# 0215Arthur/Pytorch_News_Recommender

Measured on AMD Instinct MI355X. Metric: users/sec (train step) NRMS MIND-small hist=50 cand=5, higher is better.
Workload: dtype f16 (MFMA inputs and saved activations; fp32 accumulate, softmax, loss, master weights and Adam); 1 GPU; configs[1] shapes: NRMS(nrms_v0) train step, 512 users/GPU, hist=50, cand=5, title_len=30, d=300, h=10, q=200, V=45800, dropout=0.2, Adam(lr=1e-3); users_per_gpu=512, global_batch=512, parallelism=dp1, precision=fp16, resident_batches=32

## Files before the change

include/nrms_hip.h:

```cpp
#ifndef NRMS_HIP_H
#define NRMS_HIP_H

#include <stddef.h>
#include <stdint.h>

#ifdef __cplusplus
extern "C" {
#endif

#define NRMS_OK            0
#define NRMS_EINVAL       -1
#define NRMS_ELAUNCH      -2
#define NRMS_EWORKSPACE   -3

#define NRMS_PRECISION_FP32   0
#define NRMS_PRECISION_BF16X3 1
#define NRMS_PRECISION_BF16   2
#define NRMS_FP16_KP 320
#define NRMS_FP16_DP 320
#define NRMS_FP16_QP 224
#define NRMS_PRECISION_FP16   3

#define NRMS_FLAG_PAD_ROW_ZERO 1
#define NRMS_FLAG_DEFER_WQKV 2
// ... 11 lines not shown
    int32_t  q_dim;
    int32_t  vocab;
    float    p_drop_embed;
    float    p_drop_ctx;
    int32_t  precision;
    int32_t  use_output_proj;
    int32_t  mask_mode;
    int32_t  flags;
    uint64_t seed;
    float    loss_scale;
    float    p_drop_attn;
    const int32_t* seq_index;
} nrms_encoder_desc;

typedef struct nrms_encoder_weights {
    const float* table;
    const float* w_qkv;
    const float* b_qkv;
    const float* w_o;
    const float* b_o;
    const float* w_add;
    const float* b_add;
    const float* q_vec;
} nrms_encoder_weights;

typedef struct nrms_encoder_grads {
    float* table;
    float* w_qkv;
    float* b_qkv;
    float* w_o;
    float* b_o;
    float* w_add;
    float* b_add;
    float* q_vec;
} nrms_encoder_grads;

typedef struct nrms_encoder_acts {
    float* x;
    float* qkv;
    float* attn;
    float* ctx;
    float* t;
    float* w;
    void*  scratch;
} nrms_encoder_acts;

size_t nrms_encoder_fwd_scratch_bytes(const nrms_encoder_desc* desc);
size_t nrms_encoder_fused_qkv_bytes(const nrms_encoder_desc* desc);
int nrms_encoder_fwd(const nrms_encoder_desc* desc, const nrms_encoder_weights* w,
                     const int64_t* ids, const float* x, const uint8_t* mask ,
                     const nrms_encoder_acts* acts, float* out, void* stream);

size_t nrms_encoder_bwd_workspace_bytes(const nrms_encoder_desc* desc);
int nrms_encoder_bwd(const nrms_encoder_desc* desc, const nrms_encoder_weights* w,
                     const int64_t* ids, const float* x, const uint8_t* mask,
                     const nrms_encoder_acts* acts, const float* dout,
                     const nrms_encoder_grads* grads, float* dx,
                     void* workspace, size_t workspace_bytes, void* stream);
typedef struct nrms_table_adam {
    float*   param;
    float*   exp_avg;
    float*   exp_avg_sq;
    double   lr, beta1, beta2, eps;
    int32_t  step;
    float    grad_scale;
    int32_t* n_nonfinite;
} nrms_table_adam;
int nrms_encoder_bwd_adam(const nrms_encoder_desc* desc, const nrms_encoder_weights* w,
                          const int64_t* ids, const float* x, const uint8_t* mask,
                          const nrms_encoder_acts* acts, const float* dout,
                          const nrms_encoder_grads* grads, float* dx,
                          void* workspace, size_t workspace_bytes, const nrms_table_adam* table_adam, void* stream);
int nrms_encoder_bwd_wqkv(const nrms_encoder_desc* desc, const int64_t* ids, const float* x,
                          const nrms_encoder_acts* acts, const nrms_encoder_grads* grads,
                          void* workspace, size_t workspace_bytes, void* stream);
int nrms_encoder_join(void* stream);

int nrms_sanitize_ids(const int64_t* src, int64_t* dst, int64_t n, int32_t vocab, int32_t* n_bad, void* stream);
int nrms_sanitize_ids_i32(const int32_t* src, int64_t* dst, int64_t n, int32_t vocab, int32_t* n_bad, void* stream);

int nrms_title_dedup(const int64_t* ids, int64_t n_titles, int32_t seq_len, int32_t* table, int64_t table_size,
                     int32_t* inverse, int32_t* rep_rows, int32_t* n_unique, void* stream);

int nrms_click_score_fwd(int32_t B, int32_t C, int32_t d, const float* cand, const float* user,
                         const uint8_t* mask, float* scores, void* stream);
int nrms_click_score_indexed(int32_t B, int32_t C, int32_t d, const float* news_vec, int64_t n_vec, const int32_t* index,
                             const float* user, const uint8_t* mask, float* scores, void* stream);
int nrms_click_score_bwd(int32_t B, int32_t C, int32_t d, const float* cand, const float* user,
                         const uint8_t* mask, const float* dscores, float* dcand, float* duser,
                         void* stream);

int nrms_ce_loss_fwd_bwd(int32_t B, int32_t C, const float* scores, float* loss_sum,
                         float* dscores, float grad_scale, void* stream);

int nrms_adam_step(size_t n, float* param, const float* grad, float* exp_avg, float* exp_avg_sq,
                   double lr, double beta1, double beta2, double eps, int32_t step, float grad_scale,
                   void* stream);

int nrms_adam_step_guarded(size_t n, float* param, const float* grad, float* exp_avg, float* exp_avg_sq,
                           double lr, double beta1, double beta2, double eps, int32_t step, float grad_scale,
                           int32_t* n_nonfinite, void* stream);
int nrms_adam_step_rest(size_t n, float* param, const float* grad, float* exp_avg, float* exp_avg_sq,
                        double lr, double beta1, double beta2, double eps, int32_t step, float grad_scale,
                        int32_t* n_nonfinite, void* stream);
int nrms_grad_guard(size_t n, float* grad, int32_t* n_nonfinite, void* stream);

int nrms_impression_auc(int32_t n_imp, int32_t max_c, const float* scores, const uint8_t* labels,
                        const int32_t* lens, double* auc, void* stream);

int nrms_impression_metrics(int32_t n_imp, int32_t max_c, const float* scores, const uint8_t* labels,
                            const int32_t* lens, int32_t k_a, int32_t k_b, double* auc, double* mrr, double* ndcg_a,
                            double* ndcg_b, int32_t* ranks, void* stream);

size_t nrms_topk_dot_workspace_bytes(int32_t B, int64_t N, int32_t d, int32_t k);
int nrms_topk_dot(int32_t B, int64_t N, int32_t d, int32_t k, const float* user, const float* items, const int64_t* exclude,
                  int32_t n_exclude, float* top_scores, int64_t* top_ids, void* workspace, size_t workspace_bytes, void* stream);

size_t nrms_topk_grouped_dot_workspace_bytes(int32_t B, int64_t N, int32_t d, int32_t k, int32_t G);
int nrms_topk_grouped_dot(int32_t B, int64_t N, int32_t d, int32_t k, int32_t G, const float* query, const float* items,
                          const int32_t* item_ids, const int64_t* group_ptr, const int64_t* exclude, int32_t n_exclude,
                          float* top_scores, int64_t* top_ids, void* workspace, size_t workspace_bytes, void* stream);

size_t nrms_topk_sections_dot_workspace_bytes(int32_t B, int64_t N, int32_t d, int32_t k, int32_t G, int32_t slice_tiles);
int nrms_topk_sections_dot(int32_t B, int64_t N, int32_t d, int32_t k, int32_t G, int32_t slice_tiles, const float* user,
                           const float* items , const int32_t* item_ids, const int64_t* section_ptr,
                           const float* bias , const int64_t* exclude, int32_t n_exclude,
                           float* top_scores , int64_t* top_ids , void* workspace,
                           size_t workspace_bytes, void* stream);

size_t nrms_rank_dot_workspace_bytes(int32_t B, int64_t N, int32_t d, int32_t T, int32_t n_exclude);
int nrms_rank_dot(int32_t B, int64_t N, int32_t d, int32_t T, const float* user, const float* items, const int64_t* targets,
                  const int64_t* exclude, int32_t n_exclude, int32_t* ranks, float* target_scores, void* workspace,
                  size_t workspace_bytes, void* stream);

size_t nrms_topk_dot_biased_workspace_bytes(int32_t B, int64_t N, int32_t d, int32_t k);
int nrms_topk_dot_biased(int32_t B, int64_t N, int32_t d, int32_t k, const float* user, const float* items,
                         const float* bias , const int64_t* exclude, int32_t n_exclude, float* top_scores,
                         int64_t* top_ids, void* workspace, size_t workspace_bytes, void* stream);
size_t nrms_rank_dot_biased_workspace_bytes(int32_t B, int64_t N, int32_t d, int32_t T, int32_t n_exclude);
int nrms_rank_dot_biased(int32_t B, int64_t N, int32_t d, int32_t T, const float* user, const float* items,
                         const float* bias , const int64_t* targets, const int64_t* exclude,
                         int32_t n_exclude, int32_t* ranks, float* target_scores, void* workspace, size_t workspace_bytes,
                         void* stream);

size_t nrms_topk_dot_windowed_workspace_bytes(int32_t B, int64_t N, int32_t d, int32_t k);
int nrms_topk_dot_windowed(int32_t B, int64_t N, int32_t d, int32_t k, const float* user, const float* items,
// ... 220 lines not shown
```

pytorch_news_recommender_amd/_lib.py:

```python
from __future__ import annotations

import ctypes as C
import os

PKG = os.path.dirname(os.path.abspath(__file__))
LIB_PATH = os.environ.get("NRMS_HIP_LIB") or os.path.join(PKG, "libnrms_hip.so")

NRMS_OK, NRMS_EINVAL, NRMS_ELAUNCH, NRMS_EWORKSPACE = 0, -1, -2, -3
NRMS_FLAG_PAD_ROW_ZERO = 1
NRMS_FLAG_DEFER_WQKV = 2
NRMS_FLAG_FWD_SCRATCH_KEPT = 4
NRMS_FLAG_FUSED_SEQ64 = 8
NRMS_FLAG_DEFER_USER_JOIN = 16
NRMS_FLAG_TABLE_ADAM = 32
NRMS_PRECISION_FP32 = 0
NRMS_PRECISION_BF16X3 = 1
NRMS_PRECISION_BF16 = 2
NRMS_PRECISION_FP16 = 3
NRMS_DROPOUT_FIELDS16 = 0x100
NRMS_DROPOUT_SITE_NEWSVEC = 4
NRMS_FP16_KP, NRMS_FP16_DP, NRMS_FP16_QP = 320, 320, 224
PRECISIONS = {"fp32": 0, "bf16x3": 1, "bf16": 2, "fp16": 3}


# ... 20 lines not shown


class TableAdam(C.Structure):
    _fields_ = [("param", C.c_void_p), ("exp_avg", C.c_void_p), ("exp_avg_sq", C.c_void_p), ("lr", C.c_double), ("beta1", C.c_double),
                ("beta2", C.c_double), ("eps", C.c_double), ("step", C.c_int32), ("grad_scale", C.c_float), ("n_nonfinite", C.c_void_p)]


class EncoderActs(C.Structure):
    _fields_ = [("x", C.c_void_p), ("qkv", C.c_void_p), ("attn", C.c_void_p), ("ctx", C.c_void_p),
                ("t", C.c_void_p), ("w", C.c_void_p), ("scratch", C.c_void_p)]


class SegPoolDesc(C.Structure):
    _fields_ = [("n_rows", C.c_int64), ("n_seg", C.c_int64), ("nnz", C.c_int64), ("d", C.c_int32), ("q", C.c_int32),
                ("precision", C.c_int32), ("flags", C.c_int32)]


NRMS_SEGPOOL_ROWS_UNIQUE = 1


class ClickGraphDesc(C.Structure):
    _fields_ = [("n_users", C.c_int64), ("n_news", C.c_int64), ("n_edges", C.c_int64), ("user_ptr", C.c_void_p),
                ("user_news", C.c_void_p), ("news_ptr", C.c_void_p), ("news_users", C.c_void_p)]


class NewsFeatures(C.Structure):
    _fields_ = [("n", C.c_int64), ("d_text", C.c_int32), ("d_cat", C.c_int32), ("n_cat", C.c_int32), ("n_sub", C.c_int32),
                ("p_drop", C.c_float), ("seed", C.c_uint64), ("title_vec", C.c_void_p), ("abst_vec", C.c_void_p),
                ("cat_table", C.c_void_p), ("sub_table", C.c_void_p), ("categ", C.c_void_p), ("subcateg", C.c_void_p)]


class NewsvecDesc(C.Structure):
    _fields_ = [("n_slots", C.c_int64), ("n_rows", C.c_int32), ("d", C.c_int32), ("precision", C.c_int32),
                ("p_drop", C.c_float), ("seed", C.c_uint64)]


SIGNATURES = {
    "nrms_encoder_fwd": (C.c_int, [C.POINTER(EncoderDesc), C.POINTER(EncoderWeights), C.c_void_p, C.c_void_p,
                                   C.c_void_p, C.POINTER(EncoderActs), C.c_void_p, C.c_void_p]),
    "nrms_encoder_bwd_workspace_bytes": (C.c_size_t, [C.POINTER(EncoderDesc)]),
    "nrms_encoder_fwd_scratch_bytes": (C.c_size_t, [C.POINTER(EncoderDesc)]),
    "nrms_encoder_fused_qkv_bytes": (C.c_size_t, [C.POINTER(EncoderDesc)]),
    "nrms_encoder_bwd": (C.c_int, [C.POINTER(EncoderDesc), C.POINTER(EncoderWeights), C.c_void_p, C.c_void_p,
                                   C.c_void_p, C.POINTER(EncoderActs), C.c_void_p, C.POINTER(EncoderGrads), C.c_void_p,
                                   C.c_void_p, C.c_size_t, C.c_void_p]),
    "nrms_encoder_bwd_adam": (C.c_int, [C.POINTER(EncoderDesc), C.POINTER(EncoderWeights), C.c_void_p, C.c_void_p,
                                        C.c_void_p, C.POINTER(EncoderActs), C.c_void_p, C.POINTER(EncoderGrads), C.c_void_p,
                                        C.c_void_p, C.c_size_t, C.POINTER(TableAdam), C.c_void_p]),
    "nrms_encoder_bwd_wqkv": (C.c_int, [C.POINTER(EncoderDesc), C.c_void_p, C.c_void_p, C.POINTER(EncoderActs),
                                        C.POINTER(EncoderGrads), C.c_void_p, C.c_size_t, C.c_void_p]),
    "nrms_encoder_join": (C.c_int, [C.c_void_p]),
    "nrms_sanitize_ids": (C.c_int, [C.c_void_p, C.c_void_p, C.c_int64, C.c_int32, C.c_void_p, C.c_void_p]),
    "nrms_sanitize_ids_i32": (C.c_int, [C.c_void_p, C.c_void_p, C.c_int64, C.c_int32, C.c_void_p, C.c_void_p]),
    "nrms_title_dedup": (C.c_int, [C.c_void_p, C.c_int64, C.c_int32, C.c_void_p, C.c_int64, C.c_void_p, C.c_void_p,
                                   C.c_void_p, C.c_void_p]),
    "nrms_click_score_indexed": (C.c_int, [C.c_int32, C.c_int32, C.c_int32, C.c_void_p, C.c_int64, C.c_void_p, C.c_void_p,
                                           C.c_void_p, C.c_void_p, C.c_void_p]),
    "nrms_click_score_fwd": (C.c_int, [C.c_int32, C.c_int32, C.c_int32, C.c_void_p, C.c_void_p, C.c_void_p,
                                       C.c_void_p, C.c_void_p]),
    "nrms_click_score_bwd": (C.c_int, [C.c_int32, C.c_int32, C.c_int32, C.c_void_p, C.c_void_p, C.c_void_p,
                                       C.c_void_p, C.c_void_p, C.c_void_p, C.c_void_p]),
    "nrms_ce_loss_fwd_bwd": (C.c_int, [C.c_int32, C.c_int32, C.c_void_p, C.c_void_p, C.c_void_p, C.c_float,
                                       C.c_void_p]),
    "nrms_adam_step": (C.c_int, [C.c_size_t, C.c_void_p, C.c_void_p, C.c_void_p, C.c_void_p, C.c_double,
                                 C.c_double, C.c_double, C.c_double, C.c_int32, C.c_float, C.c_void_p]),
    "nrms_adam_step_guarded": (C.c_int, [C.c_size_t, C.c_void_p, C.c_void_p, C.c_void_p, C.c_void_p, C.c_double,
                                         C.c_double, C.c_double, C.c_double, C.c_int32, C.c_float, C.c_void_p, C.c_void_p]),
    "nrms_adam_step_rest": (C.c_int, [C.c_size_t, C.c_void_p, C.c_void_p, C.c_void_p, C.c_void_p, C.c_double,
                                      C.c_double, C.c_double, C.c_double, C.c_int32, C.c_float, C.c_void_p, C.c_void_p]),
    "nrms_grad_guard": (C.c_int, [C.c_size_t, C.c_void_p, C.c_void_p, C.c_void_p]),
    "nrms_segment_pool_workspace_bytes": (C.c_size_t, [C.POINTER(SegPoolDesc)]),
    "nrms_segment_pool_fwd": (C.c_int, [C.POINTER(SegPoolDesc)] + [C.c_void_p] * 10 + [C.c_void_p, C.c_size_t, C.c_void_p]),
    "nrms_segment_pool_bwd": (C.c_int, [C.POINTER(SegPoolDesc)] + [C.c_void_p] * 12 + [C.c_void_p, C.c_size_t, C.c_void_p]),
    "nrms_hier_tree_scratch_bytes": (C.c_size_t, [C.c_int32, C.c_int32]),
    "nrms_hier_tree_build": (C.c_int, [C.c_int32, C.c_int32] + [C.c_void_p] * 16 + [C.c_size_t, C.c_void_p]),
    "nrms_hier_add_embedding_fwd": (C.c_int, [C.c_int64, C.c_int32, C.c_int32, C.c_void_p, C.c_void_p, C.c_void_p, C.c_void_p, C.c_void_p]),
    "nrms_sequence_partition_count_ints": (C.c_size_t, [C.c_int32]),
    "nrms_sequence_partition": (C.c_int, [C.c_void_p, C.c_int32, C.c_int32, C.c_void_p, C.c_void_p, C.c_void_p]),
    "nrms_encoder_empty_workspace_bytes": (C.c_size_t, [C.POINTER(EncoderDesc)]),
    "nrms_encoder_empty_saved_bytes": (C.c_size_t, [C.POINTER(EncoderDesc)]),
    "nrms_encoder_empty_fwd": (C.c_int, [C.POINTER(EncoderDesc), C.POINTER(EncoderWeights), C.c_void_p, C.c_void_p, C.c_void_p, C.c_void_p, C.c_size_t,
                                         C.c_void_p]),
    "nrms_encoder_empty_bwd": (C.c_int, [C.POINTER(EncoderDesc), C.POINTER(EncoderWeights), C.c_void_p, C.c_void_p, C.c_void_p, C.POINTER(EncoderGrads),
                                         C.c_void_p, C.c_size_t, C.c_void_p]),
    "nrms_csr_from_padded": (C.c_int, [C.c_int64, C.c_int32, C.c_void_p, C.c_int64, C.c_void_p, C.c_void_p, C.c_void_p]),
    "nrms_graph_sample_workspace_bytes": (C.c_size_t, [C.c_int64, C.c_int32]),
    "nrms_graph_sample_neighbors": (C.c_int, [C.POINTER(ClickGraphDesc), C.c_int64, C.c_int32, C.c_void_p, C.c_uint64, C.c_void_p, C.c_void_p,
                                              C.c_void_p, C.c_size_t, C.c_void_p]),
    "nrms_graph_resolve_workspace_bytes": (C.c_size_t, [C.c_int64]),
    "nrms_graph_resolve_rows": (C.c_int, [C.c_int64, C.c_int32, C.c_int64, C.c_void_p, C.c_void_p, C.c_int32] + [C.c_void_p] * 4
                                + [C.c_void_p, C.c_size_t, C.c_void_p]),
    "nrms_negative_sample_workspace_bytes": (C.c_size_t, [C.c_int64, C.c_int64, C.c_int32]),
    "nrms_negative_sample": (C.c_int, [C.c_int64] + [C.c_void_p] * 4 + [C.c_int32, C.c_int32, C.c_uint64] + [C.c_void_p] * 3
                             + [C.c_void_p, C.c_size_t, C.c_void_p]),
    "nrms_catalogue_negative_sample_workspace_bytes": (C.c_size_t, [C.c_int64, C.c_int64, C.c_int32]),
    "nrms_catalogue_negative_sample": (C.c_int, [C.c_int64] + [C.c_void_p] * 3 + [C.c_int64, C.c_void_p, C.c_void_p, C.c_int64, C.c_void_p, C.c_int32,
                                                 C.c_uint64] + [C.c_void_p] * 4 + [C.c_void_p, C.c_size_t, C.c_void_p]),
    "nrms_hier_add_embedding_bwd_workspace_bytes": (C.c_size_t, [C.c_int64, C.c_int32, C.c_int32]),
    "nrms_hier_add_embedding_bwd": (C.c_int, [C.c_int64, C.c_int32, C.c_int32, C.c_void_p, C.c_void_p, C.c_void_p, C.c_void_p, C.c_void_p,
                                              C.c_size_t, C.c_void_p]),
    "nrms_hier_match": (C.c_int, [C.c_int32, C.c_int32, C.c_int32] + [C.c_void_p] * 11 + [C.c_void_p]),
    "nrms_hier_score_fwd": (C.c_int, [C.c_int32, C.c_int32, C.c_int32] + [C.c_void_p] * 9 + [C.c_float, C.c_float, C.c_void_p, C.c_void_p]),
    "nrms_hier_score_bwd": (C.c_int, [C.c_int32, C.c_int32, C.c_int32] + [C.c_void_p] * 9 + [C.c_float, C.c_float] + [C.c_void_p] * 5 + [C.c_void_p]),
    "nrms_impression_auc": (C.c_int, [C.c_int32, C.c_int32, C.c_void_p, C.c_void_p, C.c_void_p, C.c_void_p,
                                      C.c_void_p]),
    "nrms_impression_metrics": (C.c_int, [C.c_int32, C.c_int32, C.c_void_p, C.c_void_p, C.c_void_p, C.c_int32, C.c_int32]
# ... 110 lines not shown
```

pytorch_news_recommender_amd/csrc/capi.hip:

```cpp
#include <stdarg.h>

#include <algorithm>

#include <mutex>
#include <vector>

#include "gemm.h"

namespace nrms {

int launch_attention(bool bwd, int n_seq, int S, int d, int h, const float* qkv, float* ctx, const Dropout& drop,
                     const float* dctx, float* dqkv, const uint8_t* mask, const int64_t* ids, const float* bias_hm,
                     const int* pos, float* padsum, float* dbias, hipStream_t stream, const Dropout* pdrop = nullptr,
                     bool split = false);
size_t attention_padsum_floats();
int launch_addattn_fwd(int n_seq, int S, int d, int q, const float* ctx, const float* w_add, const float* b_add,
                       const float* q_vec, float* T, float* wout, float* out, const uint8_t* mask, int npass,
                       void* wplanes, hipStream_t stream);
int addattn_bwd_rows_waves(int n_seq);
int launch_addattn_bwd_rows(int n_seq, int S, int d, int q, const float* ctx, const float* dout, const float* w,
                            const float* T, float* ds, float* dq_partial, float* dq, const uint8_t* mask,
                            hipStream_t stream);

int launch_attention_wide(bool bwd, int n_seq, int S, int d, int h, const float* qkv, float* ctx, const Dropout& pdrop,
// ... 368 lines not shown
    if (workspace_bytes < L.total) { set_error("encoder_bwd(fp16): workspace %zu < required %zu bytes", workspace_bytes, L.total); return NRMS_EWORKSPACE; }
    NRMS_REQUIRE(((uintptr_t)workspace & 255) == 0, "encoder_bwd(fp16): workspace must be 256-byte aligned");
    if (desc->n_seq == 0) return NRMS_OK;
    const int S = desc->seq_len, d = desc->d_model;
    const long M = (long)desc->n_seq * S;
    char* base = (char*)workspace;
    Fused16Bwd f{};
    f.n_seq = desc->n_seq; f.S = S; f.d = d; f.h = desc->n_heads; f.q = desc->q_dim;
    f.workspace = base + L.fused;
    f.w_qkv = w->w_qkv; f.b_qkv = w->b_qkv; f.w_add = w->w_add; f.q_vec = w->q_vec;
    f.x16 = acts->x; f.ctx16 = acts->ctx; f.t16 = acts->t; f.w = acts->w; f.dout = dout;
    f.loss_scale = desc->loss_scale;
    f.drop = make_dropout(desc->seed, desc->p_drop_ctx);
    f.dw_qkv = grads->w_qkv; f.db_qkv = grads->b_qkv; f.dw_add = grads->w_add; f.db_add = grads->b_add; f.dq_vec = grads->q_vec;
    if (v1) { f.w_o = w->w_o; f.attn16 = acts->attn; f.dw_o = grads->w_o; f.db_o = grads->b_o; }
    int rc;
    int* live = (int*)(base + L.live);
    int* n_live = (int*)(base + L.n_live);
    if (gather) {
        const bool kept = (desc->flags & NRMS_FLAG_FWD_SCRATCH_KEPT) != 0 && skip_pad_rows(desc) && acts->scratch != nullptr &&
                          kept_matches(desc, acts->scratch, ids);
        if (kept) {
            const Fwd16Scratch fs = fwd16_scratch(desc);
            char* fb = (char*)acts->scratch;
            live = (int*)(fb + fs.live);
            n_live = (int*)(fb + fs.n_live);
            f.pos = (int*)(fb + fs.pos); f.n_rows_dev = n_live; f.ids = ids;
            if (S <= 32) { f.order = (int*)(fb + fs.order); f.order_cnt = (int*)(fb + fs.order_cnt); }
        } else {
            int* pos = (int*)(base + L.pos);
            rc = launch_compact_live_rows(M, ids, live, pos, n_live, (int*)(base + L.cscr), s);
            if (rc) return rc;
            if (skip_pad_rows(desc)) {
                int* order = (int*)(base + L.order);
                int* order_cnt = (int*)(base + L.order_cnt);
                f.pos = pos; f.n_rows_dev = n_live; f.ids = ids;
                if (S <= 32) {
                    rc = launch_title_order(desc->n_seq, S, ids, order, order_cnt, s, 3);
                    if (rc) return rc;
                    f.order = order; f.order_cnt = order_cnt;
                }
            }
        }
        f.dx = (float*)(base + L.dxc);
        f.dx_fp16 = skip_pad_rows(desc);
    } else {
        f.dx = dx;
    }
    SideSet* ss_prep = (gather && skip_pad_rows(desc)) ? side_streams_for(s) : nullptr;
    bool prepared = false;
    if (ss_prep != nullptr) {
        rc = side_order(ss_prep, 5, s, ss_prep->s[1], "encoder_bwd(fp16)");
        if (rc) return rc;
        rc = launch_scatter_prepare(M, desc->vocab, ids, live, n_live, (int*)(base + L.sscr), ss_prep->s[1]);
        if (hipEventRecord(ss_prep->ev[4], ss_prep->s[1]) != hipSuccess) { set_error("encoder_bwd(fp16): hipEventRecord failed"); return NRMS_ELAUNCH; }
        if (rc) { (void)hipStreamWaitEvent(s, ss_prep->ev[4], 0); return rc; }
        prepared = true;
    }
    auto join_prepare = [&]() -> int {
        if (!prepared) return NRMS_OK;
        if (hipStreamWaitEvent(s, ss_prep->ev[4], 0) != hipSuccess) { set_error("encoder_bwd(fp16): hipStreamWaitEvent failed"); return NRMS_ELAUNCH; }
        return NRMS_OK;
    };
    const float* sc_dev = nullptr;
    f.sc_out = &sc_dev;
    f.defer_join = (desc->flags & NRMS_FLAG_DEFER_WQKV) != 0;
    rc = v1 ? launch_fused_bwd16v1(f, s) : launch_fused_bwd16(f, s);
    {
        const int rj = join_prepare();
        if (rc) return rc;
        if (rj) return rj;
    }
    if (gather) {
        const Dropout drop_e = make_dropout(desc->seed, desc->p_drop_embed);
        if (tadam != nullptr)
            rc = launch_scatter_grouped_adam(M, desc->vocab, d, ids, live, n_live, f.dx, drop_e, grads->table, (int*)(base + L.sscr), s,
                                             f.dx_fp16, NRMS_FP16_KP, sc_dev, prepared, *tadam);
        else if (skip_pad_rows(desc))
            rc = launch_scatter_grouped(M, desc->vocab, d, ids, live, n_live, f.dx, drop_e, grads->table, (int*)(base + L.sscr), s,
                                        f.dx_fp16, NRMS_FP16_KP, sc_dev, prepared);
        else
            rc = launch_scatter_dense_rows(M, d, ids, live, n_live, f.dx, drop_e, grads->table, s);
    }
    return rc;
}

extern "C" int nrms_encoder_fwd(const nrms_encoder_desc* desc, const nrms_encoder_weights* w, const int64_t* ids,
                                const float* x, const uint8_t* mask, const nrms_encoder_acts* acts, float* out,
                                void* stream) {
    int rc = validate_desc(desc, "encoder_fwd");
    if (rc) return rc;
    NRMS_REQUIRE((desc->flags & NRMS_FLAG_TABLE_ADAM) == 0, "encoder_fwd: flags 0x%x: NRMS_FLAG_TABLE_ADAM belongs to nrms_encoder_bwd_adam", desc->flags);
    if (acts != nullptr) kept_forget(acts->scratch);
    if (desc->precision == NRMS_PRECISION_FP16) {
        NRMS_REQUIRE(w && acts && out, "encoder_fwd: null argument");
        NRMS_REQUIRE(w->w_qkv && w->b_qkv && w->w_add && w->b_add && w->q_vec, "encoder_fwd: null weight");
        NRMS_REQUIRE(desc->vocab > 0 ? (ids != nullptr && w->table != nullptr) : (x != nullptr), "encoder_fwd: input missing");
        if (desc->n_seq == 0) return NRMS_OK;
        return encoder_fwd16(desc, w, ids, x, acts, out, (hipStream_t)stream);
    }
    NRMS_REQUIRE(w && acts && out, "encoder_fwd: null argument");
    NRMS_REQUIRE(w->w_qkv && w->b_qkv && w->w_add && w->b_add && w->q_vec, "encoder_fwd: null weight");
    if (desc->flags & NRMS_FLAG_FUSED_SEQ64) {
        NRMS_REQUIRE(x != nullptr && acts->qkv != nullptr && acts->scratch != nullptr, "encoder_fwd(fused): x, acts.qkv and acts.scratch are required");
        const bool train = acts->ctx != nullptr && acts->t != nullptr && acts->w != nullptr;
        if (desc->n_seq == 0) return NRMS_OK;
// ... 51 lines not shown
    }
    g.A = xin; g.lda = d;
    rc = nt_gemm(desc, A_PLAIN, E_STORE, g, wplanes, s, "qkv_proj_fwd");
    if (rc) return rc;
    Dropout pdrop_attn = make_dropout(desc->seed, desc->p_drop_attn);
    pdrop_attn.seq_index = desc->seq_index; pdrop_attn.seq_h = desc->n_heads;
    if (wide_attention(desc))
        rc = launch_attention_wide(false, desc->n_seq, S, d, desc->n_heads, acts->qkv, wo ? acts->attn : acts->ctx,
                                   pdrop_attn, nullptr, nullptr, amask, s);
    else
        rc = launch_attention(false, desc->n_seq, S, d, desc->n_heads, acts->qkv, wo ? acts->attn : acts->ctx,
                              wo ? no_drop : drop_c, nullptr, nullptr, amask,
                              (gather && skip_pad_rows(desc)) ? ids : nullptr, (gather && skip_pad_rows(desc)) ? bq_hm : nullptr,
                              nullptr, nullptr, nullptr, s, &pdrop_attn, desc->precision != NRMS_PRECISION_FP32);
    if (rc) return rc;
    if (wo) {
        NTArgs o{};
        o.M = M; o.N = d; o.K = d; o.rows_per_tile = NT_BM;
        o.A = acts->attn; o.lda = d; o.W = w->w_o; o.bias = w->b_o; o.C = acts->ctx; o.ldc = d; o.drop = drop_c;
        rc = nt_gemm(desc, A_PLAIN, E_STORE, o, wplanes, s, "out_proj_fwd");
        if (rc) return rc;
    }
    if (wide_additive(desc)) {
        NRMS_REQUIRE(acts->t != nullptr, "encoder_fwd: acts.t is required for q_dim > 256 or d_model > 512 (also for inference)");
        NTArgs z{};
        z.M = M; z.N = q; z.K = d; z.rows_per_tile = NT_BM;
        z.A = acts->ctx; z.lda = d; z.W = w->w_add; z.bias = w->b_add; z.C = acts->t; z.ldc = q;
        rc = nt_gemm(desc, A_PLAIN, E_STORE, z, wplanes, s, "addattn_proj_fwd");
        if (rc) return rc;
        return launch_addattn_rows_fwd_wide(desc->n_seq, S, d, q, acts->t, w->q_vec, acts->ctx, pmask, acts->w, out, s);
    }
    const int npass = desc->precision == NRMS_PRECISION_FP32 ? 0 : (desc->precision == NRMS_PRECISION_BF16X3 ? 3 : 1);
    return launch_addattn_fwd(desc->n_seq, S, d, q, acts->ctx, w->w_add, w->b_add, w->q_vec, acts->t, acts->w, out,
                              pmask, npass, wplanes, s);
}

extern "C" size_t nrms_encoder_fwd_scratch_bytes(const nrms_encoder_desc* desc) {
    if (validate_desc(desc, "encoder_fwd_scratch_bytes")) return 0;
    if (desc->precision == NRMS_PRECISION_FP16) return fwd16_scratch(desc).total;
    return fwd_scratch(desc).total;
}

extern "C" size_t nrms_encoder_fused_qkv_bytes(const nrms_encoder_desc* desc) {
    if (desc == nullptr || !(desc->flags & NRMS_FLAG_FUSED_SEQ64) || validate_desc(desc, "encoder_fused_qkv_bytes")) return 0;
    return user64_qkv_bytes(desc->n_seq, desc->n_heads);
}

extern "C" size_t nrms_encoder_bwd_workspace_bytes(const nrms_encoder_desc* desc) {
    if (validate_desc(desc, "encoder_bwd_workspace_bytes")) return 0;
    if (desc->precision == NRMS_PRECISION_FP16) return bwd16_layout(desc).total;
    return bwd_layout(desc).total;
}

namespace nrms {
struct SideEntry { int device; hipStream_t caller; SideSet* set; };
static std::mutex g_side_mu;
static std::vector<SideEntry> g_side_sets;

SideSet* side_streams_for(hipStream_t caller) {
    if (getenv("NRMS_NO_SIDE_STREAMS") != nullptr) return nullptr;
    int dev = 0;
    if (hipGetDevice(&dev) != hipSuccess) return nullptr;
    std::lock_guard<std::mutex> lk(g_side_mu);
    for (const SideEntry& e : g_side_sets)
        if (e.device == dev && e.caller == caller) return e.set;
    if (g_side_sets.size() >= 32) return nullptr;
    SideSet* ss = new SideSet();
    bool ok = true;
    for (int i = 0; i < 2 && ok; ++i) ok = hipStreamCreateWithFlags(&ss->s[i], hipStreamNonBlocking) == hipSuccess;
    for (int i = 0; i < SIDE_EVENTS && ok; ++i) ok = hipEventCreateWithFlags(&ss->ev[i], hipEventDisableTiming) == hipSuccess;
    if (!ok) {
        for (int i = 0; i < 2; ++i) if (ss->s[i]) (void)hipStreamDestroy(ss->s[i]);
        for (int i = 0; i < SIDE_EVENTS; ++i) if (ss->ev[i]) (void)hipEventDestroy(ss->ev[i]);
        delete ss;
        ss = nullptr;
        (void)hipGetLastError();
    }
    g_side_sets.push_back(SideEntry{dev, caller, ss});
    return ss;
}

int side_order(SideSet* ss, int e, hipStream_t from, hipStream_t to, const char* what) {
    if (hipEventRecord(ss->ev[e], from) != hipSuccess || hipStreamWaitEvent(to, ss->ev[e], 0) != hipSuccess) {
        set_error("%s: ordering the helper stream failed: %s", what, hipGetErrorString(hipGetLastError()));
        return NRMS_ELAUNCH;
    }
    return NRMS_OK;
}

int side_join_user(SideSet* ss, hipStream_t caller, const char* what) {
    if (ss == nullptr || !ss->pending_user) return NRMS_OK;
    ss->pending_user = false;
    if (hipStreamWaitEvent(caller, ss->ev[SIDE_EV_USER], 0) != hipSuccess) {
        set_error("%s: hipStreamWaitEvent failed", what);
        return NRMS_ELAUNCH;
    }
    return NRMS_OK;
}

SideJoinGuard::~SideJoinGuard() {
    if (!armed) return;
    for (int i = 0; i < 2; ++i)
        if (hipEventRecord(ss->ev[6 + i], ss->s[i]) == hipSuccess) (void)hipStreamWaitEvent(caller, ss->ev[6 + i], 0);
}
}

// ... 36 lines not shown
extern "C" int nrms_encoder_join(void* stream) { return fused_bwd16_join((hipStream_t)stream); }

static int encoder_bwd_chain(const nrms_encoder_desc* desc, const nrms_encoder_weights* w, const int64_t* ids,
                             const float* x, const uint8_t* mask, const nrms_encoder_acts* acts, const float* dout,
                             const nrms_encoder_grads* grads, float* dx, void* workspace, size_t workspace_bytes,
                             const TableAdam* tadam, hipStream_t s) {
    int rc;
    NRMS_REQUIRE(w && acts && dout && grads && workspace, "encoder_bwd: null argument");
    NRMS_REQUIRE(acts->qkv && acts->ctx && acts->t && acts->w, "encoder_bwd: all saved activations are required");
    NRMS_REQUIRE(grads->w_qkv && grads->b_qkv && grads->w_add && grads->b_add && grads->q_vec,
                 "encoder_bwd: null gradient buffer");
    const bool gather = desc->vocab > 0, wo = desc->use_output_proj != 0;
    NRMS_REQUIRE(gather ? (ids != nullptr && acts->x != nullptr && grads->table != nullptr) : (x != nullptr && dx != nullptr),
                 "encoder_bwd: %s missing", gather ? "ids/acts.x/grads.table" : "x/dx");
    NRMS_REQUIRE(!wo || (w->w_o && acts->attn && grads->w_o && grads->b_o),
                 "encoder_bwd: use_output_proj needs w_o, acts.attn, grads.w_o, grads.b_o");
    NRMS_REQUIRE(desc->mask_mode == 0 || mask != nullptr, "encoder_bwd: mask_mode=%d but mask is null", desc->mask_mode);
    const BwdWorkspace L = bwd_layout(desc);
    if (workspace_bytes < L.total) {
        set_error("encoder_bwd: workspace %zu < required %zu bytes", workspace_bytes, L.total);
        return NRMS_EWORKSPACE;
    }
    NRMS_REQUIRE(((uintptr_t)workspace & 255) == 0, "encoder_bwd: workspace must be 256-byte aligned");
    if (desc->n_seq == 0) return NRMS_OK;
    const int S = desc->seq_len, d = desc->d_model, q = desc->q_dim, M = desc->n_seq * S;
    const Dropout drop_e = make_dropout(desc->seed, desc->p_drop_embed);
    const Dropout drop_c = make_dropout(desc->seed, desc->p_drop_ctx);
    const Dropout no_drop = make_dropout(0, 0.f);
    const uint8_t* amask = (desc->mask_mode & 1) ? mask : nullptr;
    const uint8_t* pmask = (desc->mask_mode & 2) ? mask : nullptr;
    char* base = (char*)workspace;
    float* dctx = (float*)(base + L.dctx);
    float* dqkv = (float*)(base + L.dqkv);
    float* dattn = (float*)(base + L.dattn);
    float* ds = (float*)(base + L.ds);
    float* wqkv_t = (float*)(base + L.wqkv_t);
    float* wadd_t = (float*)(base + L.wadd_t);
    float* wo_t = (float*)(base + L.wo_t);
    float* tn_partial = (float*)(base + L.tn_partial);
    float* dq_partial = (float*)(base + L.dq_partial);
    void* wplanes = (void*)(base + L.wplanes);

    rc = fused_bwd16_join(s);
    if (rc) return rc;
    SideSet* ss = side_streams_for(s);
    const bool side = ss != nullptr;
    hipStream_t s2 = side ? ss->s[0] : s;
    SideJoinGuard join_guard(ss, s);
    auto fork = [&](int i) -> int {
        return side ? side_order(ss, i, s, s2, "encoder_bwd") : NRMS_OK;
    };

    const bool fused64 = (desc->flags & NRMS_FLAG_FUSED_SEQ64) != 0;
    if (fused64) {
        rc = launch_user64_bwd(desc->n_seq, S, d, desc->n_heads, q, w->w_add, w->q_vec, base + L.u64planes, dout, acts->t, acts->w,
                               acts->qkv, ds, dq_partial, grads->q_vec, dqkv, s);
        if (rc) return rc;
    } else {
        if (wide_additive(desc))
            rc = launch_addattn_rows_bwd_wide(desc->n_seq, S, d, q, acts->ctx, dout, acts->w, acts->t, ds, dq_partial, grads->q_vec,
                                              pmask, s);
        else
            rc = launch_addattn_bwd_rows(desc->n_seq, S, d, q, acts->ctx, dout, acts->w, acts->t, ds, dq_partial, grads->q_vec,
                                         pmask, s);
        if (rc) return rc;
    }
    rc = fork(0);
    if (rc) return rc;
    {
        TNArgs t{};
        t.M = M; t.N = q; t.K = d; t.amode = A_DZ;
        t.ds = ds; t.qv = w->q_vec; t.T = acts->t; t.B = acts->ctx; t.ldb = d;
        t.dW = grads->w_add; t.dbias = grads->b_add; t.partial = tn_partial;
        rc = tn_gemm(desc, t, s2, "dwadd_bwd");
        if (rc) return rc;
    }
    if (!fused64) {
        rc = launch_transpose(w->w_add, wadd_t, q, d, s);
        if (rc) return rc;
        {
            NTArgs g{};
            g.M = M; g.N = d; g.K = q; g.rows_per_tile = NT_BM;
            g.ds = ds; g.qv = w->q_vec; g.T = acts->t;
            g.W = wadd_t; g.C = dctx; g.ldc = d;
            g.wrow = acts->w; g.dout = dout; g.seq_of_row = make_row_div((uint32_t)S);
            g.drop = drop_c;
            rc = nt_gemm(desc, A_DZ, E_DCTX, g, wplanes, s, "dctx_bwd");
            if (rc) return rc;
        }
}
    const float* dattn_in = dctx;
    if (wo) {
        rc = fork(1);
        if (rc) return rc;
        TNArgs t{};
        t.M = M; t.N = d; t.K = d; t.amode = A_PLAIN;
        t.A = dctx; t.lda = d; t.B = acts->attn; t.ldb = d;
        t.dW = grads->w_o; t.dbias = grads->b_o; t.partial = tn_partial;
        rc = tn_gemm(desc, t, s2, "dwo_bwd");
        if (rc) return rc;
        if (side && hipEventRecord(ss->ev[3], s2) != hipSuccess) {
            set_error("encoder_bwd: hipEventRecord failed");
            return NRMS_ELAUNCH;
        }
        rc = launch_transpose(w->w_o, wo_t, d, d, s);
        if (rc) return rc;
        NTArgs g{};
        g.M = M; g.N = d; g.K = d; g.rows_per_tile = NT_BM;
        g.A = dctx; g.lda = d; g.W = wo_t; g.C = dattn; g.ldc = d;
        rc = nt_gemm(desc, A_PLAIN, E_STORE, g, wplanes, s, "dattn_bwd");
        if (rc) return rc;
        dattn_in = dattn;
    }
    int* live = (int*)(base + L.live);
    int* pos = (int*)(base + L.pos);
    int* n_live = (int*)(base + L.n_live);
    const bool compact = skip_pad_rows(desc);
    const HeadPerm perm{d / desc->n_heads, desc->n_heads};
    if (gather) {
        rc = launch_compact_live_rows((long)M, ids, live, compact ? pos : nullptr, n_live, (int*)(base + L.cscr), s);
        if (rc) return rc;
    }
    Dropout pdrop_attn = make_dropout(desc->seed, desc->p_drop_attn);
    pdrop_attn.seq_index = desc->seq_index; pdrop_attn.seq_h = desc->n_heads;
    if (fused64)
        rc = NRMS_OK;
    else if (wide_attention(desc))
        rc = launch_attention_wide(true, desc->n_seq, S, d, desc->n_heads, acts->qkv, nullptr, pdrop_attn, dattn_in, dqkv, amask, s);
    else
        rc = launch_attention(true, desc->n_seq, S, d, desc->n_heads, acts->qkv, nullptr, no_drop, dattn_in, dqkv, amask,
                              nullptr, nullptr, compact ? pos : nullptr, compact ? (float*)(base + L.padsum) : nullptr,
                              compact ? grads->b_qkv : nullptr, s, &pdrop_attn, desc->precision != NRMS_PRECISION_FP32);
    if (rc) return rc;
    if ((desc->flags & NRMS_FLAG_DEFER_WQKV) == 0) {
        rc = fork(2);
        if (rc) return rc;
        rc = bwd_wqkv(desc, gather ? acts->x : x, dqkv, n_live, grads, tn_partial, s2);
        if (rc) return rc;
    }
    rc = launch_transpose(w->w_qkv, wqkv_t, 3 * d, d, s, perm);
    if (rc) return rc;
    {
        NTArgs g{};
        g.M = M; g.N = d; g.K = 3 * d; g.rows_per_tile = NT_BM;
        g.A = dqkv; g.lda = 3 * d; g.W = wqkv_t;
        g.C = gather ? dctx : dx; g.ldc = d;
        if (gather) { g.a_rows = compact ? nullptr : live; g.m_dev = n_live; }
        if (side && wo && gather && hipStreamWaitEvent(s, ss->ev[3], 0) != hipSuccess) {
            set_error("encoder_bwd: hipStreamWaitEvent failed");
            return NRMS_ELAUNCH;
        }
        rc = nt_gemm(desc, A_PLAIN, E_STORE, g, wplanes, s, "dx_bwd");
        if (rc) return rc;
    }
    if (gather) {
        const bool atomic_scatter = getenv("NRMS_ATOMIC_SCATTER") != nullptr;
        if (tadam != nullptr)
            rc = launch_scatter_grouped_adam((long)M, desc->vocab, d, ids, live, n_live, dctx, drop_e, grads->table,
                                             (int*)(base + L.sscr), s, false, 0, nullptr, false, *tadam);
        else if (atomic_scatter) rc = launch_scatter_dropout_compact((long)M, d, ids, live, n_live, dctx, drop_e, grads->table, s);
        else rc = launch_scatter_grouped((long)M, desc->vocab, d, ids, live, n_live, dctx, drop_e, grads->table,
                                         (int*)(base + L.sscr), s);
    }
    if (side && rc == NRMS_OK) {
        if (!gather && (desc->flags & NRMS_FLAG_DEFER_USER_JOIN) != 0) {
            if (hipEventRecord(ss->ev[SIDE_EV_USER], s2) != hipSuccess) { set_error("encoder_bwd: hipEventRecord failed"); return NRMS_ELAUNCH; }
            ss->pending_user = true;
            join_guard.disarm();
        } else {
            rc = side_order(ss, 4, s2, s, "encoder_bwd");
            if (rc == NRMS_OK) join_guard.disarm();
        }
    }
    return rc;
}

extern "C" int nrms_encoder_bwd(const nrms_encoder_desc* desc, const nrms_encoder_weights* w, const int64_t* ids,
                                const float* x, const uint8_t* mask, const nrms_encoder_acts* acts, const float* dout,
                                const nrms_encoder_grads* grads, float* dx, void* workspace, size_t workspace_bytes,
                                void* stream) {
    return nrms_encoder_bwd_adam(desc, w, ids, x, mask, acts, dout, grads, dx, workspace, workspace_bytes, nullptr, stream);
}

extern "C" int nrms_encoder_bwd_adam(const nrms_encoder_desc* desc, const nrms_encoder_weights* w, const int64_t* ids,
                                     const float* x, const uint8_t* mask, const nrms_encoder_acts* acts, const float* dout,
                                     const nrms_encoder_grads* grads, float* dx, void* workspace, size_t workspace_bytes,
                                     const nrms_table_adam* table_adam, void* stream) {
    int rc = validate_desc(desc, "encoder_bwd");
    if (rc) return rc;
    NRMS_REQUIRE(((desc->flags & NRMS_FLAG_TABLE_ADAM) != 0) == (table_adam != nullptr),
                 "encoder_bwd: NRMS_FLAG_TABLE_ADAM and the nrms_table_adam operands (nrms_encoder_bwd_adam) go together");
    TableAdam tadam_v{};
    const TableAdam* tadam = nullptr;
    if (table_adam != nullptr) {
        rc = table_adam_args(desc, w, grads, table_adam, &tadam_v);
        if (rc) return rc;
        tadam = &tadam_v;
        NRMS_REQUIRE(desc->precision == NRMS_PRECISION_FP16 || getenv("NRMS_ATOMIC_SCATTER") == nullptr,
// ... 32 lines not shown
                                  const float* dy, float* dx, float* dgamma_dbeta, void* workspace, size_t workspace_bytes,
                                  void* stream) {
    NRMS_REQUIRE(n_rows >= 0 && d > 0, "layernorm_bwd: n_rows=%ld d=%d", (long)n_rows, d);
    NRMS_REQUIRE(n_rows == 0 || (x && gamma && stats && dy && dx && dgamma_dbeta && workspace), "layernorm_bwd: null argument");
    if (workspace_bytes < nrms_layernorm_bwd_workspace_bytes(d)) {
        set_error("layernorm_bwd: workspace %zu < required %zu bytes", workspace_bytes, nrms_layernorm_bwd_workspace_bytes(d));
        return NRMS_EWORKSPACE;
    }
    return launch_layernorm_bwd((long)n_rows, d, x, gamma, stats, dy, dx, dgamma_dbeta, (float*)workspace, (hipStream_t)stream);
}

static int features_args(const nrms_news_features* f, FeatArgs* a, const char* who) {
    NRMS_REQUIRE(f != nullptr, "%s: null descriptor", who);
    NRMS_REQUIRE(f->n >= 0 && f->d_text > 0 && f->d_cat > 0 && f->n_cat > 0 && f->n_sub > 0, "%s: bad sizes", who);
    NRMS_REQUIRE(f->p_drop >= 0.f && f->p_drop < 1.f, "%s: p_drop must be in [0,1)", who);
    NRMS_REQUIRE((long)f->n * (2 * f->d_text + 2 * f->d_cat) < (1L << 40), "%s: too many elements", who);
    NRMS_REQUIRE(f->n == 0 || (f->categ && f->subcateg), "%s: null ids", who);
    a->n = (long)f->n; a->dt = f->d_text; a->dc = f->d_cat; a->n_cat = f->n_cat; a->n_sub = f->n_sub;
    a->title = f->title_vec; a->abst = f->abst_vec; a->cat_table = f->cat_table; a->sub_table = f->sub_table;
    a->categ = f->categ; a->subcateg = f->subcateg;
    a->drop = make_dropout(f->seed, f->p_drop);
    return NRMS_OK;
}

extern "C" int nrms_news_features_fwd(const nrms_news_features* f, float* out, void* stream) {
    FeatArgs a{};
    int rc = features_args(f, &a, "news_features_fwd");
    if (rc) return rc;
    NRMS_REQUIRE(f->n == 0 || (f->title_vec && f->abst_vec && f->cat_table && f->sub_table && out), "news_features_fwd: null argument");
    a.out = out;
    return launch_features_fwd(a, (hipStream_t)stream);
}

extern "C" int nrms_news_features_bwd(const nrms_news_features* f, const float* dout, float* d_title_vec, float* d_abst_vec,
                                      float* d_cat_table, float* d_sub_table, void* stream) {
    FeatArgs a{};
    int rc = features_args(f, &a, "news_features_bwd");
    if (rc) return rc;
    NRMS_REQUIRE(f->n == 0 || (dout && d_title_vec && d_abst_vec && d_cat_table && d_sub_table), "news_features_bwd: null argument");
    a.dout = dout; a.d_title = d_title_vec; a.d_abst = d_abst_vec; a.d_cat_table = d_cat_table; a.d_sub_table = d_sub_table;
    return launch_features_bwd(a, (hipStream_t)stream);
}

extern "C" int nrms_sanitize_ids(const int64_t* src, int64_t* dst, int64_t n, int32_t vocab, int32_t* n_bad, void* stream) {
    NRMS_REQUIRE(n >= 0 && vocab > 0, "sanitize_ids: n=%ld vocab=%d", (long)n, vocab);
    NRMS_REQUIRE(n == 0 || (src && dst && n_bad), "sanitize_ids: null argument");
    return launch_sanitize_ids((long)n, src, false, dst, vocab, n_bad, (hipStream_t)stream);
}

extern "C" int nrms_sanitize_ids_i32(const int32_t* src, int64_t* dst, int64_t n, int32_t vocab, int32_t* n_bad, void* stream) {
    NRMS_REQUIRE(n >= 0 && vocab > 0, "sanitize_ids_i32: n=%ld vocab=%d", (long)n, vocab);
    NRMS_REQUIRE(n == 0 || (src && dst && n_bad), "sanitize_ids_i32: null argument");
    return launch_sanitize_ids((long)n, src, true, dst, vocab, n_bad, (hipStream_t)stream);
}

extern "C" size_t nrms_sequence_partition_count_ints(int32_t n_seq) { return n_seq >= 0 ? title_order_cnt_ints(n_seq) : 0; }

extern "C" int nrms_sequence_partition(const int64_t* ids, int32_t n_seq, int32_t seq_len, int32_t* order, int32_t* counts, void* stream) {
    NRMS_REQUIRE(n_seq >= 0 && seq_len >= 1 && seq_len <= 64, "sequence_partition: n_seq=%d seq_len=%d", n_seq, seq_len);
    NRMS_REQUIRE(counts != nullptr, "sequence_partition: null counts");
    if (n_seq == 0) return hipMemsetAsync(counts, 0, 2 * sizeof(int), (hipStream_t)stream) == hipSuccess ? NRMS_OK : NRMS_ELAUNCH;
    NRMS_REQUIRE(ids && order, "sequence_partition: null argument");
    return launch_title_order(n_seq, seq_len, ids, order, counts, (hipStream_t)stream, 2);
}

extern "C" int nrms_title_dedup(const int64_t* ids, int64_t n_titles, int32_t seq_len, int32_t* table, int64_t table_size,
                                int32_t* inverse, int32_t* rep_rows, int32_t* n_unique, void* stream) {
    NRMS_REQUIRE(n_titles >= 0 && n_titles < (1L << 30) && seq_len >= 1, "title_dedup: n_titles=%ld seq_len=%d", (long)n_titles, seq_len);
    NRMS_REQUIRE(n_unique != nullptr, "title_dedup: null n_unique");
    NRMS_REQUIRE(n_titles == 0 || (ids && table && inverse && rep_rows), "title_dedup: null argument");
    NRMS_REQUIRE(n_titles == 0 || (table_size >= 2 * n_titles && (table_size & (table_size - 1)) == 0),
                 "title_dedup: table_size=%ld must be a power of two >= 2 * n_titles (%ld)", (long)table_size, (long)n_titles);
    return launch_title_dedup((long)n_titles, seq_len, ids, table, (long)table_size, inverse, rep_rows, n_unique, (hipStream_t)stream);
}

extern "C" void nrms_timing_enable(int enable) {
    std::lock_guard<std::mutex> lk(g_tmu);
    g_timing = enable != 0;
}

extern "C" void nrms_timing_reset(void) {
    std::lock_guard<std::mutex> lk(g_tmu);
    for (auto& t : g_launches) { (void)hipEventDestroy(t.start); (void)hipEventDestroy(t.stop); }
    g_launches.clear();
}

extern "C" int nrms_timing_read(const char* prefix, double* total_ms, int64_t* launches) {
    std::lock_guard<std::mutex> lk(g_tmu);
    double tot = 0.0;
    int64_t n = 0;
    const std::string p = prefix ? prefix : "";
    for (auto& t : g_launches) {
        if (t.name.compare(0, p.size(), p) != 0) continue;
        if (hipEventSynchronize(t.stop) != hipSuccess) { set_error("timing_read: event sync failed"); return NRMS_ELAUNCH; }
        float ms = 0.f;
        if (hipEventElapsedTime(&ms, t.start, t.stop) != hipSuccess) { set_error("timing_read: elapsed failed"); return NRMS_ELAUNCH; }
        tot += ms;
        ++n;
    }
    if (total_ms) *total_ms = tot;
    if (launches) *launches = n;
    return NRMS_OK;
}

extern "C" const char* nrms_last_error(void) { return g_err; }
extern "C" const char* nrms_version(void) { return "nrms_hip 0.3 (gfx950, fp32 MFMA; nrms_v0 + nrms_v1 topologies)"; }
// ... 1 lines not shown
```

pytorch_news_recommender_amd/csrc/common.h:

```cpp
#pragma once
#include <hip/hip_runtime.h>
#include <stdint.h>
#include <stdio.h>
#include <string>

#include "../../include/nrms_hip.h"

namespace nrms {

typedef float f32x4 __attribute__((ext_vector_type(4)));
typedef float f32x16 __attribute__((ext_vector_type(16)));

constexpr int WAVE = 64;

__device__ __forceinline__ f32x4 mfma16(float a, float b, f32x4 c) {
    return __builtin_amdgcn_mfma_f32_16x16x4f32(a, b, c, 0, 0, 0);
}
__device__ __forceinline__ f32x16 mfma32(float a, float b, f32x16 c) {
    return __builtin_amdgcn_mfma_f32_32x32x2f32(a, b, c, 0, 0, 0);
}
__device__ __forceinline__ int crow32(int r, int hh) { return (r & 3) + 8 * (r >> 2) + 4 * hh; }

struct Keep4 { bool k[4]; };

// ... 84 lines not shown
    }
};

struct Dropout {
    uint64_t seed;
    uint32_t thresh;
    float inv_keep;
    uint32_t thresh16;
    const int* seq_index;
    int seq_h;
    __device__ __forceinline__ long unit_of(long unit) const {
        if (seq_index == nullptr) return unit;
        const long seq = unit / seq_h;
        return (long)seq_index[seq] * seq_h + (unit - seq * seq_h);
    }
};

inline Dropout make_dropout(uint64_t seed, float p) {
    Dropout d;
    d.seed = seed;
    d.thresh = drop_threshold(p);
    d.thresh16 = drop_threshold16(p);
    d.inv_keep = p > 0.f ? 1.0f / (1.0f - p) : 1.0f;
    d.seq_index = nullptr;
    d.seq_h = 1;
    return d;
}

__device__ __forceinline__ float wave_sum(float v) {
#pragma unroll
    for (int o = 32; o > 0; o >>= 1) v += __shfl_xor(v, o, 64);
    return v;
}
__device__ __forceinline__ float wave_max(float v) {
#pragma unroll
    for (int o = 32; o > 0; o >>= 1) v = fmaxf(v, __shfl_xor(v, o, 64));
    return v;
}

__device__ __forceinline__ void adam_update(float& p, float& m, float& v, float g, float step_size, float b1, float b2, float omb1,
                                            float omb2, float inv_sqrt_bc2, float eps) {
#pragma clang fp contract(off)
    m = b1 * m + omb1 * g;
    v = b2 * v + omb2 * g * g;
    const float denom = sqrtf(v) * inv_sqrt_bc2 + eps;
    p = __builtin_fmaf(-step_size, m / denom, p);
}
struct AdamConsts { float step_size, b1, b2, omb1, omb2, inv_sqrt_bc2, eps; };
AdamConsts adam_consts(double lr, double beta1, double beta2, double eps, int32_t step);

void set_error(const char* fmt, ...);
int check_launch(const char* what);

constexpr int SIDE_EVENTS = 9, SIDE_EV_USER = 8;
struct SideSet {
    hipStream_t s[2] = {nullptr, nullptr};
    hipEvent_t ev[SIDE_EVENTS] = {nullptr, nullptr, nullptr, nullptr, nullptr, nullptr, nullptr, nullptr, nullptr};
    bool pending = false;
    bool pending_user = false;
};
int side_join_user(SideSet* ss, hipStream_t caller, const char* what);
SideSet* side_streams_for(hipStream_t caller);
int side_order(SideSet* ss, int e, hipStream_t from, hipStream_t to, const char* what);
struct SideJoinGuard {
    SideSet* ss; hipStream_t caller; bool armed;
    SideJoinGuard(SideSet* set, hipStream_t c) : ss(set), caller(c), armed(set != nullptr) {}
    void disarm() { armed = false; }
    ~SideJoinGuard();
};

struct TimingScope {
    TimingScope(const char* name, hipStream_t s);
    ~TimingScope();
    bool active;
    int slot;
    hipStream_t stream;
};

#define NRMS_REQUIRE(cond, ...)                         \
    do {                                                \
        if (!(cond)) {                                  \
            ::nrms::set_error(__VA_ARGS__);             \
            return NRMS_EINVAL;                         \
        }                                               \
    } while (0)

__host__ __device__ inline int cdiv(long a, long b) { return (int)((a + b - 1) / b); }

}
```

pytorch_news_recommender_amd/csrc/embed.hip:

```cpp
#include "gemm.h"

#include <algorithm>

namespace nrms {

__global__ __launch_bounds__(256) void gather_dropout_kernel(unsigned total4, unsigned d4, const int64_t* ids,
                                                             const float* table, Dropout drop, float* x) {
    const unsigned stride = gridDim.x * blockDim.x;
    for (unsigned i = blockIdx.x * blockDim.x + threadIdx.x; i < total4; i += stride) {
        const unsigned m = i / d4, c4 = i - m * d4;
        const long id = ids[m];
        f32x4 v = *reinterpret_cast<const f32x4*>(table + id * (long)(4 * d4) + 4 * c4);
        if (drop.thresh != 0u) v *= dropout_scale4(drop.seed, 0u, (uint64_t)i, drop.thresh, drop.inv_keep);
        reinterpret_cast<f32x4*>(x)[i] = v;
    }
}

__global__ __launch_bounds__(256) void gather_dropout_compact_kernel(unsigned d4, const int64_t* ids, const int* live,
                                                                     const int* n_live, const float* table, Dropout drop,
                                                                     float* x) {
    const unsigned total4 = (unsigned)(*n_live) * d4;
    const unsigned stride = gridDim.x * blockDim.x;
    for (unsigned i = blockIdx.x * blockDim.x + threadIdx.x; i < total4; i += stride) {
        const unsigned r = i / d4, c4 = i - r * d4;
        const long t = live[r];
        f32x4 v = *reinterpret_cast<const f32x4*>(table + ids[t] * (long)(4 * d4) + 4 * c4);
        if (drop.thresh != 0u) v *= dropout_scale4(drop.seed, 0u, (uint64_t)(t * d4 + c4), drop.thresh, drop.inv_keep);
        reinterpret_cast<f32x4*>(x)[i] = v;
    }
}

int launch_gather_dropout_compact(long M, int d, const int64_t* ids, const int* live, const int* n_live,
                                  const float* table, const Dropout& drop, float* x, hipStream_t stream) {
    if (M <= 0) return NRMS_OK;
    if (M * (d / 4) >= (1L << 32)) { set_error("gather: %ld float4 elements overflow the 32-bit index", M * (d / 4)); return NRMS_EINVAL; }
    int blocks = cdiv(M * (d / 4), 256);
    if (blocks > 256 * 16) blocks = 256 * 16;
    TimingScope ts("gather_dropout", stream);
    hipLaunchKernelGGL(gather_dropout_compact_kernel, dim3(blocks), dim3(256), 0, stream, (unsigned)(d / 4), ids, live,
                       n_live, table, drop, x);
    return check_launch("gather_dropout");
}

template <bool SKIP_ALL_PAD, int FILL_SLICES>
__global__ __launch_bounds__(256) void fill_pad_rows_kernel_t(long n_seq, int S, int n4, const int64_t* ids, const float* row,
                                                              float* out) {
    const int lane = threadIdx.x & 63;
    const long wave = (long)blockIdx.x * 4 + (threadIdx.x >> 6), n_waves = (long)gridDim.x * 4;
    f32x4 b[FILL_SLICES];
#pragma unroll
    for (int i = 0; i < FILL_SLICES; ++i)
        b[i] = (lane + 64 * i < n4) ? reinterpret_cast<const f32x4*>(row)[lane + 64 * i] : f32x4{0.f, 0.f, 0.f, 0.f};
    for (long q = wave; q < n_seq; q += n_waves) {
        const bool is_pad = lane < S && ids[q * S + lane] == 0;
        unsigned long long m = __ballot(is_pad);
// ... 371 lines not shown
    return check_launch("scatter_grouped");
}

int launch_scatter_grouped_adam(long M, int V, int d, const int64_t* ids, const int* live, const int* n_live, const void* dx,
                                const Dropout& drop, float* dtable, int* scratch, hipStream_t stream, bool dx_fp16, int ldx,
                                const float* sc, bool prepared, const TableAdam& a) {
    if (M <= 0 || V <= 0) { set_error("scatter_grouped_adam: nothing to scatter (the caller runs the plain Adam step)"); return NRMS_EINVAL; }
    if ((d & 3) != 0 || d > 1024 || (dx_fp16 && d > 512)) { set_error("scatter_grouped_adam: d=%d unsupported", d); return NRMS_EINVAL; }
    if (!prepared) {
        const int rc = launch_scatter_prepare(M, V, ids, live, n_live, scratch, stream);
        if (rc) return rc;
    }
    int* cnt = scratch;
    int* cursor = cnt + V + 64;
    int* total = cursor + V;
    int* order = cursor + V + 64;
    const bool guard = a.n_bad != nullptr;
    TimingScope ts("adam", stream);
    auto go = [&](auto kernel, int ld, const float* scp) {
        hipLaunchKernelGGL(kernel, dim3(cdiv(V, 4)), dim3(256), 0, stream, V, d / 4, live, cnt, total, order, dx, ld, scp, drop, dtable, a);
    };
    if (dx_fp16) { if (guard) go(scatter_grouped_adam_kernel<true, 2, true>, ldx, sc); else go(scatter_grouped_adam_kernel<true, 2, false>, ldx, sc); }
    else if (d <= 512) { if (guard) go(scatter_grouped_adam_kernel<false, 2, true>, d, nullptr); else go(scatter_grouped_adam_kernel<false, 2, false>, d, nullptr); }
    else { if (guard) go(scatter_grouped_adam_kernel<false, 4, true>, d, nullptr); else go(scatter_grouped_adam_kernel<false, 4, false>, d, nullptr); }
    return check_launch("scatter_grouped_adam");
}

template <class SRC>
__global__ __launch_bounds__(256) void sanitize_ids_kernel(long n, const SRC* src, int64_t* dst, long vocab, int* n_bad) {
    int bad = 0;
    for (long i = (long)blockIdx.x * blockDim.x + threadIdx.x; i < n; i += (long)gridDim.x * blockDim.x) {
        const int64_t v = (int64_t)src[i];
        const bool ok = v >= 0 && v < vocab;
        bad += ok ? 0 : 1;
        dst[i] = ok ? v : 0;
    }
    const unsigned long long m = __ballot(bad != 0);
    if (m != 0ull) {
        bad = (int)wave_sum((float)bad);
        if ((threadIdx.x & 63) == 0) atomicAdd(n_bad, bad);
    }
}

int launch_sanitize_ids(long n, const void* src, bool src_is_int32, int64_t* dst, int vocab, int* n_bad, hipStream_t stream) {
    if (n <= 0) return NRMS_OK;
    int blocks = cdiv(n, 256 * 4);
    if (blocks > 256 * 8) blocks = 256 * 8;
    TimingScope ts("sanitize_ids", stream);
    if (src_is_int32)
        hipLaunchKernelGGL(sanitize_ids_kernel<int32_t>, dim3(blocks), dim3(256), 0, stream, n, (const int32_t*)src, dst, (long)vocab, n_bad);
    else
        hipLaunchKernelGGL(sanitize_ids_kernel<int64_t>, dim3(blocks), dim3(256), 0, stream, n, (const int64_t*)src, dst, (long)vocab, n_bad);
    return check_launch("sanitize_ids");
}

__global__ __launch_bounds__(256) void dedup_insert_kernel(long n, int L, const int64_t* ids, int* table, unsigned mask,
                                                           int* inverse, int* rep_rows, int* n_unique) {
    const int lane = threadIdx.x & 63;
    for (long t = (long)blockIdx.x * blockDim.x + threadIdx.x; t < n; t += (long)gridDim.x * blockDim.x) {
        const int64_t* row = ids + t * L;
        uint64_t h = 0x9E3779B97F4A7C15ull ^ (uint64_t)L;
        int64_t any = 0;
        for (int i = 0; i < L; ++i) {
            const int64_t w = row[i];
            any |= w;
            uint64_t k = (uint64_t)w * 0xFF51AFD7ED558CCDull;
            k ^= k >> 32;
            h = (h ^ k) * 0xC4CEB9FE1A85EC53ull;
            h ^= h >> 29;
        }
        h ^= h >> 33; h *= 0xFF51AFD7ED558CCDull; h ^= h >> 33;
        const bool pad = any == 0;
        const unsigned long long pads = __ballot(pad);
        const int leader = pads != 0 ? __ffsll((long long)pads) - 1 : 0;
        int result = 0;
        if (!pad || lane == leader) {
            unsigned slot = (unsigned)h & mask;
            for (;;) {
                int cur = __hip_atomic_load(table + slot, __ATOMIC_RELAXED, __HIP_MEMORY_SCOPE_AGENT);
                if (cur < 0) {
                    cur = atomicCAS(table + slot, -1, (int)t);
                    if (cur < 0) {
                        const int u = atomicAdd(n_unique, 1);
                        rep_rows[u] = (int)t;
                        result = u;
                        break;
                    }
                }
                const int64_t* other = ids + (long)cur * L;
                bool same = true;
                for (int i = 0; i < L; ++i) same = same && other[i] == row[i];
                if (same) { result = -cur - 1; break; }
                slot = (slot + 1) & mask;
            }
        }
        const int lead = __shfl(result, leader);
        inverse[t] = (pad && lane != leader) ? lead : result;
    }
}

__global__ __launch_bounds__(256) void dedup_resolve_kernel(long n, int* inverse) {
    for (long t = (long)blockIdx.x * blockDim.x + threadIdx.x; t < n; t += (long)gridDim.x * blockDim.x) {
        const int v = inverse[t];
        if (v < 0) inverse[t] = inverse[-v - 1];
    }
}
// ... 33 lines not shown
```

pytorch_news_recommender_amd/csrc/fused16_bwd.hip:

```cpp
#include <stdlib.h>

#include <type_traits>

#include "fused16_bwd.h"

namespace nrms {

template <int SB>
__global__ __launch_bounds__(F16_THREADS, SB == 1 ? 8 / F16_WAVES : 1) void fused_bwd16_pool_kernel(Bwd16Args a) {
    extern __shared__ __attribute__((aligned(16))) char smem[];
    float* red = reinterpret_cast<float*>(smem + 3 * F16_SLOT);
    float* stg_t = red + B16_RED;
    float* stg_h = stg_t + F16_WAVES * SB * 2 * F16_QT * 32;
    const int tid = threadIdx.x, lane = tid & 63;
    const int wave = __builtin_amdgcn_readfirstlane(tid >> 6);
    const int l32 = lane & 31, hh = lane >> 5;
    const int S = a.S;
    constexpr int DP = F16_DP, QP = F16_QP;

    for (int i = tid; i < B16_RED; i += F16_THREADS) red[i] = 0.f;

    h8 idf[2], sel[2];
#pragma unroll
    for (int s = 0; s < 2; ++s)
// ... 498 lines not shown
                        dq = mfma32h(acc_frag(k, 1), sf[jb][ib][1], dq);
                    }
                    const h8 dq0 = acc_frag(dq, 0), dq1 = acc_frag(dq, 1);
                    if (drow[ib] >= 0) {
                        _Float16* orow = a.dqkv16 + drow[ib] * (long)B16_DQ + head * 96 + 8 * hh;
                        *reinterpret_cast<h8*>(orow) = dq0;
                        *reinterpret_cast<h8*>(orow + 16) = dq1;
                    }
                    sq += regsum(transpose_frags(dq0, dq1, idf));
                }
                sq += __shfl_xor(sq, 32, 64);
                if (hh == 0) srow[0] = sq;
            }
            if constexpr (DMA) {
                if (has_rows) ring.template step_barrier<6>(st); else ring.step_barrier(st);
                ++st;
            } else {
                __syncthreads();
            }
            if (tid < 96) {
                float sum = 0.f;
#pragma unroll
                for (int w = 0; w < F16_WAVES; ++w) sum += stg[(((head & 1) * F16_WAVES + w) * 3) * 32 + tid];
                red[3 * head * 32 + tid] += sum;
            }
            ++n;
        }
#pragma unroll
        for (int b = 0; b < SB; ++b) {
            if (drow[b] >= 0) {
                for (int head = a.h; head < 10; ++head) {
                    _Float16* orow = a.dqkv16 + drow[b] * (long)B16_DQ + head * 96 + 8 * hh;
#pragma unroll
                    for (int c = 0; c < 96; c += 16) *reinterpret_cast<h8*>(orow + c) = z8;
                }
            }
        }
        if constexpr (!DMA) __syncthreads();
    }
    __syncthreads();
    float* out = a.red + (long)blockIdx.x * B16_RED;
    for (int i = tid; i < B16_RED; i += F16_THREADS) out[i] = red[i];
}

__device__ __forceinline__ float loss_scale_from_max(unsigned max_bits, float fixed) {
    if (fixed > 0.f) return fixed;
    const int e = (int)((max_bits >> 23) & 0xFF) - 127;
    if (max_bits == 0u || e == 128) return 1.0f;
    int k = 6 - e + (int)fmaxf(fixed, -24.f);
    k = k < -100 ? -100 : (k > 100 ? 100 : k);
    return __uint_as_float((unsigned)(k + 127) << 23);
}

__global__ __launch_bounds__(256) void absmax_kernel(long n, const float* x, unsigned* max_bits) {
    unsigned m = 0u;
    const long tid = (long)blockIdx.x * blockDim.x + threadIdx.x, nth = (long)gridDim.x * blockDim.x;
    if ((reinterpret_cast<uintptr_t>(x) & 15) == 0) {
        const f32x4* x4 = reinterpret_cast<const f32x4*>(x);
        const long n4 = n / 4;
        long i = tid;
        for (; i + 3 * nth < n4; i += 4 * nth) {
            f32x4 v[4];
#pragma unroll
            for (int u = 0; u < 4; ++u) v[u] = x4[i + u * nth];
#pragma unroll
            for (int u = 0; u < 4; ++u)
#pragma unroll
                for (int e = 0; e < 4; ++e) m = max(m, __float_as_uint(v[u][e]) & 0x7FFFFFFFu);
        }
        for (; i < n4; i += nth) {
            const f32x4 v = x4[i];
#pragma unroll
            for (int e = 0; e < 4; ++e) m = max(m, __float_as_uint(v[e]) & 0x7FFFFFFFu);
        }
        for (long i = (n & ~3L) + tid; i < n; i += nth) m = max(m, __float_as_uint(x[i]) & 0x7FFFFFFFu);
    } else {
        for (long i = tid; i < n; i += nth) m = max(m, __float_as_uint(x[i]) & 0x7FFFFFFFu);
    }
#pragma unroll
    for (int o = 32; o > 0; o >>= 1) m = max(m, (unsigned)__shfl_xor((int)m, o, 64));
    __shared__ unsigned wmax[4];
    if ((threadIdx.x & 63) == 0) wmax[threadIdx.x >> 6] = m;
    __syncthreads();
    if (threadIdx.x == 0) {
        m = max(max(wmax[0], wmax[1]), max(wmax[2], wmax[3]));
        if (m != 0u) atomicMax(max_bits, m);
    }
}

__device__ __forceinline__ void dout16_rows(long n_seq, int d, int h, int dk, float scale, float* sc, const float* dout, _Float16* dout16,
                                            int n_blocks) {
    if (blockIdx.x == 0 && threadIdx.x == 0) { sc[0] = scale; sc[1] = 1.0f / scale; }
    const long total = n_seq * F16_DP;
    for (long i = (long)blockIdx.x * blockDim.x + threadIdx.x; i < total; i += (long)n_blocks * blockDim.x) {
        const long r = i / F16_DP;
        const int p = (int)(i - r * F16_DP);
        const int b16 = p >> 4, t = p & 15, hh = t >> 3, jj = t & 7;
        const int fpad = 16 * b16 + 8 * (jj >> 2) + 4 * hh + (jj & 3);
        const int head = fpad >> 5, f = fpad & 31;
        float v = 0.f;
        if (head < h && f < dk) v = dout[r * d + head * dk + f] * scale;
        dout16[i] = (_Float16)v;
    }
}

__global__ __launch_bounds__(256) void dout16_kernel(long n_seq, int d, int h, int dk, float fixed_scale, const unsigned* max_bits,
                                                     float* sc, const float* dout, _Float16* dout16) {
    dout16_rows(n_seq, d, h, dk, loss_scale_from_max(*max_bits, fixed_scale), sc, dout, dout16, (int)gridDim.x);
}

struct Prep16bArgs {
    int d, h, dk, q;
    const float* w_qkv;
    const float* b_qkv;
    const float* w_add;
    const float* q_vec;
    float* bqkv32;
    _Float16* btiles;
    int dma_tiles;
    _Float16* xtiles;
    _Float16* qv16;
    unsigned* max_bits;
};

__global__ __launch_bounds__(256) void prep16b_kernel(Prep16bArgs a) {
    if (a.max_bits != nullptr && blockIdx.x == 0 && threadIdx.x == 0) *a.max_bits = 0u;
    const float qscale = 1.0f / sqrtf((float)a.dk);
    constexpr int KP = F16_KP;
    const long n1 = (long)4 * a.h * 32 * KP, n2 = (long)30 * 32 * KP, n3 = F16_QP, n4 = (long)3 * a.h * 32;
    for (long i = (long)blockIdx.x * blockDim.x + threadIdx.x; i < n1 + n2 + n3 + n4; i += (long)gridDim.x * blockDim.x) {
        if (i < n1) {
            int c = (int)(i % KP);
            const long r = i / KP;
            int f = (int)(r & 31);
            const int tile = (int)(r >> 5);
            float v = 0.f;
            if (tile < a.h) {
                const int head = tile;
                if (f < a.dk && c < a.q) v = a.w_add[(long)c * a.d + head * a.dk + f];
            } else {
// ... 325 lines not shown
    __syncthreads();
    if (rg != 0 || i >= B16_RED) return;
    s = 0.f;
#pragma unroll
    for (int r = 0; r < 32; ++r) s += part[r][c];
    s *= inv_scale;
    if (i < B16_RED_QKV) {
        const int tile = i >> 5, f = i & 31, head = tile / 3, which = tile - 3 * head;
        if (head < h && f < dk) db_qkv[which * d + head * dk + f] += s * (which == 0 ? qscale : 1.0f);
    } else if (i < B16_RED_QKV + F16_QP) {
        const int qq = i - B16_RED_QKV;
        if (qq < q) db_add[qq] += s;
    } else {
        const int qq = i - B16_RED_QKV - F16_QP;
        if (qq < q) dq_vec[qq] += s;
    }
}

struct Maps16 { int *nmap_qkv, *kmap_x, *nmap_add, *kmap_ctx; float *nscale_qkv, *nscale_add; };
__device__ __forceinline__ void maps16_entry(int i, int d, int h, int dk, int q, float inv_scale, float qscale, const Maps16& m) {
    int* const nmap_qkv = m.nmap_qkv; int* const kmap_x = m.kmap_x; int* const nmap_add = m.nmap_add; int* const kmap_ctx = m.kmap_ctx;
    float* const nscale_qkv = m.nscale_qkv; float* const nscale_add = m.nscale_add;
    if (i < B16_DQ) {
        const int head = i / 96, rem = i - head * 96, which = rem >> 5, p = rem & 31;
        const int s = p >> 4, t = p & 15, hh = t >> 3, jj = t & 7;
        const int f = 16 * s + 8 * (jj >> 2) + 4 * hh + (jj & 3);
        nmap_qkv[i] = (head < h && f < dk) ? which * d + head * dk + f : -1;
        nscale_qkv[i] = inv_scale * (which == 0 ? qscale : 1.0f);
    }
    if (i < F16_KP) kmap_x[i] = i < d ? i : -1;
    if (i < F16_QP) { nmap_add[i] = i < q ? i : -1; nscale_add[i] = inv_scale; }
    if (i < F16_DP) {
        const int b16 = i >> 4, t = i & 15, hh = t >> 3, jj = t & 7;
        const int fpad = 16 * b16 + 8 * (jj >> 2) + 4 * hh + (jj & 3);
        const int head = fpad >> 5, f = fpad & 31;
        kmap_ctx[i] = (head < h && f < dk) ? head * dk + f : -1;
    }
}

constexpr int MAPS16_BLOCKS = (B16_DQ + 255) / 256;
static_assert(B16_DQ >= F16_KP && B16_DQ >= F16_QP && B16_DQ >= F16_DP, "maps16_entry: one thread per entry of the longest map");
__global__ __launch_bounds__(256) void dout16_maps_kernel(long n_seq, int d, int h, int dk, int q, float fixed_scale, float qscale,
                                                          const unsigned* max_bits, float* sc, const float* dout, _Float16* dout16,
                                                          Maps16 m) {
    const float scale = loss_scale_from_max(*max_bits, fixed_scale);
    const int n_rows_blocks = (int)gridDim.x - MAPS16_BLOCKS;
    if ((int)blockIdx.x >= n_rows_blocks) {
        maps16_entry(((int)blockIdx.x - n_rows_blocks) * 256 + (int)threadIdx.x, d, h, dk, q, 1.0f / scale, qscale, m);
        return;
    }
    dout16_rows(n_seq, d, h, dk, scale, sc, dout, dout16, n_rows_blocks);
}

static size_t up256(size_t x) { return (x + 255) / 256 * 256; }


Fused16BwdLayout fused16_bwd_layout(long M, int n_seq) {
    Fused16BwdLayout L;
    const long Mp = (long)n_seq * (M > (long)n_seq * 32 ? 64 : 32);
    size_t off = 0;
    auto take = [&](size_t bytes) { size_t o = off; off = up256(off + bytes); return o; };
    L.n_wg = 512;
    L.btiles = take((size_t)40 * 32 * F16_KP * 2);
    L.xtiles = take((size_t)DX_SLABS * DX_B_BYTES);
    L.qv16 = take((size_t)F16_QP * 2);
    L.bqkv32 = take((size_t)30 * 32 * 4);
    L.dout16 = take((size_t)n_seq * F16_DP * 2);
    L.dz16 = take((size_t)Mp * F16_QP * 2);
    L.dctx16 = take((size_t)Mp * F16_DP * 2);
    L.dqkv16 = take((size_t)(M + 32) * B16_DQ * 2);
    L.red = take((size_t)2 * L.n_wg * B16_RED * 4);
    L.maps = take((size_t)(B16_DQ * 2 + F16_KP + F16_QP * 2 + F16_DP) * 4);
    L.scale = take(256);
    L.tn_splits_qkv = 40;
    L.tn_splits_add = 192;
    if (const char* e = getenv("NRMS_TN_SPLITS_QKV")) L.tn_splits_qkv = atoi(e);
    if (const char* e = getenv("NRMS_TN_SPLITS_ADD")) L.tn_splits_add = atoi(e);
    const size_t p1 = (size_t)L.tn_splits_qkv * B16_DQ * F16_KP * 4, p2 = (size_t)L.tn_splits_add * F16_QP * F16_DP * 4;
    L.partial = take(up256(p1) + p2);
    L.total = off;
    return L;
}

int launch_tn16(int geom, const _Float16* A, int lda, int N, const _Float16* B, int ldb, int K, int M, const int* m_dev,
                float* partial, int splits, const int* nmap, const int* kmap, const float* nscale, int ldw, float* dW,
                hipStream_t stream, const char* name, float* dbias, const int* blk_list, const int* blk_cnt, int blk_stride) {
    Tn16Args t{};
    t.M = M; t.m_dev = m_dev; t.A = A; t.lda = lda; t.N = N; t.B = B; t.ldb = ldb; t.K = K; t.partial = partial;
    t.blk_list = geom != 0 ? blk_list : nullptr; t.blk_cnt = blk_cnt; t.blk_stride = blk_stride;
    typedef void (*Kern)(Tn16Args);
    const Kern fn = geom == 1 ? (Kern)gemm16_tn_kernel<true, 2, 7, 4, 5> : geom == 2 ? (Kern)gemm16_tn_kernel<true, 4, 5, 2, 5>
                                                                                     : (Kern)gemm16_tn_kernel<false, 4, 5, 2, 5>;
    const int aw = geom == 1 ? Tn16Add::AW : Tn16Qkv::AW, bw = geom == 1 ? Tn16Add::BW : Tn16Qkv::BW;
    t.splits = splits; t.n_blk = cdiv(N, aw); t.k_blk = cdiv(K, bw);
    const size_t lds = 2 * (size_t)(geom == 1 ? Tn16Add::STAGE : Tn16Qkv::STAGE);
    const hipError_t e = hipFuncSetAttribute((const void*)fn, hipFuncAttributeMaxDynamicSharedMemorySize, (int)lds);
    if (e != hipSuccess) { set_error("%s: hipFuncSetAttribute: %s", name, hipGetErrorString(e)); return NRMS_ELAUNCH; }
    {
        TimingScope ts(name, stream);
        hipLaunchKernelGGL(fn, dim3(splits * t.n_blk * t.k_blk), dim3(T16_THREADS), lds, stream, t);
    }
    int rc = check_launch(name);
    if (rc) return rc;
    TimingScope ts("tn_reduce", stream);
    hipLaunchKernelGGL(tn16_reduce_kernel, dim3(cdiv((long)N * K, 256)), dim3(256), 0, stream, partial, splits, N, K, nmap, kmap,
                       nscale, ldw, dW, dbias);
    return check_launch("tn16_reduce");
}

static size_t bwd16_attn_dma_lds() {
    return (size_t)3 * F16_SLOT_DMA + (size_t)B16_RED * 4 + (size_t)2 * F16_WAVES * 3 * 32 * 4 + (size_t)F16_WAVES * 2048;
}
static_assert(2 * (3 * F16_SLOT_DMA + B16_RED * 4 + 2 * F16_WAVES * 3 * 32 * 4 + F16_WAVES * 2048) <= 160 * 1024, "two workgroups per CU");

size_t bwd16_fused_lds(bool two) {
    static_assert(F16_WAVES * 2 * F16_QT * 32 + 2 * F16_WAVES * 32 >= 2 * F16_WAVES * 3 * 32, "the attention kernel's staging fits the same size");
    return (size_t)3 * F16_SLOT + (size_t)B16_RED * 4 + (size_t)(F16_WAVES * (two ? 2 : 1) * 2 * F16_QT * 32 + 2 * F16_WAVES * 32) * 4;
}

int launch_bwd16_pool(const Bwd16Args& a, int n_wg, bool two, hipStream_t stream) {
    const size_t lds = bwd16_fused_lds(two);
    const void* fp = two ? (const void*)fused_bwd16_pool_kernel<2> : (const void*)fused_bwd16_pool_kernel<1>;
    const hipError_t e = hipFuncSetAttribute(fp, hipFuncAttributeMaxDynamicSharedMemorySize, (int)lds);
    if (e != hipSuccess) { set_error("fused_bwd16: hipFuncSetAttribute: %s", hipGetErrorString(e)); return NRMS_ELAUNCH; }
    TimingScope ts(two ? "fused64_bwd16_pool" : "fused_bwd16_pool", stream);
    if (two) hipLaunchKernelGGL(fused_bwd16_pool_kernel<2>, dim3(n_wg), dim3(F16_THREADS), lds, stream, a);
    else hipLaunchKernelGGL(fused_bwd16_pool_kernel<1>, dim3(n_wg), dim3(F16_THREADS), lds, stream, a);
    return check_launch("fused_bwd16_pool");
}

int launch_dx16(const Dx16Args& g, bool out16, hipStream_t stream) {
    if ((g.d & 3) != 0 || ((uintptr_t)g.c & 15) != 0) { set_error("gemm16_dx: dx must be 16-byte aligned, d %% 4 == 0"); return NRMS_EINVAL; }
    const size_t lds = (size_t)2 * DX_SLOT;
    const void* fn = out16 ? (const void*)gemm16_dx_kernel<true> : (const void*)gemm16_dx_kernel<false>;
    const hipError_t e = hipFuncSetAttribute(fn, hipFuncAttributeMaxDynamicSharedMemorySize, (int)lds);
    if (e != hipSuccess) { set_error("gemm16_dx: hipFuncSetAttribute: %s", hipGetErrorString(e)); return NRMS_ELAUNCH; }
    TimingScope ts("dx_bwd", stream);
    if (out16) hipLaunchKernelGGL(gemm16_dx_kernel<true>, dim3(cdiv(g.M, DX_BM)), dim3(DX_THREADS), lds, stream, g);
    else hipLaunchKernelGGL(gemm16_dx_kernel<false>, dim3(cdiv(g.M, DX_BM)), dim3(DX_THREADS), lds, stream, g);
    return check_launch("gemm16_dx");
}

int launch_dout16(long n_seq, int d, int h, int dk, float fixed_scale, float* sc, const float* dout, _Float16* dout16, hipStream_t stream) {
    unsigned* max_bits = (unsigned*)(sc + 2);
    if (hipMemsetAsync(max_bits, 0, sizeof(unsigned), stream) != hipSuccess) { set_error("fused_bwd16: memset failed"); return NRMS_ELAUNCH; }
    const long nd = n_seq * d;
    if (!(fixed_scale > 0.f))
        hipLaunchKernelGGL(absmax_kernel, dim3(nd > 512L * 1024 ? 512 : (int)cdiv(nd, 1024)), dim3(256), 0, stream, nd, dout, max_bits);
    hipLaunchKernelGGL(dout16_kernel, dim3(cdiv(n_seq * F16_DP, 256) > 4096 ? 4096 : cdiv(n_seq * F16_DP, 256)),
                       dim3(256), 0, stream, n_seq, d, h, dk, fixed_scale, max_bits, sc, dout, dout16);
    return check_launch("dout16");
}

static int launch_dout16_maps(long n_seq, int d, int h, int dk, int q, float fixed_scale, float qscale, float* sc, const float* dout,
                              _Float16* dout16, const Maps16& m, hipStream_t stream) {
    unsigned* max_bits = (unsigned*)(sc + 2);
    const long nd = n_seq * d;
    if (!(fixed_scale > 0.f))
        hipLaunchKernelGGL(absmax_kernel, dim3(nd > 512L * 1024 ? 512 : (int)cdiv(nd, 1024)), dim3(256), 0, stream, nd, dout, max_bits);
    const int row_blocks = cdiv(n_seq * F16_DP, 256) > 4096 ? 4096 : cdiv(n_seq * F16_DP, 256);
    hipLaunchKernelGGL(dout16_maps_kernel, dim3(row_blocks + MAPS16_BLOCKS), dim3(256), 0, stream, n_seq, d, h, dk, q, fixed_scale,
                       qscale, max_bits, sc, dout, dout16, m);
    return check_launch("dout16");
}

int launch_fused_bwd16(const Fused16Bwd& f, hipStream_t stream) {
    if (f.n_seq <= 0) return NRMS_OK;
    const long M = (long)f.n_seq * f.S;
    const Fused16BwdLayout L = fused16_bwd_layout(M, f.n_seq);
    char* base = (char*)f.workspace;
    const int dk = f.d / f.h;
    const float qscale = 1.0f / sqrtf((float)dk);
    _Float16* btiles = (_Float16*)(base + L.btiles);
    _Float16* xtiles = (_Float16*)(base + L.xtiles);
    _Float16* qv16 = (_Float16*)(base + L.qv16);
    float* bqkv32 = (float*)(base + L.bqkv32);
    _Float16* dout16 = (_Float16*)(base + L.dout16);
    _Float16* dz16 = (_Float16*)(base + L.dz16);
    _Float16* dctx16 = (_Float16*)(base + L.dctx16);
    _Float16* dqkv16 = (_Float16*)(base + L.dqkv16);
    float* red = (float*)(base + L.red);
    int* nmap_qkv = (int*)(base + L.maps);
    float* nscale_qkv = (float*)(nmap_qkv + B16_DQ);
    int* kmap_x = (int*)(nscale_qkv + B16_DQ);
    int* nmap_add = kmap_x + F16_KP;
    float* nscale_add = (float*)(nmap_add + F16_QP);
    int* kmap_ctx = (int*)(nscale_add + F16_QP);
    float* sc = (float*)(base + L.scale);
    if (f.sc_out != nullptr) *f.sc_out = sc;
    float* partial_qkv = (float*)(base + L.partial);
    float* partial_add = (float*)(base + L.partial + up256((size_t)L.tn_splits_qkv * B16_DQ * F16_KP * 4));
    { const int jr = fused_bwd16_join(stream, false); if (jr) return jr; }
    SideSet* ss = side_streams_for(stream);
    const bool side = ss != nullptr;
    hipStream_t s_add = side ? ss->s[0] : stream, s_qkv = side ? ss->s[1] : stream;
    SideJoinGuard join_guard(ss, stream);
    const int Mp = f.n_seq * 32 * (f.S > 32 ? 2 : 1);
    const char* staged_env = getenv("NRMS_BWD_ATTN_STAGED");
    const bool attn_dma = f.S <= 32 && !(staged_env != nullptr && atoi(staged_env) != 0);
    {
        Prep16bArgs p{};
        p.d = f.d; p.h = f.h; p.dk = dk; p.q = f.q; p.w_qkv = f.w_qkv; p.b_qkv = f.b_qkv; p.w_add = f.w_add; p.q_vec = f.q_vec;
        p.btiles = btiles; p.xtiles = xtiles; p.qv16 = qv16; p.bqkv32 = bqkv32;
        p.dma_tiles = attn_dma ? 1 : 0;
        p.max_bits = (unsigned*)(sc + 2);
        TimingScope ts("prep16", stream);
        hipLaunchKernelGGL(prep16b_kernel, dim3(2048), dim3(256), 0, stream, p);
        int rc = check_launch("prep16b");
        if (rc) return rc;
        Maps16 mp;
        mp.nmap_qkv = nmap_qkv; mp.nscale_qkv = nscale_qkv; mp.kmap_x = kmap_x; mp.nmap_add = nmap_add; mp.nscale_add = nscale_add;
        mp.kmap_ctx = kmap_ctx;
        rc = launch_dout16_maps((long)f.n_seq, f.d, f.h, dk, f.q, f.loss_scale, qscale, sc, f.dout, dout16, mp, stream);
        if (rc) return rc;
    }
    Bwd16Args a{};
    a.n_seq = f.n_seq; a.S = f.S; a.d = f.d; a.h = f.h; a.dk = dk; a.q = f.q;
    const bool lists = f.order != nullptr && f.S <= 32;
    a.n_groups = cdiv(f.n_seq, F16_WAVES) + (lists ? 2 : 0);
    a.n_cls = lists ? 3 : 2;
    a.x16 = (const _Float16*)f.x16; a.pos = f.pos; a.n_rows = f.n_rows_dev; a.ids = f.ids;
    a.order = lists ? f.order : nullptr; a.order_cnt = lists ? f.order_cnt : nullptr;
    a.btiles = btiles; a.bqkv32 = bqkv32; a.qv16 = qv16;
    a.ctx16 = (const _Float16*)f.ctx16; a.t16 = (const _Float16*)f.t16; a.w = f.w; a.dout16 = dout16;
    a.dz16 = dz16; a.dctx16 = dctx16; a.dqkv16 = dqkv16; a.red = red; a.drop = f.drop;
    a.dbg = 0;
#ifdef NRMS_F16_EXPERIMENTS
    { const char* e = getenv("NRMS_F16_DBG"); a.dbg = e ? atoi(e) : 0; }
#endif
    const int n_wg = a.n_groups < L.n_wg ? a.n_groups : L.n_wg;
    {
        const bool two = f.S > 32;
        const size_t lds = attn_dma ? bwd16_attn_dma_lds() : bwd16_fused_lds(two);
        const void* fa = two ? (const void*)fused_bwd16_attn_kernel<2, false>
                             : attn_dma ? (const void*)fused_bwd16_attn_kernel<1, true> : (const void*)fused_bwd16_attn_kernel<1, false>;
        const hipError_t e = hipFuncSetAttribute(fa, hipFuncAttributeMaxDynamicSharedMemorySize, (int)lds);
        if (e != hipSuccess) { set_error("fused_bwd16: hipFuncSetAttribute: %s", hipGetErrorString(e)); return NRMS_ELAUNCH; }
        {
            const int rcp = launch_bwd16_pool(a, n_wg, two, stream);
            if (rcp) return rcp;
        }
        if (side) {
            int rc = side_order(ss, 0, stream, s_add, "fused_bwd16");
            if (rc) return rc;
            rc = launch_tn16(1, dz16, F16_QP, F16_QP, (const _Float16*)f.ctx16, F16_DP, F16_DP, Mp, nullptr, partial_add,
                             L.tn_splits_add, nmap_add, kmap_ctx, nscale_add, f.d, f.dw_add, s_add, "dwadd_bwd");
            if (rc) return rc;
            if (hipEventRecord(ss->ev[2], s_add) != hipSuccess) { set_error("fused_bwd16: hipEventRecord failed"); return NRMS_ELAUNCH; }
        }
        Bwd16Args b = a;
        b.red = red + (long)n_wg * B16_RED;
        {
            TimingScope ts(two ? "fused64_bwd16_attn" : "fused_bwd16_attn", stream);
            if (two) hipLaunchKernelGGL((fused_bwd16_attn_kernel<2, false>), dim3(n_wg), dim3(F16_THREADS), lds, stream, b);
            else if (attn_dma) hipLaunchKernelGGL((fused_bwd16_attn_kernel<1, true>), dim3(n_wg), dim3(F16_THREADS), lds, stream, b);
            else hipLaunchKernelGGL((fused_bwd16_attn_kernel<1, false>), dim3(n_wg), dim3(F16_THREADS), lds, stream, b);
        }
        int rc = check_launch("fused_bwd16");
        if (rc) return rc;
    }
    int rc = NRMS_OK;
    if (!side) {
        rc = launch_tn16(1, dz16, F16_QP, F16_QP, (const _Float16*)f.ctx16, F16_DP, F16_DP, Mp, nullptr, partial_add,
                         L.tn_splits_add, nmap_add, kmap_ctx, nscale_add, f.d, f.dw_add, stream, "dwadd_bwd");
        if (rc) return rc;
    }
    if (side) {
// ... 45 lines not shown
```

pytorch_news_recommender_amd/csrc/gemm.h:

```cpp
#pragma once
#include "common.h"
#include "rowdiv.h"

namespace nrms {

constexpr int NT_BM = 128;
constexpr int NT_BK = 16;
constexpr int NT_STAGE_A = NT_BM * NT_BK;

enum { A_PLAIN = 0, A_DZ = 2 };
enum { E_STORE = 0, E_DCTX = 1 };

struct NTArgs {
    int M, N, K;
    int rows_per_tile;
    const float* A; int lda;
    const float* ds;
    const float* qv;
    const float* T;
    const float* W;
    const float* bias;
    float* C; int ldc;
    const float* wrow;
    const float* dout;
    RowDiv seq_of_row;
    Dropout drop;
    const int* a_rows;
    const int* m_dev;
    const int* c_rows;
};

__device__ __forceinline__ int nt_swz(int row) { return (0x1230 >> (((row >> 2) & 3) * 4)) & 3; }

template <int NT, int AMODE>
__device__ __forceinline__ void gemm_nt_mainloop(const NTArgs& a, int row0, int rows_valid, int col0,
                                                 f32x4 (&acc)[2][NT], float* lds) {
    constexpr int STAGE = (NT_BM + 16 * NT) * NT_BK;
    constexpr int B_F4 = NT * 16 * 4;
    constexpr int B_IT = (B_F4 + 255) / 256;
    const int tid = threadIdx.x;
    const int lane = tid & 63, wave = tid >> 6;
    const int r16 = lane & 15, kq = lane >> 4;

    const int chunk = tid & 3;
    const float* arow[2];
    float ascale[2];
    bool a_ok[2];
    int a_lds[2];
#pragma unroll
    for (int i = 0; i < 2; ++i) {
        const int r = (tid >> 2) + 64 * i;
        const long g = (long)row0 + min(r, rows_valid - 1);
        a_ok[i] = r < rows_valid;
        a_lds[i] = (r * 4 + (chunk ^ nt_swz(r))) * 4;
        if (AMODE == A_PLAIN) { arow[i] = a.A + (a.a_rows != nullptr ? (long)a.a_rows[g] : g) * a.lda; ascale[i] = 0.f; }
        else { arow[i] = a.T + g * (long)a.K; ascale[i] = a.ds[g]; }
    }
    const float* brow[B_IT];
    bool b_ok[B_IT];
    int b_lds[B_IT];
#pragma unroll
    for (int i = 0; i < B_IT; ++i) {
        const int idx = tid + 256 * i;
        const int r = idx >> 2;
        const int n = col0 + r;
        b_ok[i] = idx < B_F4 && n < a.N;
        brow[i] = a.W + (long)min(n, a.N - 1) * a.K;
        b_lds[i] = idx < B_F4 ? NT_STAGE_A + (r * 4 + (chunk ^ nt_swz(r))) * 4 : -1;
    }
    const int fsw = kq ^ nt_swz(r16);
    const int a_frag0 = ((32 * wave + r16) * 4 + fsw) * 4;
    const int a_frag1 = ((32 * wave + 16 + r16) * 4 + fsw) * 4;
    const int b_frag = NT_STAGE_A + (r16 * 4 + fsw) * 4;

    f32x4 av[2], bv[B_IT], qv4;
    const int k_last = a.K - 4;
    auto load_stage = [&](int k0) {
        const int k = min(k0 + chunk * 4, k_last);
#pragma unroll
        for (int i = 0; i < 2; ++i) av[i] = *reinterpret_cast<const f32x4*>(arow[i] + k);
        if (AMODE == A_DZ) qv4 = *reinterpret_cast<const f32x4*>(a.qv + k);
#pragma unroll
// ... 116 lines not shown
                    f32x4 v = *reinterpret_cast<const f32x4*>(wave_lds + sr * S + 4 * c4a);
                    if (!dropped) v = fix(v, gr, na, bias_a);
                    *reinterpret_cast<f32x4*>(g.C + (g.c_rows != nullptr ? (long)g.c_rows[gr] : gr) * g.ldc + na) = v;
                }
            }
            if (REM > 0) {
                for (int idx = lane; idx < 8 * REM; idx += 64) {
                    int sr, c4, rl, n;
                    if (!rem_pos(idx, rbase, sr, c4, rl, n)) continue;
                    const long gr = (long)row0 + rl;
                    f32x4 v = *reinterpret_cast<const f32x4*>(wave_lds + sr * S + 4 * c4);
                    if (!dropped) {
                        f32x4 b4 = {0.f, 0.f, 0.f, 0.f};
                        if (EMODE == E_STORE && g.bias != nullptr) b4 = *reinterpret_cast<const f32x4*>(g.bias + n);
                        v = fix(v, gr, n, b4);
                    }
                    *reinterpret_cast<f32x4*>(g.C + (g.c_rows != nullptr ? (long)g.c_rows[gr] : gr) * g.ldc + n) = v;
                }
            }
            __builtin_amdgcn_fence(__ATOMIC_RELEASE, "wavefront");
            __builtin_amdgcn_wave_barrier();
            __builtin_amdgcn_fence(__ATOMIC_ACQUIRE, "wavefront");
        }
    }
}

int launch_gemm_nt(int amode, int emode, const NTArgs& a, hipStream_t stream, const char* name);

struct TNArgs {
    int M, N, K;
    int amode;
    const float* A; int lda;
    const float* ds;
    const float* qv;
    const float* T;
    const float* B; int ldb;
    float* dW;
    float* dbias;
    float* partial;
    int splits;
    int rows_per_split;
    HeadPerm perm;
    const int* m_dev;
};
size_t gemm_tn_workspace_floats(int M, int N, int K, int* splits_out);
int launch_gemm_tn(const TNArgs& a, hipStream_t stream, const char* name);

int launch_transpose(const float* in, float* out, int rows, int cols, hipStream_t stream, HeadPerm perm = HeadPerm{0, 0});
int launch_permute_rows(const float* w, const float* b, float* w2, float* b2, int rows, int cols, HeadPerm perm,
                        hipStream_t stream);

int launch_gemm_nt_bf16(int amode, int emode, int npass, const NTArgs& a, void* wplanes, hipStream_t stream,
                        const char* name);
size_t gemm_nt_bf16_wplane_bytes(int N, int K);
int launch_gemm_tn_bf16(int npass, const TNArgs& a, hipStream_t stream, const char* name);

struct AddFwdArgs {
    NTArgs g;
    const float* qv;
    float* T;
    float* wout;
    float* out;
    int S, d;
    const uint8_t* mask;
};
int launch_addattn_fwd_bf16(int npass, const AddFwdArgs& a, void* wplanes, hipStream_t stream);
int launch_colsum_add(const float* partial, int rows, int cols, float* out, hipStream_t stream);

struct Fused16Layout { int KP, DP, QP; size_t wqkv16, wadd16, bqkv32, badd32, qv32, total; };
Fused16Layout fused16_layout(int d, int h, int q);
bool fused16_supported(int S, int d, int h, int q, const char** why);
int launch_prep16(int d, int h, int q, const float* w_qkv, const float* b_qkv, const float* w_add, const float* b_add,
                  const float* q_vec, void* planes, hipStream_t stream);
int launch_gather16(long M, int d, int KP, const int64_t* ids, const int* live, const int* n_live, const float* table,
                    const Dropout& drop, void* x16, hipStream_t stream);
int launch_cast16(long M, int d, int KP, const float* x, void* x16, hipStream_t stream);
struct Fused16Fwd {
    int n_seq, S, d, h, q;
    const void* planes;
    const void* x16;
    const int* pos;
    const int* n_rows;
    const int64_t* ids;
    const int* order;
    const int* order_cnt;
    void* ctx16;
    void* t16;
    float* w;
    float* out;
    Dropout drop;
};
int launch_fused_fwd16(const Fused16Fwd& f, hipStream_t stream);
bool fused16v1_supported(int S, int d, int h, int q, const char** why);
size_t fused16v1_planes_bytes(int d, int h, int q);
int launch_prep16v1(int d, int h, int q, const float* w_qkv, const float* b_qkv, const float* w_o, const float* b_o,
                    const float* w_add, const float* b_add, const float* q_vec, void* planes, hipStream_t stream);
int launch_fused_fwd16v1(const Fused16Fwd& f, int h, void* attn16, hipStream_t stream);
size_t title_order_cnt_ints(int n_seq);
int launch_title_order(int n_seq, int S, const int64_t* ids, int* order, int* cnt, hipStream_t stream, int n_classes = 2);

struct Fused16BwdLayout { int n_wg, tn_splits_qkv, tn_splits_add; size_t btiles, xtiles, qv16, bqkv32, dout16, dz16, dctx16, dqkv16, red, maps, scale, partial, total; };
Fused16BwdLayout fused16_bwd_layout(long M, int n_seq);
struct Fused16Bwd {
    int n_seq, S, d, h, q;
    void* workspace;
    const float* w_qkv; const float* b_qkv; const float* w_add; const float* q_vec;
    const void* x16;
    const int* pos;
    const int* n_rows_dev;
    const int64_t* ids;
    const int* order; const int* order_cnt;
    const void* ctx16; const void* t16; const float* w;
    const float* dout;
    float loss_scale;
    Dropout drop;
    float* dw_qkv; float* db_qkv; float* dw_add; float* db_add; float* dq_vec;
    float* dx;
    bool dx_fp16;
    const float** sc_out;
    bool defer_join;
    const float* w_o; const void* attn16; float* dw_o; float* db_o;
};
int launch_fused_bwd16(const Fused16Bwd& f, hipStream_t stream);
size_t fused16v1_bwd_bytes(long M, int n_seq, int h);
int launch_fused_bwd16v1(const Fused16Bwd& f, hipStream_t stream);
int fused_bwd16_join(hipStream_t stream, bool user = true);

bool user64_supported(int S, int d, int h, int q, const char** why);
size_t user64_qkv_bytes(int n_seq, int h);
size_t user64_fwd_planes_bytes(int h);
size_t user64_bwd_planes_bytes(int h);
size_t user64_dq_partial_floats(int n_seq);
int launch_user64_fwd(int n_seq, int S, int d, int h, int q, const float* x, const float* w_qkv, const float* b_qkv,
                      const float* w_add, const float* b_add, const float* q_vec, void* planes, float* ctx, float* t, float* w,
                      void* qkv, float* out, bool train, hipStream_t stream);
int launch_user64_bwd(int n_seq, int S, int d, int h, int q, const float* w_add, const float* q_vec, void* planes, const float* dout,
                      const float* t, const float* w, const void* qkv, float* ds, float* dq_partial, float* dq_vec, float* dqkv,
                      hipStream_t stream);

int launch_sanitize_ids(long n, const void* src, bool src_is_int32, int64_t* dst, int vocab, int* n_bad, hipStream_t stream);
int launch_title_dedup(long n, int L, const int64_t* ids, int* table, long table_size, int* inverse, int* rep_rows,
                       int* n_unique, hipStream_t stream);
int launch_gather_dropout(long M, int d, const int64_t* ids, const float* table, const Dropout& drop, float* x,
                          hipStream_t stream);
int launch_gather_dropout_compact(long M, int d, const int64_t* ids, const int* live, const int* n_live,
                                  const float* table, const Dropout& drop, float* x, hipStream_t stream);
int launch_fill_pad_rows(long n_seq, int S, int n, const int64_t* ids, const float* row, float* out, bool skip_all_pad,
                         hipStream_t stream);
size_t compact_scratch_ints(long M);
int launch_compact_live_rows(long M, const int64_t* ids, int* live, int* pos, int* n_live, int* scratch,
                             hipStream_t stream);
size_t scatter_grouped_scratch_ints(long M, int V);
int launch_scatter_grouped(long M, int V, int d, const int64_t* ids, const int* live, const int* n_live, const void* dx,
                           const Dropout& drop, float* dtable, int* scratch, hipStream_t stream, bool dx_fp16 = false, int ldx = 0,
                           const float* sc = nullptr, bool prepared = false);
struct TableAdam {
    float *p, *m, *v;
    AdamConsts c;
    float gscale;
    int* n_bad;
};
int launch_scatter_grouped_adam(long M, int V, int d, const int64_t* ids, const int* live, const int* n_live, const void* dx,
                                const Dropout& drop, float* dtable, int* scratch, hipStream_t stream, bool dx_fp16, int ldx,
                                const float* sc, bool prepared, const TableAdam& a);
int launch_scatter_prepare(long M, int V, const int64_t* ids, const int* live, const int* n_live, int* scratch, hipStream_t stream);
int launch_scatter_dense_rows(long M, int d, const int64_t* ids, const int* live, const int* n_live, const float* dx,
                              const Dropout& drop, float* dtable, hipStream_t stream);
int launch_scatter_dropout_compact(long M, int d, const int64_t* ids, const int* live, const int* n_live, const float* dx,
                                   const Dropout& drop, float* dtable, hipStream_t stream);

}
```

pytorch_news_recommender_amd/csrc/gemm_bf16.hip:

```cpp
#include <stdlib.h>

#include <atomic>

#include "gemm.h"

namespace nrms {

typedef __bf16 bf16x8 __attribute__((ext_vector_type(8)));

constexpr int BF_BM = 256;
constexpr int BF_BK = 32;
constexpr int BF_THREADS = 512;
constexpr int BF_ROWB = 64;

struct Split8 { bf16x8 hi, lo; };

__device__ __forceinline__ Split8 split8(const f32x4& u, const f32x4& v) {
    Split8 s;
#pragma unroll
    for (int i = 0; i < 4; ++i) {
        const __bf16 h0 = (__bf16)u[i], h1 = (__bf16)v[i];
        s.hi[i] = h0; s.hi[4 + i] = h1;
        s.lo[i] = (__bf16)(u[i] - (float)h0);
        s.lo[4 + i] = (__bf16)(v[i] - (float)h1);
// ... 225 lines not shown
    TimingScope ts(name, stream);
    hipLaunchKernelGGL((gemm_nt_bf16_kernel<NT, AMODE, EMODE, NPASS>), grid, dim3(BF_THREADS), lds_bytes, stream, a);
    return check_launch(name);
}

static int cu_count() {
    static std::atomic<int> cached{0};
    int n = cached.load(std::memory_order_relaxed);
    if (n > 0) return n;
    int dev = 0;
    hipDeviceProp_t prop;
    if (hipGetDevice(&dev) != hipSuccess || hipGetDeviceProperties(&prop, dev) != hipSuccess || prop.multiProcessorCount <= 0) {
        (void)hipGetLastError();
        return 256;
    }
    cached.store(prop.multiProcessorCount, std::memory_order_relaxed);
    return prop.multiProcessorCount;
}

template <int AMODE, int EMODE, int NPASS>
static int launch_bf_mode(const BFArgs& a, hipStream_t stream, const char* name) {
    const int N = a.g.N;
    const int cand[6] = {19, 15, 13, 10, 8, 4};
    int nt = 19;
    long best = -1;
    for (int i = 0; i < 6; ++i) {
        if (cand[i] < 8 && N > 128) continue;
        const long pad = (long)cdiv(N, cand[i] * 16) * cand[i] * 16;
        if (best < 0 || pad < best) { best = pad; nt = cand[i]; }
    }
    const long row_tiles = cdiv(a.g.M, a.g.rows_per_tile);
    const int n_cu = cu_count();
    if (2 * row_tiles * cdiv(N, nt * 16) <= n_cu && getenv("NRMS_NT_WIDE_TILES") == nullptr) {
        const int blocks0 = cdiv(N, nt * 16);
        long best2 = -1;
        for (int i = 0; i < 6; ++i) {
            if (cand[i] < 8) continue;
            const int blocks = cdiv(N, cand[i] * 16);
            if (blocks <= blocks0 || row_tiles * blocks > n_cu) continue;
            const long pad = (long)blocks * cand[i] * 16;
            if (best2 < 0 || pad < best2) { best2 = pad; nt = cand[i]; }
        }
    }
    switch (nt) {
        case 19: return launch_bf_inst<19, AMODE, EMODE, NPASS>(a, stream, name);
        case 15: return launch_bf_inst<15, AMODE, EMODE, NPASS>(a, stream, name);
        case 13: return launch_bf_inst<13, AMODE, EMODE, NPASS>(a, stream, name);
        case 10: return launch_bf_inst<10, AMODE, EMODE, NPASS>(a, stream, name);
        case 8: return launch_bf_inst<8, AMODE, EMODE, NPASS>(a, stream, name);
        default: return launch_bf_inst<4, AMODE, EMODE, NPASS>(a, stream, name);
    }
}

int launch_gemm_nt_bf16(int amode, int emode, int npass, const NTArgs& g_in, void* wplanes, hipStream_t stream,
                        const char* name) {
    if (g_in.M <= 0) return NRMS_OK;
    if ((g_in.K & 3) != 0) { set_error("%s: K=%d must be a multiple of 4", name, g_in.K); return NRMS_EINVAL; }
    BFArgs a;
    a.g = g_in;
    a.g.rows_per_tile = BF_BM;
    a.Kp = cdiv(g_in.K, BF_BK) * BF_BK;
    a.Np = cdiv(g_in.N, 16) * 16;
    a.whi = (const __bf16*)wplanes;
    a.wlo = a.whi + (long)a.Np * a.Kp;
    int rc = launch_split_planes(g_in.W, g_in.N, a.Np, g_in.K, a.Kp, wplanes, (void*)a.wlo, stream);
    if (rc) return rc;
    if (npass == 3) {
        if (amode == A_PLAIN && emode == E_STORE) return launch_bf_mode<A_PLAIN, E_STORE, 3>(a, stream, name);
        if (amode == A_DZ && emode == E_DCTX) return launch_bf_mode<A_DZ, E_DCTX, 3>(a, stream, name);
        if (amode == A_DZ && emode == E_STORE) return launch_bf_mode<A_DZ, E_STORE, 3>(a, stream, name);
    } else {
        if (amode == A_PLAIN && emode == E_STORE) return launch_bf_mode<A_PLAIN, E_STORE, 1>(a, stream, name);
        if (amode == A_DZ && emode == E_DCTX) return launch_bf_mode<A_DZ, E_DCTX, 1>(a, stream, name);
        if (amode == A_DZ && emode == E_STORE) return launch_bf_mode<A_DZ, E_STORE, 1>(a, stream, name);
    }
    set_error("%s: unsupported bf16 gemm mode %d/%d", name, amode, emode);
    return NRMS_EINVAL;
}

template <int NT, int NPASS>
__global__ __launch_bounds__(BF_THREADS, 2) void addattn_fwd_bf16_kernel(AddFwdArgs a, BFArgs b) {
    extern __shared__ __attribute__((aligned(16))) char smem[];
    __shared__ float sc[BF_BM];
    const NTArgs& g = b.g;
    const int row0 = blockIdx.x * g.rows_per_tile;
    const int rows_valid = min(g.rows_per_tile, g.M - row0);
    f32x4 acc[2][NT];
#pragma unroll
    for (int mt = 0; mt < 2; ++mt)
#pragma unroll
        for (int nt = 0; nt < NT; ++nt) acc[mt][nt] = f32x4{0.f, 0.f, 0.f, 0.f};
    bf16_nt_mainloop<NT, A_PLAIN, NPASS>(b, row0, rows_valid, 0, acc, smem);

    const int tid = threadIdx.x, lane = tid & 63;
    const int wave = __builtin_amdgcn_readfirstlane(tid >> 6);
    const int r16 = lane & 15, kq = lane >> 4;
    float bcol[NT], qcol[NT];
#pragma unroll
    for (int nt = 0; nt < NT; ++nt) {
        const int n = 16 * nt + r16;
        const bool ok = n < g.N;
        bcol[nt] = ok ? g.bias[n] : 0.f;
        qcol[nt] = ok ? a.qv[n] : 0.f;
    }
#pragma unroll
    for (int mt = 0; mt < 2; ++mt)
#pragma unroll
        for (int reg = 0; reg < 4; ++reg) {
            float part = 0.f;
#pragma unroll
            for (int nt = 0; nt < NT; ++nt) {
                const float t = fast_tanh(acc[mt][nt][reg] + bcol[nt]);
                part += t * qcol[nt];
                acc[mt][nt][reg] = t;
            }
            part += __shfl_xor(part, 1, 64);
            part += __shfl_xor(part, 2, 64);
            part += __shfl_xor(part, 4, 64);
            part += __shfl_xor(part, 8, 64);
// ... 383 lines not shown
```

pytorch_news_recommender_amd/csrc/pool.hip:

```cpp
#include "gemm.h"

namespace nrms {

template <int NT>
__global__ __launch_bounds__(256, 2) void addattn_fwd_kernel(AddFwdArgs a) {
    __shared__ __attribute__((aligned(16))) float lds[2 * (NT_BM + 16 * NT) * NT_BK];
    __shared__ float sc[NT_BM];

    const NTArgs& g = a.g;
    const int row0 = blockIdx.x * g.rows_per_tile;
    const int rows_valid = min(g.rows_per_tile, g.M - row0);
    f32x4 acc[2][NT];
#pragma unroll
    for (int mt = 0; mt < 2; ++mt)
#pragma unroll
        for (int nt = 0; nt < NT; ++nt) acc[mt][nt] = f32x4{0.f, 0.f, 0.f, 0.f};
    gemm_nt_mainloop<NT, A_PLAIN>(g, row0, rows_valid, 0, acc, lds);

    const int tid = threadIdx.x, lane = tid & 63;
    const int wave = __builtin_amdgcn_readfirstlane(tid >> 6);
    const int r16 = lane & 15, kq = lane >> 4;
    float bcol[NT], qcol[NT];
#pragma unroll
    for (int nt = 0; nt < NT; ++nt) {
        const int n = 16 * nt + r16;
        const bool ok = n < g.N;
        bcol[nt] = ok ? g.bias[n] : 0.f;
        qcol[nt] = ok ? a.qv[n] : 0.f;
    }
#pragma unroll
    for (int mt = 0; mt < 2; ++mt)
#pragma unroll
        for (int reg = 0; reg < 4; ++reg) {
            const int rl = 32 * wave + 16 * mt + 4 * kq + reg;
            float part = 0.f;
#pragma unroll
            for (int nt = 0; nt < NT; ++nt) {
                const float t = tanhf(acc[mt][nt][reg] + bcol[nt]);
                part += t * qcol[nt];
                acc[mt][nt][reg] = t;
            }
            part += __shfl_xor(part, 1, 64);
            part += __shfl_xor(part, 2, 64);
            part += __shfl_xor(part, 4, 64);
            part += __shfl_xor(part, 8, 64);
            if (r16 == 0) sc[rl] = part;
        }
    if (a.T != nullptr) {
        static_assert(4 * 8 * (16 * NT + 8) <= 2 * (NT_BM + 16 * NT) * NT_BK, "epilogue strips must fit the stage buffers");
        __syncthreads();
        NTArgs tg = g;
        tg.bias = nullptr; tg.C = a.T; tg.ldc = g.N;
        nt_epilogue<NT, E_STORE>(tg, acc, row0, rows_valid, 0, wave, lane, lds + wave * 8 * (16 * NT + 8));
// ... 170 lines not shown

int launch_colsum_add(const float* partial, int rows, int cols, float* out, hipStream_t stream) {
    TimingScope ts("colsum_add", stream);
    hipLaunchKernelGGL(colsum_add_kernel, dim3(cdiv(cols, 16)), dim3(1024), 0, stream, partial, rows, cols, out);
    return check_launch("colsum_add");
}

__global__ void click_fwd_kernel(int B, int C, int d, const float* cand, const float* user, const uint8_t* mask,
                                 float* scores) {
    const int lane = threadIdx.x & 63;
    const long u = (long)blockIdx.x * (blockDim.x >> 6) + (threadIdx.x >> 6);
    if (u >= (long)B * C) return;
    const long b = u / C;
    const float* cv = cand + u * d;
    const float* uv = user + b * d;
    float p = 0.f;
    for (int k = lane; k < d; k += 64) p += cv[k] * uv[k];
    p = wave_sum(p);
    if (lane == 0) scores[u] = (mask != nullptr && mask[u] == 0) ? -1e9f : p;
}

__global__ void click_indexed_kernel(int B, int C, int d, const float* vec, long n_vec, const int* index, const float* user,
                                     const uint8_t* mask, float* scores) {
    const int lane = threadIdx.x & 63;
    const long u = (long)blockIdx.x * (blockDim.x >> 6) + (threadIdx.x >> 6);
    if (u >= (long)B * C) return;
    const long b = u / C;
    const long r = index[u];
    const bool ok = r >= 0 && r < n_vec;
    const float* cv = vec + (ok ? r : 0) * d;
    const float* uv = user + b * d;
    float p = 0.f;
    for (int k = lane; k < d; k += 64) p += cv[k] * uv[k];
    p = wave_sum(p);
    if (lane == 0) scores[u] = (mask != nullptr && mask[u] == 0) ? -1e9f : (ok ? p : __builtin_nanf(""));
}

__global__ void click_bwd_kernel(int B, int C, int d, const float* cand, const float* user, const uint8_t* mask,
                                 const float* dscores, float* dcand, float* duser) {
    const int b = blockIdx.x;
    for (int k = threadIdx.x; k < d; k += blockDim.x) {
        const float uv = user[(long)b * d + k];
        float du = 0.f;
        for (int c = 0; c < C; ++c) {
            const long u = (long)b * C + c;
            const float g = (mask != nullptr && mask[u] == 0) ? 0.f : dscores[u];
            dcand[u * d + k] = g * uv;
            du += g * cand[u * d + k];
        }
        duser[(long)b * d + k] = du;
    }
}

__global__ void ce_loss_kernel(int B, int C, const float* scores, float* loss_sum, float* dscores, float gscale) {
    __shared__ float red[256];
    float local = 0.f;
    for (int b = threadIdx.x; b < B; b += blockDim.x) {
        const float* s = scores + (long)b * C;
        float mx = -3.0e38f;
        for (int c = 0; c < C; ++c) mx = fmaxf(mx, s[c]);
        double sum = 0.0;
        for (int c0 = 0; c0 < C; c0 += 16) {
            const int c1 = c0 + 16 < C ? c0 + 16 : C;
            float run = 0.f;
            for (int c = c0; c < c1; ++c) run += expf(s[c] - mx);
            sum += (double)run;
        }
        local += (float)(((double)mx - (double)s[0]) + log(sum));
        if (dscores != nullptr) {
            const float inv = (float)(1.0 / sum);
            for (int c = 0; c < C; ++c) {
                const float e = expf(s[c] - mx);
                const float p = (c == 0) ? __builtin_fmaf(e, inv, -1.0f) : e * inv;
                dscores[(long)b * C + c] = p * gscale;
            }
        }
    }
    red[threadIdx.x] = local;
    __syncthreads();
    for (int o = 128; o > 0; o >>= 1) {
        if ((int)threadIdx.x < o) red[threadIdx.x] += red[threadIdx.x + o];
        __syncthreads();
    }
    if (threadIdx.x == 0) loss_sum[0] += red[0];
}

template <bool GUARD>
__global__ void adam_kernel(size_t n4, size_t n, float* p, const float* g, float* m, float* v, float step_size,
                            float b1, float b2, float omb1, float omb2, float inv_sqrt_bc2, float eps, float gscale, int* n_bad) {
    const size_t stride = (size_t)gridDim.x * blockDim.x;
    int bad = 0;
    for (size_t i = (size_t)blockIdx.x * blockDim.x + threadIdx.x; i < n4; i += stride) {
        f32x4 pv = reinterpret_cast<f32x4*>(p)[i];
        const f32x4 gv = reinterpret_cast<const f32x4*>(g)[i] * gscale;
        f32x4 mv = reinterpret_cast<f32x4*>(m)[i];
        f32x4 vv = reinterpret_cast<f32x4*>(v)[i];
#pragma unroll
        for (int e = 0; e < 4; ++e) {
            if (GUARD && (__float_as_uint(gv[e]) & 0x7F800000u) == 0x7F800000u) { ++bad; continue; }
            float pe = pv[e], me = mv[e], ve = vv[e];
            adam_update(pe, me, ve, gv[e], step_size, b1, b2, omb1, omb2, inv_sqrt_bc2, eps);
            pv[e] = pe; mv[e] = me; vv[e] = ve;
        }
        reinterpret_cast<f32x4*>(p)[i] = pv;
        reinterpret_cast<f32x4*>(m)[i] = mv;
        reinterpret_cast<f32x4*>(v)[i] = vv;
    }
    const size_t t = n4 * 4 + (size_t)blockIdx.x * blockDim.x + threadIdx.x;
    if (t < n) {
        const float gv = g[t] * gscale;
        if (GUARD && (__float_as_uint(gv) & 0x7F800000u) == 0x7F800000u) {
            ++bad;
        } else {
            float pe = p[t], me = m[t], ve = v[t];
            adam_update(pe, me, ve, gv, step_size, b1, b2, omb1, omb2, inv_sqrt_bc2, eps);
            p[t] = pe; m[t] = me; v[t] = ve;
        }
    }
    if (GUARD) {
#pragma unroll
        for (int o = 32; o > 0; o >>= 1) bad += __shfl_xor(bad, o, 64);
        if (bad != 0 && (threadIdx.x & 63) == 0) atomicAdd(n_bad, bad);
    }
}

__global__ void grad_guard_kernel(size_t n, float* g, int* n_bad) {
    const size_t stride = (size_t)gridDim.x * blockDim.x;
    int bad = 0;
    const size_t n4 = ((reinterpret_cast<uintptr_t>(g) & 15) == 0) ? n / 4 : 0;
    for (size_t i = (size_t)blockIdx.x * blockDim.x + threadIdx.x; i < n4; i += stride) {
        f32x4 gv = reinterpret_cast<f32x4*>(g)[i];
        int b = 0;
#pragma unroll
        for (int e = 0; e < 4; ++e)
            if ((__float_as_uint(gv[e]) & 0x7F800000u) == 0x7F800000u) { gv[e] = 0.f; ++b; }
        if (b) { reinterpret_cast<f32x4*>(g)[i] = gv; bad += b; }
    }
// ... 64 lines not shown

extern "C" int nrms_impression_auc(int32_t n_imp, int32_t max_c, const float* scores, const uint8_t* labels,
                                   const int32_t* lens, double* auc, void* stream) {
    NRMS_REQUIRE(n_imp >= 0 && max_c > 0 && scores && labels && lens && auc, "impression_auc: bad arguments");
    if (n_imp == 0) return NRMS_OK;
    hipStream_t s = (hipStream_t)stream;
    TimingScope ts("impression_auc", s);
    hipLaunchKernelGGL(impression_auc_kernel, dim3(cdiv(n_imp, 4)), dim3(256), 0, s, n_imp, max_c, scores, labels, lens, auc);
    return check_launch("impression_auc");
}

extern "C" int nrms_click_score_fwd(int32_t B, int32_t C, int32_t d, const float* cand, const float* user,
                                    const uint8_t* mask, float* scores, void* stream) {
    NRMS_REQUIRE(B >= 0 && C > 0 && d > 0 && cand && user && scores, "click_score_fwd: bad arguments");
    if (B == 0) return NRMS_OK;
    hipStream_t s = (hipStream_t)stream;
    TimingScope ts("click_fwd", s);
    hipLaunchKernelGGL(click_fwd_kernel, dim3(cdiv((long)B * C, 4)), dim3(256), 0, s, B, C, d, cand, user, mask, scores);
    return check_launch("click_fwd");
}

extern "C" int nrms_click_score_indexed(int32_t B, int32_t C, int32_t d, const float* news_vec, int64_t n_vec, const int32_t* index,
                                        const float* user, const uint8_t* mask, float* scores, void* stream) {
    NRMS_REQUIRE(B >= 0 && C > 0 && d > 0 && n_vec > 0 && news_vec && index && user && scores, "click_score_indexed: bad arguments");
    if (B == 0) return NRMS_OK;
    hipStream_t s = (hipStream_t)stream;
    TimingScope ts("click_fwd", s);
    hipLaunchKernelGGL(click_indexed_kernel, dim3(cdiv((long)B * C, 4)), dim3(256), 0, s, B, C, d, news_vec, (long)n_vec, index,
                       user, mask, scores);
    return check_launch("click_indexed");
}

extern "C" int nrms_click_score_bwd(int32_t B, int32_t C, int32_t d, const float* cand, const float* user,
                                    const uint8_t* mask, const float* dscores, float* dcand, float* duser,
                                    void* stream) {
    NRMS_REQUIRE(B >= 0 && C > 0 && d > 0 && cand && user && dscores && dcand && duser, "click_score_bwd: bad arguments");
    if (B == 0) return NRMS_OK;
    hipStream_t s = (hipStream_t)stream;
    TimingScope ts("click_bwd", s);
    hipLaunchKernelGGL(click_bwd_kernel, dim3(B), dim3(128), 0, s, B, C, d, cand, user, mask, dscores, dcand, duser);
    return check_launch("click_bwd");
}

extern "C" int nrms_ce_loss_fwd_bwd(int32_t B, int32_t C, const float* scores, float* loss_sum, float* dscores,
                                    float grad_scale, void* stream) {
    NRMS_REQUIRE(B >= 0 && C > 0 && scores && loss_sum, "ce_loss: bad arguments");
    if (B == 0) return NRMS_OK;
    hipStream_t s = (hipStream_t)stream;
    TimingScope ts("ce_loss", s);
    hipLaunchKernelGGL(ce_loss_kernel, dim3(1), dim3(256), 0, s, B, C, scores, loss_sum, dscores, grad_scale);
    return check_launch("ce_loss");
}

namespace nrms {
AdamConsts adam_consts(double lr, double beta1, double beta2, double eps, int32_t step) {
    const double bc1 = 1.0 - pow(beta1, (double)step);
    const double bc2 = 1.0 - pow(beta2, (double)step);
    AdamConsts c;
    c.step_size = (float)(lr / bc1);
    c.b1 = (float)beta1; c.b2 = (float)beta2; c.omb1 = (float)(1.0 - beta1); c.omb2 = (float)(1.0 - beta2);
    c.inv_sqrt_bc2 = (float)(1.0 / sqrt(bc2));
    c.eps = (float)eps;
    return c;
}
}

static int adam_step(size_t n, float* param, const float* grad, float* exp_avg, float* exp_avg_sq, double lr, double beta1,
                     double beta2, double eps, int32_t step, float grad_scale, int32_t* n_nonfinite, void* stream,
                     const char* timer = "adam") {
    NRMS_REQUIRE(param && grad && exp_avg && exp_avg_sq && step >= 1, "adam_step: bad arguments");
    NRMS_REQUIRE((((uintptr_t)param | (uintptr_t)grad | (uintptr_t)exp_avg | (uintptr_t)exp_avg_sq) & 15) == 0,
                 "adam_step: buffers must be 16-byte aligned");
    if (n == 0) return NRMS_OK;
    const AdamConsts c = adam_consts(lr, beta1, beta2, eps, step);
    hipStream_t s = (hipStream_t)stream;
    const size_t n4 = n / 4;
    int blocks = (int)((n4 + 255) / 256);
    if (blocks > 256 * 8) blocks = 256 * 8;
    if (blocks < 1) blocks = 1;
    TimingScope ts(timer, s);
    if (n_nonfinite != nullptr)
        hipLaunchKernelGGL(adam_kernel<true>, dim3(blocks), dim3(256), 0, s, n4, n, param, grad, exp_avg, exp_avg_sq, c.step_size,
                           c.b1, c.b2, c.omb1, c.omb2, c.inv_sqrt_bc2, c.eps, grad_scale, (int*)n_nonfinite);
    else
        hipLaunchKernelGGL(adam_kernel<false>, dim3(blocks), dim3(256), 0, s, n4, n, param, grad, exp_avg, exp_avg_sq, c.step_size,
                           c.b1, c.b2, c.omb1, c.omb2, c.inv_sqrt_bc2, c.eps, grad_scale, (int*)nullptr);
    return check_launch("adam");
}

extern "C" int nrms_adam_step_rest(size_t n, float* param, const float* grad, float* exp_avg, float* exp_avg_sq, double lr,
                                   double beta1, double beta2, double eps, int32_t step, float grad_scale, int32_t* n_nonfinite,
                                   void* stream) {
    return adam_step(n, param, grad, exp_avg, exp_avg_sq, lr, beta1, beta2, eps, step, grad_scale, n_nonfinite, stream, "rest_adam");
}

extern "C" int nrms_adam_step(size_t n, float* param, const float* grad, float* exp_avg, float* exp_avg_sq, double lr,
                              double beta1, double beta2, double eps, int32_t step, float grad_scale, void* stream) {
    return adam_step(n, param, grad, exp_avg, exp_avg_sq, lr, beta1, beta2, eps, step, grad_scale, nullptr, stream);
}

extern "C" int nrms_adam_step_guarded(size_t n, float* param, const float* grad, float* exp_avg, float* exp_avg_sq, double lr,
                                      double beta1, double beta2, double eps, int32_t step, float grad_scale,
                                      int32_t* n_nonfinite, void* stream) {
    NRMS_REQUIRE(n_nonfinite != nullptr, "adam_step_guarded: null counter");
    return adam_step(n, param, grad, exp_avg, exp_avg_sq, lr, beta1, beta2, eps, step, grad_scale, n_nonfinite, stream);
}
// ... 30 lines not shown
```

pytorch_news_recommender_amd/csrc/user64.hip:

```cpp
#include "gemm.h"

namespace nrms {

typedef __bf16 b8 __attribute__((ext_vector_type(8)));
struct B2 { b8 hi, lo; };

#define U64_DI __device__ __forceinline__
#ifdef NRMS_U64_EXPERIMENTS
#include <stdlib.h>
#define U64_DBG(flags, bit) ((flags) & (bit))
#else
#define U64_DBG(flags, bit) 0
#endif

U64_DI f32x16 mfb(const b8& a, const b8& b, const f32x16& c) { return __builtin_amdgcn_mfma_f32_32x32x16_bf16(a, b, c, 0, 0, 0); }
U64_DI void mma3(f32x16& acc, const B2& a, const B2& b) {
    acc = mfb(a.lo, b.hi, acc);
    acc = mfb(a.hi, b.lo, acc);
    acc = mfb(a.hi, b.hi, acc);
}
U64_DI f32x16 zero16u() {
    f32x16 r;
#pragma unroll
    for (int i = 0; i < 16; ++i) r[i] = 0.f;
// ... 725 lines not shown

size_t user64_qkv_bytes(int n_seq, int h) {
    return (size_t)n_seq * h * 2 * 12 * 1024 + (size_t)n_seq * 2 * U_CS * 2048;
}
static size_t user64_ctxf_offset(int n_seq, int h) { return (size_t)n_seq * h * 2 * 12 * 1024; }

size_t user64_fwd_planes_bytes(int h) { return (size_t)(3 * h + U_QT) * U_TILE + 2 * U_QP * 4; }
size_t user64_bwd_planes_bytes(int h) { return (size_t)h * U_BTILE + U_QP * 4; }

int launch_user64_fwd(int n_seq, int S, int d, int h, int q, const float* x, const float* w_qkv, const float* b_qkv,
                      const float* w_add, const float* b_add, const float* q_vec, void* planes, float* ctx, float* t, float* w,
                      void* qkv, float* out, bool train, hipStream_t stream) {
    if (n_seq <= 0) return NRMS_OK;
    char* pb = (char*)planes;
    U64PrepArgs p{};
    p.d = d; p.h = h; p.dk = d / h; p.q = q; p.w_qkv = w_qkv; p.b_qkv = b_qkv; p.w_add = w_add; p.b_add = b_add; p.q_vec = q_vec;
    p.wtiles = (__bf16*)pb; p.addv = (float*)(pb + (size_t)(3 * h + U_QT) * U_TILE);
    {
        TimingScope ts("user64_prep", stream);
        hipLaunchKernelGGL(user64_prep_kernel, dim3(1024), dim3(256), 0, stream, p);
    }
    U64FwdArgs a{};
    a.n_seq = n_seq; a.S = S; a.d = d; a.h = h; a.dk = d / h; a.q = q;
    a.x = x; a.wtiles = pb; a.addv = p.addv; a.ctx = ctx; a.t = t; a.w = w;
    a.qkvf = train ? (b8*)qkv : nullptr;
    a.ctxf = (b8*)((char*)qkv + user64_ctxf_offset(n_seq, h));
    a.out = out;
    a.dbg = 0;
    a.stamps = nullptr;
#ifdef NRMS_U64_EXPERIMENTS
    { const char* e = getenv("NRMS_U64_DBG"); a.dbg = e ? atoi(e) : 0; }
    static unsigned long long* g_stamps = nullptr;
    if (g_stamps == nullptr) (void)hipHostMalloc((void**)&g_stamps, 64 * sizeof(unsigned long long));
    a.stamps = g_stamps;
    if (g_stamps != nullptr && getenv("NRMS_U64_STAMPS") != nullptr) {
        (void)hipStreamSynchronize(stream);
        fprintf(stderr, "[shader clock over the head loop: %.0f MHz]\n", (double)(g_stamps[32 + 2] - g_stamps[32 + 1]) / ((g_stamps[2] - g_stamps[1]) * 0.01));
        fprintf(stderr, "[user64_fwd stamps, us] prologue %.2f | tile0 %.2f | head1 (Q..V barrier %.2f, attention+stores %.2f) | heads total %.2f | zero+reload %.2f | additive %.2f | softmax+pool %.2f\n",
                (g_stamps[1] - g_stamps[0]) * 0.01, 0.0, (g_stamps[8] - g_stamps[6]) * 0.01, (g_stamps[7] - g_stamps[8]) * 0.01,
                (g_stamps[2] - g_stamps[1]) * 0.01, (g_stamps[3] - g_stamps[2]) * 0.01, (g_stamps[4] - g_stamps[3]) * 0.01, (g_stamps[5] - g_stamps[4]) * 0.01);
    }
#endif
    const void* fn = train ? (const void*)user64_fwd_kernel<true> : (const void*)user64_fwd_kernel<false>;
    const hipError_t e = hipFuncSetAttribute(fn, hipFuncAttributeMaxDynamicSharedMemorySize, U_FWD_LDS);
    if (e != hipSuccess) { set_error("user64_fwd: hipFuncSetAttribute: %s", hipGetErrorString(e)); return NRMS_ELAUNCH; }
    TimingScope ts("user64_fwd", stream);
    const dim3 grid(cdiv(n_seq, 2));
    if (train) hipLaunchKernelGGL(user64_fwd_kernel<true>, grid, dim3(U_THREADS), U_FWD_LDS, stream, a);
    else hipLaunchKernelGGL(user64_fwd_kernel<false>, grid, dim3(U_THREADS), U_FWD_LDS, stream, a);
    return check_launch("user64_fwd");
}

size_t user64_dq_partial_floats(int n_seq) { return (size_t)cdiv(n_seq > 0 ? n_seq : 1, 2) * U_QP; }
int launch_user64_bwd(int n_seq, int S, int d, int h, int q, const float* w_add, const float* q_vec, void* planes, const float* dout,
                      const float* t, const float* w, const void* qkv, float* ds, float* dq_partial, float* dq_vec, float* dqkv,
                      hipStream_t stream) {
    if (n_seq <= 0) return NRMS_OK;
    char* pb = (char*)planes;
    U64PrepArgs p{};
    p.d = d; p.h = h; p.dk = d / h; p.q = q; p.w_add = w_add; p.q_vec = q_vec;
    p.btiles = (__bf16*)pb; p.qv = (float*)(pb + (size_t)h * U_BTILE);
    {
        TimingScope ts("user64_prep", stream);
        hipLaunchKernelGGL(user64_prep_kernel, dim3(512), dim3(256), 0, stream, p);
    }
    U64BwdArgs a{};
    a.n_seq = n_seq; a.S = S; a.d = d; a.h = h; a.dk = d / h; a.q = q; a.qscale = 1.0f / sqrtf((float)(d / h));
    a.btiles = pb; a.qv = p.qv; a.dout = dout; a.t = t; a.w = w;
    a.qkvf = (const b8*)qkv; a.ctxf = (const b8*)((const char*)qkv + user64_ctxf_offset(n_seq, h));
    a.ds = ds; a.dq_partial = dq_partial; a.dqkv = dqkv;
    const hipError_t e = hipFuncSetAttribute((const void*)user64_bwd_kernel, hipFuncAttributeMaxDynamicSharedMemorySize, U_BWD_LDS);
    if (e != hipSuccess) { set_error("user64_bwd: hipFuncSetAttribute: %s", hipGetErrorString(e)); return NRMS_ELAUNCH; }
    const int n_wg = cdiv(n_seq, 2);
    {
        TimingScope ts("user64_bwd", stream);
        hipLaunchKernelGGL(user64_bwd_kernel, dim3(n_wg), dim3(U_THREADS), U_BWD_LDS, stream, a);
    }
    int rc = check_launch("user64_bwd");
    if (rc) return rc;
    return launch_colsum_add(dq_partial, n_wg, q, dq_vec, stream);
}

}
```

pytorch_news_recommender_amd/engine.py:

```python
from __future__ import annotations

import ctypes as C
import math
import os
from dataclasses import dataclass

import torch

from . import _lib
from .synth import ENCODERS


@dataclass(frozen=True)
class ModelDims:
    n_words: int
    word_embed_size: int
    num_attention_heads: int
    query_vector_dim: int
    news_heads: int = 0
    output_proj: bool = False
    style: str = "v0"

    def heads(self, enc):
        return self.news_heads if (enc == "news_encoder" and self.news_heads) else self.num_attention_heads
# ... 193 lines not shown
        return self._ptrs(_lib.EncoderWeights, flat, enc)

    def _grads(self, gflat, enc):
        return self._ptrs(_lib.EncoderGrads, gflat, enc)

    def _acts(self, tag, M, need_bwd, gather=False, desc=None):
        d, q = self.dims.word_embed_size, self.dims.query_vector_dim
        if desc is not None and desc.precision == _lib.NRMS_PRECISION_FP16:
            KP, DP, QP = _lib.NRMS_FP16_KP, _lib.NRMS_FP16_DP, _lib.NRMS_FP16_QP
            h = torch.float16
            x = self._buf(tag + ".x16", (M + 1) * KP, h)
            Mp = desc.n_seq * (32 if desc.seq_len <= 32 else 64)
            ctx = self._buf(tag + ".ctx16", Mp * DP, h)
            t = self._buf(tag + ".t16", Mp * QP, h) if need_bwd else None
            w = self._buf(tag + ".w", M) if need_bwd else None
            nbytes = int(self.lib.nrms_encoder_fwd_scratch_bytes(C.byref(desc)))
            scratch = self._buf(tag + ".scratch16", (nbytes + 3) // 4)
            attn = self._buf(tag + ".attn16", Mp * DP, h) if desc.use_output_proj else None
            dp = lambda z: None if z is None else z.data_ptr()
            return _lib.EncoderActs(x=dp(x), qkv=None, attn=dp(attn), ctx=dp(ctx), t=dp(t), w=dp(w), scratch=dp(scratch))
        x = self._buf(tag + ".x", M * d) if gather else None
        if desc is not None and desc.flags & _lib.NRMS_FLAG_FUSED_SEQ64:
            nb = int(self.lib.nrms_encoder_fused_qkv_bytes(C.byref(desc)))
            qkv = self._buf(tag + ".qkvf", (nb + 3) // 4)
            ctx = self._buf(tag + ".ctx", M * d) if need_bwd else None
            t = self._buf(tag + ".t", M * q) if need_bwd else None
            w = self._buf(tag + ".w", M) if need_bwd else None
            ns = int(self.lib.nrms_encoder_fwd_scratch_bytes(C.byref(desc)))
            scratch = self._buf("fwd_scratch64", (ns + 3) // 4)
            dp = lambda z: None if z is None else z.data_ptr()
            return _lib.EncoderActs(x=None, qkv=dp(qkv), attn=None, ctx=dp(ctx), t=dp(t), w=dp(w), scratch=dp(scratch))
        qkv = self._buf(tag + ".qkv", M * 3 * d)
        attn = self._buf(tag + ".attn", M * d) if self.dims.output_proj else None
        ctx = self._buf(tag + ".ctx", M * d)
        t = self._buf(tag + ".t", M * q) if need_bwd else None
        w = self._buf(tag + ".w", M) if need_bwd else None
        scratch = self._buf("fwd_scratch", 3 * d * d + 3 * d + 256 + (3 * d + 32) * (d + 32) + (M + M // 1024 + 512 if gather else 0))
        dp = lambda z: None if z is None else z.data_ptr()
        return _lib.EncoderActs(x=dp(x), qkv=dp(qkv), attn=dp(attn), ctx=dp(ctx), t=dp(t), w=dp(w), scratch=dp(scratch))

    def sanitize_ids(self, src, dst):
        n = src.numel()
        if n == 0:
            return dst
        fn = self.lib.nrms_sanitize_ids_i32 if src.dtype == torch.int32 else self.lib.nrms_sanitize_ids
        rc = fn(_lib.ptr(src), _lib.ptr(dst), C.c_int64(n), int(self.dims.n_words), _lib.ptr(self._bad_ids), _stream())
        _lib.check(rc, "nrms_sanitize_ids")
        self._bad_host.copy_(self._bad_ids, non_blocking=True)
        ev = torch.cuda.Event()
        ev.record()
        self._bad_event = ev
        return dst

    def note_bad_ids(self):
        self._bad_host.copy_(self._bad_ids, non_blocking=True)
        ev = torch.cuda.Event()
        ev.record()
        self._bad_event = ev

    def _raise_bad_ids(self):
        n = int(self._bad_host.item())
        if n:
            self._bad_ids.zero_()
            self._bad_host.zero_()
            raise _lib.NrmsError("%d word id(s) outside [0, %d) reached the embedding gather (treated as the padding "
                                 "id on the device; the vocabulary and the embedding table disagree)" % (n, self.dims.n_words))

    def poll_ids(self):
        if self._bad_event is not None and self._bad_event.query():
            self._bad_event = None
            self._raise_bad_ids()

    def check_ids(self):
        if self._bad_event is not None:
            self._bad_event.synchronize()
            self._bad_event = None
        self._raise_bad_ids()

    def encode_titles(self, flat, ids, out=None, p_embed=0.0, p_ctx=0.0, seed=0, save=False, tag=None,
                      chunk_titles=32768, mask=None, mask_mode=0, trusted_ids=False):
        N, L = ids.shape
        d = self.dims.word_embed_size
        if tag is None:
            tag = "news" if save else "news_eval"
        if out is None:
            out = torch.empty(N, d, dtype=torch.float32, device=self.device)
        if trusted_ids:
            ids = ids.contiguous()
        else:
            self.poll_ids()
            ids = self.sanitize_ids(ids.contiguous(), self._buf(tag + ".ids", N * L, torch.int64)[:N * L].view(N, L))
        if mask is not None:
            mask = mask.contiguous()
        w = self._weights(flat, "news_encoder")
        step = N if save else min(N, chunk_titles)
        for s0 in range(0, N, max(step, 1)):
            n = min(step, N - s0)
            desc = self._desc("news_encoder", n, L, p_embed, p_ctx, seed, mask_mode if mask is not None else 0, training=save)
            acts = self._acts(tag, n * L, save, gather=True, desc=desc)
            mp = None if mask is None else C.c_void_p(mask[s0:].data_ptr())
            rc = self.lib.nrms_encoder_fwd(C.byref(desc), C.byref(w), C.c_void_p(ids[s0:].data_ptr()), None, mp,
                                           C.byref(acts), C.c_void_p(out[s0:].data_ptr()), _stream())
            _lib.check(rc, "nrms_encoder_fwd(news)")
        return out

    def encode_users(self, flat, news_vectors, out=None, save=False, tag=None, mask=None, mask_mode=0):
        B, H, d = news_vectors.shape
        if tag is None:
            tag = "user" if save else "user_eval"
        if out is None:
            out = torch.empty(B, d, dtype=torch.float32, device=self.device)
        w = self._weights(flat, "user_encoder")
        desc = self._desc("user_encoder", B, H, mask_mode=mask_mode if mask is not None else 0, training=save)
        acts = self._acts(tag, B * H, save, desc=desc)
        rc = self.lib.nrms_encoder_fwd(C.byref(desc), C.byref(w), None, C.c_void_p(news_vectors.data_ptr()),
                                       _lib.ptr(None if mask is None else mask.contiguous()), C.byref(acts),
                                       C.c_void_p(out.data_ptr()), _stream())
        _lib.check(rc, "nrms_encoder_fwd(user)")
        return out

    def _parts_of(self, tag, B, H, d):
        M = B * H
        return self._bufs[tag + ".ctx"][:M * d].view(B, H, d).clone(), self._bufs[tag + ".w"][:M].view(B, H).clone()

    def user_parts(self, flat, news_vectors, mask=None, mask_mode=0):
        B, H, d = news_vectors.shape
        tag = "user_parts"
        out = torch.empty(B, d, dtype=torch.float32, device=self.device)
        wts = self._weights(flat, "user_encoder")
        desc = self._desc("user_encoder", B, H, mask_mode=mask_mode if mask is not None else 0, training=False)
        if desc.precision == _lib.NRMS_PRECISION_FP16:
            desc.precision = _lib.PRECISIONS["bf16x3"]
        acts = self._acts(tag, B * H, True, desc=desc)
        rc = self.lib.nrms_encoder_fwd(C.byref(desc), C.byref(wts), None, C.c_void_p(news_vectors.data_ptr()),
                                       _lib.ptr(None if mask is None else mask.contiguous()), C.byref(acts),
                                       C.c_void_p(out.data_ptr()), _stream())
        _lib.check(rc, "nrms_encoder_fwd(user parts)")
        return (out,) + self._parts_of(tag, B, H, d)

    def click_scores(self, cand_vec, user_vec, cand_mask=None, out=None):
        B, Cn, d = cand_vec.shape
        if out is None:
            out = torch.empty(B, Cn, dtype=torch.float32, device=self.device)
        rc = self.lib.nrms_click_score_fwd(B, Cn, d, _lib.ptr(cand_vec), _lib.ptr(user_vec), _lib.ptr(cand_mask),
                                           _lib.ptr(out), _stream())
        _lib.check(rc, "nrms_click_score_fwd")
        return out

    def forward(self, flat, hist_ids, cand_ids, cand_mask, training, p_drop=0.0, seed=0, user_mask=None,
                user_mask_mode=0):
        B, H, L = hist_ids.shape
        Cn = cand_ids.shape[1]
        d = self.dims.word_embed_size
        N = B * (H + Cn)
        sfx = "" if training else "_eval"
        self.poll_ids()
        ids = self._buf("ids" + sfx, N * L, torch.int64)[:N * L].view(N, L)
        self.sanitize_ids(hist_ids.reshape(B * H, L).contiguous(), ids[:B * H])
        self.sanitize_ids(cand_ids.reshape(B * Cn, L).contiguous(), ids[B * H:])
        nv = self._buf("news_vec" + sfx, N * d)[:N * d].view(N, d)
        p = float(p_drop)
        p_embed = 0.0 if self.dims.style == "v1" else p
        self.encode_titles(flat, ids, out=nv, p_embed=p_embed, p_ctx=p, seed=seed, save=training, tag="news" + sfx,
                           trusted_ids=True)
        hist = nv[:B * H].view(B, H, d)
        cand = nv[B * H:].view(B, Cn, d)
        user = self._buf("user_vec" + sfx, B * d)[:B * d].view(B, d)
        self.encode_users(flat, hist, out=user, save=training, tag="user" + sfx, mask=user_mask, mask_mode=user_mask_mode)
        if cand_mask is not None:
            cand_mask = cand_mask.contiguous()
        scores = torch.empty(B, Cn, dtype=torch.float32, device=self.device)
        self.click_scores(cand, user, cand_mask, out=scores)
        if training:
            self._gen += 1
            self._saved = dict(B=B, H=H, C=Cn, L=L, ids=ids, nv=nv, user=user, mask=cand_mask, p=p, p_embed=p_embed,
                               seed=seed, user_mask=user_mask, user_mask_mode=user_mask_mode if user_mask is not None else 0,
                               gen=self._gen)
        return scores

    def ce_loss(self, scores, grad_scale=None, want_grad=True):
        B, Cn = scores.shape
        loss_sum = torch.zeros(1, dtype=torch.float32, device=self.device)
        dscores = torch.empty_like(scores) if want_grad else None
        gs = (1.0 / B) if grad_scale is None else grad_scale
        rc = self.lib.nrms_ce_loss_fwd_bwd(B, Cn, _lib.ptr(scores), _lib.ptr(loss_sum), _lib.ptr(dscores),
                                           C.c_float(gs), _stream())
        _lib.check(rc, "nrms_ce_loss_fwd_bwd")
        return loss_sum, dscores

    def _bwd_workspace(self, *descs):
        nbytes = max(self.lib.nrms_encoder_bwd_workspace_bytes(C.byref(d)) for d in descs)
        return self._buf("bwd_ws", (nbytes + 3) // 4)

    def encode_users_backward(self, flat, gflat, news_vectors, dout, dx=None, tag="user", mask=None, mask_mode=0,
                              defer_join=False):
        B, H, d = news_vectors.shape
        if dx is None:
            dx = torch.empty(B * H, d, dtype=torch.float32, device=self.device)
        desc = self._desc("user_encoder", B, H, mask_mode=mask_mode if mask is not None else 0, training=True)
        if defer_join and desc.precision != _lib.NRMS_PRECISION_FP16:
            desc.flags |= _lib.NRMS_FLAG_DEFER_USER_JOIN
            nbytes = self.lib.nrms_encoder_bwd_workspace_bytes(C.byref(desc))
            ws = self._buf("bwd_ws_user", (nbytes + 3) // 4)
        else:
            ws = self._bwd_workspace(desc)
        w, g = self._weights(flat, "user_encoder"), self._grads(gflat, "user_encoder")
        acts = self._acts(tag, B * H, True, desc=desc)
        rc = self.lib.nrms_encoder_bwd(C.byref(desc), C.byref(w), None, _lib.ptr(news_vectors),
                                       _lib.ptr(None if mask is None else mask.contiguous()), C.byref(acts),
                                       _lib.ptr(dout.contiguous()), C.byref(g), _lib.ptr(dx), _lib.ptr(ws),
                                       C.c_size_t(ws.numel() * 4), _stream())
        _lib.check(rc, "nrms_encoder_bwd(user)")
        return dx[:B * H].view(B, H, d)

    def join_backward(self):
        _lib.check(self.lib.nrms_encoder_join(_stream()), "nrms_encoder_join")

    POOLED_VEC = ("nv", "d_news_vec")

    def _head_buffers(self, sv, width):
        B, H, Cn = sv["B"], sv["H"], sv["C"]
        N = B * (H + Cn)
        key, dkey = self.POOLED_VEC
        dvec = self._buf(dkey, N * width)[:N * width].view(N, width)
        duser = self._buf("d_user_vec", B * width)[:B * width].view(B, width)
        return sv[key][B * H:], sv["user"], dvec, duser

    def _head_backward(self, dscores, gen, width):
        sv = self._saved
        if sv is None:
            raise _lib.NrmsError("backward() without a training forward()")
        if gen is not None and gen != sv["gen"]:
            raise _lib.NrmsError("backward() for training forward #%d, but the saved activations belong to forward #%d: "
                                 "a later training forward replaced them (one forward/backward pair at a time)" % (gen, sv["gen"]))
        B, H, Cn = sv["B"], sv["H"], sv["C"]
        cand, user, dvec, duser = self._head_buffers(sv, width)
        if dscores is None:
            if getattr(self, "_pooled_gen", None) != sv["gen"]:
                raise _lib.NrmsError("backward(dscores=None) needs the gradients of pooled_ce_loss(), and none was computed for "
                                     "training forward #%d" % sv["gen"])
        else:
            rc = self.lib.nrms_click_score_bwd(B, Cn, width, _lib.ptr(cand), _lib.ptr(user), _lib.ptr(sv["mask"]),
                                               _lib.ptr(dscores.contiguous()), C.c_void_p(dvec[B * H:].data_ptr()), _lib.ptr(duser),
                                               _stream())
            _lib.check(rc, "nrms_click_score_bwd")
        return sv, dvec, duser

    def pooled_ce_loss(self, cand_ids, reject=None, col_bias=None, grad_scale=None, want_grad=True):
        sv = self._saved
        if sv is None:
            raise _lib.NrmsError("pooled_ce_loss() without a training forward()")
        B, Cn = sv["B"], sv["C"]
        key, _ = self.POOLED_VEC
        width = sv[key].shape[1]
        cand, user, dvec, duser = self._head_buffers(sv, width)
        dev = self.device
        ids = torch.as_tensor(cand_ids).to(dev, torch.int64).contiguous()
        if ids.numel() != B * Cn:
            raise _lib.NrmsError("pooled_ce_loss: cand_ids must be [%d, %d] (got %s)" % (B, Cn, tuple(ids.shape)))
        R = 0
        if reject is not None:
            reject = torch.as_tensor(reject).to(dev, torch.int64).contiguous()
            if reject.dim() != 2 or reject.shape[0] != B:
                raise _lib.NrmsError("pooled_ce_loss: reject must be [%d, R] (got %s)" % (B, tuple(reject.shape)))
            R = reject.shape[1]
            if R == 0:
                reject = None
        if col_bias is not None:
            col_bias = torch.as_tensor(col_bias).to(dev, torch.float32).contiguous()
            if col_bias.numel() != B * Cn:
                raise _lib.NrmsError("pooled_ce_loss: col_bias must be [%d, %d] (got %s)" % (B, Cn, tuple(col_bias.shape)))
        nbytes = self.lib.nrms_pooled_ce_workspace_bytes(B, Cn, width, R)
        if nbytes == 0:
            raise _lib.NrmsError("pooled_ce_loss: arguments rejected (B=%d, C=%d, d=%d, R=%d; B <= 4096, C <= 64, B*C <= 32768, "
                                 "d <= 1024, R <= 256)" % (B, Cn, width, R))
        ws = self._buf("pooled_ce_ws", (nbytes + 3) // 4)
        loss_sum = torch.zeros(1, dtype=torch.float32, device=dev)
        self.pooled_pairs = torch.zeros(1, dtype=torch.int64, device=dev)
        gs = (1.0 / B) if grad_scale is None else grad_scale
        H = sv["H"]
        rc = self.lib.nrms_pooled_ce_fwd_bwd(B, Cn, width, R, _lib.ptr(cand), _lib.ptr(user), _lib.ptr(ids), _lib.ptr(sv["mask"]),
                                             _lib.ptr(reject), _lib.ptr(col_bias), C.c_float(gs), _lib.ptr(loss_sum),
                                             C.c_void_p(dvec[B * H:].data_ptr()) if want_grad else None,
                                             _lib.ptr(duser) if want_grad else None, _lib.ptr(self.pooled_pairs), _lib.ptr(ws),
                                             C.c_size_t(ws.numel() * 4), _stream())
        _lib.check(rc, "nrms_pooled_ce_fwd_bwd")
        if want_grad:
            self._pooled_gen = sv["gen"]
        return loss_sum

    single_table_scatter = True

    def __init_subclass__(cls, **kw):
# ... 710 lines not shown
```

pytorch_news_recommender_amd/model/_flat_model.py:

```python
from __future__ import annotations

import os

import torch
import torch.nn as nn

from .. import _lib
from ..engine import nrms_entries


def news_encoder_entries(dims, extra):
    return [e for e in nrms_entries(dims) if e[2] == "news_encoder"] + [(name, shape, None, None) for name, shape in extra]


def additive_entries(prefix, q, d):
    return [(prefix + ".linear.weight", (q, d)), (prefix + ".linear.bias", (q,)), (prefix + ".attention_query_vector", (q,))]


class _FlatFunction(torch.autograd.Function):

    @staticmethod
    def forward(ctx, model, args, p_drop, seed, *params):
        ctx.model = model
        scores = model._engine.forward(model._flat, *args, training=True, p_drop=p_drop, seed=seed)
        ctx.gen = model._engine._saved["gen"]
        return scores

    @staticmethod
    def backward(ctx, dscores):
        model = ctx.model
        reuse = bool(getattr(model, "reuse_grad_buffer", False)) and not any(p.grad is not None for p in model.parameters())
        gflat = model._autograd_grad if reuse else None
        if gflat is None or gflat.shape != model._flat.shape or gflat.device != model._flat.device:
            gflat = torch.empty_like(model._flat)
            if reuse:
                model._autograd_grad = gflat
        gflat.zero_()
        model._backward(gflat, dscores, gen=ctx.gen)
        if model._engine.precision == "fp16":
            model._engine.grad_guard(gflat)
            model._engine.note_grad_check()
        return (None, None, None, None) + tuple(model._layout.view(gflat, n) for n in model._names)


class FlatHipModel(nn.Module):
    KEYS = ()
    OPTIONAL = ("candidate_mask",)

    def _finish(self, layout, device):
        self._layout = layout
        self._names = layout.names
        named = dict(self.named_parameters())
        assert sorted(named) == sorted(self._names), sorted(set(named) ^ set(self._names))
        self._flat = self._engine = self._opt = None
        self._pad_zero = None
        self._calls = self._prepare_calls = 0
        self._autograd_grad = None
        self.reuse_grad_buffer = False
        self._flatten(device)
        self.register_load_state_dict_post_hook(FlatHipModel._reset_pad_flag)

# ... 68 lines not shown
        for k in self.KEYS:
            v = batch.get(k) if hasattr(batch, "get") else batch[k]
            if v is None:
                if k in self.OPTIONAL:
                    continue
                raise KeyError("%s: the batch dict lacks %r" % (type(self).__module__, k))
            out[k] = torch.as_tensor(v).to(dev, non_blocking=True)
        return (out,)

    def _infer(self, batch, args, p_drop, seed):
        return self._engine.forward(self._flat, *args, training=False, p_drop=p_drop, seed=seed)

    TRAIN_LOSSES = ("rowwise", "pooled")

    def _train_loss(self):
        name = getattr(self.config, "train_loss", "rowwise")
        if name not in self.TRAIN_LOSSES:
            raise ValueError("config.train_loss must be one of %s (got %r)" % (self.TRAIN_LOSSES, name))
        return name

    def _pooled_loss(self, batch, grad_scale):
        get = batch.get if hasattr(batch, "get") else (lambda k: batch[k] if k in batch else None)
        ids = get("candidate_ids")
        if ids is None:
            raise KeyError("%s: config.train_loss = 'pooled' needs the batch key 'candidate_ids' (the news id of every candidate "
                           "slot)" % type(self).__module__)
        logq = get("candidate_logq") if getattr(self.config, "logq_correction", True) else None
        dev = self._flat.device
        bias = None if logq is None else -torch.as_tensor(logq).to(dev, torch.float32)
        return self._engine.pooled_ce_loss(ids, reject=get("browsed_ids"), col_bias=bias, grad_scale=grad_scale)

    def forward(self, batch):
        dev = self._prepare()
        args = self._engine_args(batch, dev)
        p_drop = float(self.config.dropout) if self.training else 0.0
        seed = self._next_seed() if p_drop > 0 else 0
        named = dict(self.named_parameters())
        params = [named[n] for n in self._names]
        if torch.is_grad_enabled() and any(p.requires_grad for p in params):
            return _FlatFunction.apply(self, args, p_drop, seed, *params)
        return self._infer(batch, args, p_drop, seed)

    def train_step(self, batch, lr=None, betas=(0.9, 0.999), eps=1e-8, world_size=1, all_reduce=None, global_batch=None):
        dev = self._prepare()
        eng = self._engine
        pooled = self._train_loss() == "pooled"
        args = self._engine_args(batch, dev)
        if self._opt is None:
            self._opt = dict(step=0, g=torch.zeros_like(self._flat), m=torch.zeros_like(self._flat),
                             v=torch.zeros_like(self._flat))
        st = self._opt
        p_drop = float(self.config.dropout) if self.training else 0.0
        seed = self._next_seed() if p_drop > 0 else 0
        scores = eng.forward(self._flat, *args, training=True, p_drop=p_drop, seed=seed)
        gb = scores.shape[0] * world_size if global_batch is None else global_batch
        if pooled:
            loss_sum, dscores = self._pooled_loss(batch, 1.0 / gb), None
        else:
            loss_sum, dscores = eng.ce_loss(scores, grad_scale=1.0 / gb)
        lr_ = float(self.config.learning_rate if lr is None else lr)
        if self._fuses_table_adam(world_size, all_reduce):
            n_table = self._layout.entries[self._names[0]][2]
            st["g"][n_table:].zero_()
            self._backward(st["g"], dscores, table_adam=dict(m=st["m"], v=st["v"], step=st["step"] + 1, lr=lr_, betas=betas, eps=eps))
            st["step"] += 1
            eng.adam_step(self._flat[n_table:], st["g"][n_table:], st["m"][n_table:], st["v"][n_table:], st["step"], lr=lr_,
                          betas=betas, eps=eps, rest=True)
            if eng.precision == "fp16":
                eng.note_grad_check()
            self._last_scores = scores
            return loss_sum
        st["g"].zero_()
        overlap = not os.environ.get("NRMS_NO_OVERLAP")
        if all_reduce is not None and hasattr(all_reduce, "owned"):
            pending = []
            if overlap:
                self._backward(st["g"], dscores, table_grad_ready=lambda: pending.append(all_reduce.start(st["g"], 0)))
            else:
                self._backward(st["g"], dscores)
                pending.append(all_reduce.start(st["g"], 0))
            pending.append(all_reduce.start(st["g"], 1))
            for h in pending:
                h.wait()
            st["step"] += 1
            for lo, hi, gshard in all_reduce.owned():
                eng.adam_step(self._flat[lo:hi], gshard, st["m"][lo:hi], st["v"][lo:hi], st["step"], lr=lr_, betas=betas, eps=eps)
            if eng.precision == "fp16":
                eng.note_grad_check()
            all_reduce.gather(self._flat)
            self._last_scores = scores
            return loss_sum
        if all_reduce is not None and hasattr(all_reduce, "start") and overlap:
            n_table = self._layout.entries[self._names[0]][2]
            pending = []
            self._backward(st["g"], dscores, table_grad_ready=lambda: pending.append(all_reduce.start(st["g"][:n_table])))
            all_reduce(st["g"][n_table:])
            for h in pending:
                h.wait()
        else:
            self._backward(st["g"], dscores)
            if all_reduce is not None:
                all_reduce(st["g"])
        st["step"] += 1
        eng.adam_step(self._flat, st["g"], st["m"], st["v"], st["step"], lr=lr_, betas=betas, eps=eps)
        if eng.precision == "fp16":
            eng.note_grad_check()
        self._last_scores = scores
        return loss_sum

    @property
    def engine(self):
        self._prepare()
# ... 2 lines not shown
```

Before: 177,000 users/s.

## Fuse click-score/CE head, merge id sanitization, and overlap backward prep on side streams

Bundles several changes. The click-score forward, CE loss and score backward are fused into a single click_ce_step launch for the train step, and the two id-sanitize launches become one kernel. The fp16 backward-plane prep and the w_qkv transpose/plane prep run on a side stream so they overlap the user-encoder backward, and the dq column-sum moves to the second stream. The absmax reduction is split into per-block row maxima to drop the atomic. Together these aim to cut launch count and serial dependencies, at the cost of more event synchronisation and environment-gated code paths.

```diff
diff --git a/include/nrms_hip.h b/include/nrms_hip.h
--- a/include/nrms_hip.h
+++ b/include/nrms_hip.h
@@ -87,6 +87,7 @@
                      const nrms_encoder_acts* acts, float* out, void* stream);
 
 size_t nrms_encoder_bwd_workspace_bytes(const nrms_encoder_desc* desc);
+size_t nrms_encoder_bwd_scale_offset(const nrms_encoder_desc* desc);
 int nrms_encoder_bwd(const nrms_encoder_desc* desc, const nrms_encoder_weights* w,
                      const int64_t* ids, const float* x, const uint8_t* mask,
                      const nrms_encoder_acts* acts, const float* dout,
@@ -113,6 +114,10 @@
 
 int nrms_sanitize_ids(const int64_t* src, int64_t* dst, int64_t n, int32_t vocab, int32_t* n_bad, void* stream);
 int nrms_sanitize_ids_i32(const int32_t* src, int64_t* dst, int64_t n, int32_t vocab, int32_t* n_bad, void* stream);
+int nrms_sanitize_ids2(const int64_t* src0, int64_t n0, const int64_t* src1, int64_t n1, int64_t* dst, int32_t vocab,
+                       int32_t* n_bad, void* stream);
+int nrms_sanitize_ids2_i32(const int32_t* src0, int64_t n0, const int32_t* src1, int64_t n1, int64_t* dst, int32_t vocab,
+                           int32_t* n_bad, void* stream);
 
 int nrms_title_dedup(const int64_t* ids, int64_t n_titles, int32_t seq_len, int32_t* table, int64_t table_size,
                      int32_t* inverse, int32_t* rep_rows, int32_t* n_unique, void* stream);
@@ -127,6 +132,11 @@
 
 int nrms_ce_loss_fwd_bwd(int32_t B, int32_t C, const float* scores, float* loss_sum,
                          float* dscores, float grad_scale, void* stream);
+
+size_t nrms_click_ce_step_workspace_bytes(int32_t B);
+int nrms_click_ce_step(int32_t B, int32_t C, int32_t d, const float* cand, const float* user, const uint8_t* mask,
+                       float grad_scale, float* scores, float* dscores, float* loss_sum, float* dcand, float* duser,
+                       void* workspace, size_t workspace_bytes, void* stream);
 
 int nrms_adam_step(size_t n, float* param, const float* grad, float* exp_avg, float* exp_avg_sq,
                    double lr, double beta1, double beta2, double eps, int32_t step, float grad_scale,
diff --git a/pytorch_news_recommender_amd/_lib.py b/pytorch_news_recommender_amd/_lib.py
--- a/pytorch_news_recommender_amd/_lib.py
+++ b/pytorch_news_recommender_amd/_lib.py
@@ -96,6 +96,12 @@
     "nrms_encoder_join": (C.c_int, [C.c_void_p]),
     "nrms_sanitize_ids": (C.c_int, [C.c_void_p, C.c_void_p, C.c_int64, C.c_int32, C.c_void_p, C.c_void_p]),
     "nrms_sanitize_ids_i32": (C.c_int, [C.c_void_p, C.c_void_p, C.c_int64, C.c_int32, C.c_void_p, C.c_void_p]),
+    "nrms_encoder_bwd_scale_offset": (C.c_size_t, [C.POINTER(EncoderDesc)]),
+    "nrms_sanitize_ids2": (C.c_int, [C.c_void_p, C.c_int64, C.c_void_p, C.c_int64, C.c_void_p, C.c_int32, C.c_void_p, C.c_void_p]),
+    "nrms_sanitize_ids2_i32": (C.c_int, [C.c_void_p, C.c_int64, C.c_void_p, C.c_int64, C.c_void_p, C.c_int32, C.c_void_p, C.c_void_p]),
+    "nrms_click_ce_step_workspace_bytes": (C.c_size_t, [C.c_int32]),
+    "nrms_click_ce_step": (C.c_int, [C.c_int32, C.c_int32, C.c_int32, C.c_void_p, C.c_void_p, C.c_void_p, C.c_float, C.c_void_p,
+                                     C.c_void_p, C.c_void_p, C.c_void_p, C.c_void_p, C.c_void_p, C.c_size_t, C.c_void_p]),
     "nrms_title_dedup": (C.c_int, [C.c_void_p, C.c_int64, C.c_int32, C.c_void_p, C.c_int64, C.c_void_p, C.c_void_p,
                                    C.c_void_p, C.c_void_p]),
     "nrms_click_score_indexed": (C.c_int, [C.c_int32, C.c_int32, C.c_int32, C.c_void_p, C.c_int64, C.c_void_p, C.c_void_p,
diff --git a/pytorch_news_recommender_amd/csrc/capi.hip b/pytorch_news_recommender_amd/csrc/capi.hip
--- a/pytorch_news_recommender_amd/csrc/capi.hip
+++ b/pytorch_news_recommender_amd/csrc/capi.hip
@@ -444,6 +444,18 @@
     if (ss_prep != nullptr) {
         rc = side_order(ss_prep, 5, s, ss_prep->s[1], "encoder_bwd(fp16)");
         if (rc) return rc;
+        if (!v1 && !fused_bwd16_serial_scale_chain()) {
+            rc = launch_fused_bwd16_planes(f, ss_prep->s[1]);
+            if (rc == NRMS_OK && hipEventRecord(ss_prep->ev[SIDE_EV_PLANES], ss_prep->s[1]) != hipSuccess) {
+                set_error("encoder_bwd(fp16): hipEventRecord failed");
+                rc = NRMS_ELAUNCH;
+            }
+            if (rc) {
+                if (hipEventRecord(ss_prep->ev[4], ss_prep->s[1]) == hipSuccess) (void)hipStreamWaitEvent(s, ss_prep->ev[4], 0);
+                return rc;
+            }
+            f.planes_ready = ss_prep->ev[SIDE_EV_PLANES];
+        }
         rc = launch_scatter_prepare(M, desc->vocab, ids, live, n_live, (int*)(base + L.sscr), ss_prep->s[1]);
         if (hipEventRecord(ss_prep->ev[4], ss_prep->s[1]) != hipSuccess) { set_error("encoder_bwd(fp16): hipEventRecord failed"); return NRMS_ELAUNCH; }
         if (rc) { (void)hipStreamWaitEvent(s, ss_prep->ev[4], 0); return rc; }
@@ -601,6 +613,12 @@
     return bwd_layout(desc).total;
 }
 
+extern "C" size_t nrms_encoder_bwd_scale_offset(const nrms_encoder_desc* desc) {
+    if (validate_desc(desc, "encoder_bwd_scale_offset") || desc->precision != NRMS_PRECISION_FP16 || desc->use_output_proj)
+        return (size_t)-1;
+    return bwd16_layout(desc).fused + fused16_bwd_layout((long)desc->n_seq * desc->seq_len, desc->n_seq).scale;
+}
+
 namespace nrms {
 struct SideEntry { int device; hipStream_t caller; SideSet* set; };
 static std::mutex g_side_mu;
@@ -743,7 +761,28 @@
     };
 
     const bool fused64 = (desc->flags & NRMS_FLAG_FUSED_SEQ64) != 0;
-    if (fused64) {
+    const HeadPerm perm{d / desc->n_heads, desc->n_heads};
+    const char* serial_prep_env = getenv("NRMS_SERIAL_USER_PREP");
+    const bool prep_aside = fused64 && side && !(serial_prep_env != nullptr && atoi(serial_prep_env) != 0);
+    NTArgs gx{};
+    gx.M = M; gx.N = d; gx.K = 3 * d; gx.rows_per_tile = NT_BM;
+    gx.A = dqkv; gx.lda = 3 * d; gx.W = wqkv_t;
+    if (prep_aside) {
+        hipStream_t s3 = ss->s[1];
+        rc = side_order(ss, 1, s, s3, "encoder_bwd");
+        if (rc) return rc;
+        rc = launch_transpose(w->w_qkv, wqkv_t, 3 * d, d, s3, perm);
+        if (rc) return rc;
+        rc = launch_gemm_nt_bf16_planes(gx, wplanes, s3);
+        if (rc) return rc;
+        gx.w_planes_ready = true;
+        if (hipEventRecord(ss->ev[5], s3) != hipSuccess) { set_error("encoder_bwd: hipEventRecord failed"); return NRMS_ELAUNCH; }
+        rc = launch_user64_bwd_planes(d, desc->n_heads, q, w->w_add, w->q_vec, base + L.u64planes, s);
+        if (rc) return rc;
+        rc = launch_user64_bwd_kernel(desc->n_seq, S, d, desc->n_heads, q, base + L.u64planes, dout, acts->t, acts->w, acts->qkv, ds,
+                                      dq_partial, dqkv, s);
+        if (rc) return rc;
+    } else if (fused64) {
         rc = launch_user64_bwd(desc->n_seq, S, d, desc->n_heads, q, w->w_add, w->q_vec, base + L.u64planes, dout, acts->t, acts->w,
                                acts->qkv, ds, dq_partial, grads->q_vec, dqkv, s);
         if (rc) return rc;
@@ -765,6 +804,10 @@
         t.dW = grads->w_add; t.dbias = grads->b_add; t.partial = tn_partial;
         rc = tn_gemm(desc, t, s2, "dwadd_bwd");
         if (rc) return rc;
+        if (prep_aside) {
+            rc = launch_user64_bwd_dq(desc->n_seq, q, dq_partial, grads->q_vec, s2);
+            if (rc) return rc;
+        }
     }
     if (!fused64) {
         rc = launch_transpose(w->w_add, wadd_t, q, d, s);
@@ -807,7 +850,6 @@
     int* pos = (int*)(base + L.pos);
     int* n_live = (int*)(base + L.n_live);
     const bool compact = skip_pad_rows(desc);
-    const HeadPerm perm{d / desc->n_heads, desc->n_heads};
     if (gather) {
         rc = launch_compact_live_rows((long)M, ids, live, compact ? pos : nullptr, n_live, (int*)(base + L.cscr), s);
         if (rc) return rc;
@@ -829,12 +871,14 @@
         rc = bwd_wqkv(desc, gather ? acts->x : x, dqkv, n_live, grads, tn_partial, s2);
         if (rc) return rc;
     }
-    rc = launch_transpose(w->w_qkv, wqkv_t, 3 * d, d, s, perm);
-    if (rc) return rc;
+    if (prep_aside) {
+        if (hipStreamWaitEvent(s, ss->ev[5], 0) != hipSuccess) { set_error("encoder_bwd: hipStreamWaitEvent failed"); return NRMS_ELAUNCH; }
+    } else {
+        rc = launch_transpose(w->w_qkv, wqkv_t, 3 * d, d, s, perm);
+        if (rc) return rc;
+    }
     {
-        NTArgs g{};
-        g.M = M; g.N = d; g.K = 3 * d; g.rows_per_tile = NT_BM;
-        g.A = dqkv; g.lda = 3 * d; g.W = wqkv_t;
+        NTArgs g = gx;
         g.C = gather ? dctx : dx; g.ldc = d;
         if (gather) { g.a_rows = compact ? nullptr : live; g.m_dev = n_live; }
         if (side && wo && gather && hipStreamWaitEvent(s, ss->ev[3], 0) != hipSuccess) {
@@ -973,6 +1017,20 @@
     NRMS_REQUIRE(n >= 0 && vocab > 0, "sanitize_ids_i32: n=%ld vocab=%d", (long)n, vocab);
     NRMS_REQUIRE(n == 0 || (src && dst && n_bad), "sanitize_ids_i32: null argument");
     return launch_sanitize_ids((long)n, src, true, dst, vocab, n_bad, (hipStream_t)stream);
+}
+
+extern "C" int nrms_sanitize_ids2(const int64_t* src0, int64_t n0, const int64_t* src1, int64_t n1, int64_t* dst, int32_t vocab,
+                                  int32_t* n_bad, void* stream) {
+    NRMS_REQUIRE(n0 >= 0 && n1 >= 0 && vocab > 0, "sanitize_ids2: n0=%ld n1=%ld vocab=%d", (long)n0, (long)n1, vocab);
+    NRMS_REQUIRE((n0 == 0 || src0) && (n1 == 0 || src1) && (n0 + n1 == 0 || (dst && n_bad)), "sanitize_ids2: null argument");
+    return launch_sanitize_ids2((long)n0, src0, (long)n1, src1, false, dst, vocab, n_bad, (hipStream_t)stream);
+}
+
+extern "C" int nrms_sanitize_ids2_i32(const int32_t* src0, int64_t n0, const int32_t* src1, int64_t n1, int64_t* dst, int32_t vocab,
+                                      int32_t* n_bad, void* stream) {
+    NRMS_REQUIRE(n0 >= 0 && n1 >= 0 && vocab > 0, "sanitize_ids2_i32: n0=%ld n1=%ld vocab=%d", (long)n0, (long)n1, vocab);
+    NRMS_REQUIRE((n0 == 0 || src0) && (n1 == 0 || src1) && (n0 + n1 == 0 || (dst && n_bad)), "sanitize_ids2_i32: null argument");
+    return launch_sanitize_ids2((long)n0, src0, (long)n1, src1, true, dst, vocab, n_bad, (hipStream_t)stream);
 }
 
 extern "C" size_t nrms_sequence_partition_count_ints(int32_t n_seq) { return n_seq >= 0 ? title_order_cnt_ints(n_seq) : 0; }
diff --git a/pytorch_news_recommender_amd/csrc/common.h b/pytorch_news_recommender_amd/csrc/common.h
--- a/pytorch_news_recommender_amd/csrc/common.h
+++ b/pytorch_news_recommender_amd/csrc/common.h
@@ -160,10 +160,10 @@
 void set_error(const char* fmt, ...);
 int check_launch(const char* what);
 
-constexpr int SIDE_EVENTS = 9, SIDE_EV_USER = 8;
+constexpr int SIDE_EVENTS = 10, SIDE_EV_USER = 8, SIDE_EV_PLANES = 9;
 struct SideSet {
     hipStream_t s[2] = {nullptr, nullptr};
-    hipEvent_t ev[SIDE_EVENTS] = {nullptr, nullptr, nullptr, nullptr, nullptr, nullptr, nullptr, nullptr, nullptr};
+    hipEvent_t ev[SIDE_EVENTS] = {nullptr, nullptr, nullptr, nullptr, nullptr, nullptr, nullptr, nullptr, nullptr, nullptr};
     bool pending = false;
     bool pending_user = false;
 };
diff --git a/pytorch_news_recommender_amd/csrc/embed.hip b/pytorch_news_recommender_amd/csrc/embed.hip
--- a/pytorch_news_recommender_amd/csrc/embed.hip
+++ b/pytorch_news_recommender_amd/csrc/embed.hip
@@ -1,6 +1,7 @@
 #include "gemm.h"
 
 #include <algorithm>
+#include <stdlib.h>
 
 namespace nrms {
 
@@ -478,6 +479,43 @@
     else
         hipLaunchKernelGGL(sanitize_ids_kernel<int64_t>, dim3(blocks), dim3(256), 0, stream, n, (const int64_t*)src, dst, (long)vocab, n_bad);
     return check_launch("sanitize_ids");
+}
+
+template <class SRC>
+__global__ __launch_bounds__(256) void sanitize_ids2_kernel(long n0, const SRC* src0, long n1, const SRC* src1, int64_t* dst, long vocab,
+                                                            int* n_bad) {
+    int bad = 0;
+    for (long i = (long)blockIdx.x * blockDim.x + threadIdx.x; i < n0 + n1; i += (long)gridDim.x * blockDim.x) {
+        const int64_t v = (int64_t)(i < n0 ? src0[i] : src1[i - n0]);
+        const bool ok = v >= 0 && v < vocab;
+        bad += ok ? 0 : 1;
+        dst[i] = ok ? v : 0;
+    }
+    const unsigned long long m = __ballot(bad != 0);
+    if (m != 0ull) {
+        bad = (int)wave_sum((float)bad);
+        if ((threadIdx.x & 63) == 0) atomicAdd(n_bad, bad);
+    }
+}
+
+int launch_sanitize_ids2(long n0, const void* src0, long n1, const void* src1, bool src_is_int32, int64_t* dst, int vocab, int* n_bad,
+                         hipStream_t stream) {
+    if (n0 + n1 <= 0) return NRMS_OK;
+    const char* serial_env = getenv("NRMS_SERIAL_SANITIZE");
+    if (serial_env != nullptr && atoi(serial_env) != 0) {
+        const int rc = launch_sanitize_ids(n0, src0, src_is_int32, dst, vocab, n_bad, stream);
+        return rc ? rc : launch_sanitize_ids(n1, src1, src_is_int32, dst + n0, vocab, n_bad, stream);
+    }
+    int blocks = cdiv(n0 + n1, 256 * 4);
+    if (blocks > 256 * 8) blocks = 256 * 8;
+    TimingScope ts("sanitize_ids", stream);
+    if (src_is_int32)
+        hipLaunchKernelGGL(sanitize_ids2_kernel<int32_t>, dim3(blocks), dim3(256), 0, stream, n0, (const int32_t*)src0, n1,
+                           (const int32_t*)src1, dst, (long)vocab, n_bad);
+    else
+        hipLaunchKernelGGL(sanitize_ids2_kernel<int64_t>, dim3(blocks), dim3(256), 0, stream, n0, (const int64_t*)src0, n1,
+                           (const int64_t*)src1, dst, (long)vocab, n_bad);
+    return check_launch("sanitize_ids2");
 }
 
 __global__ __launch_bounds__(256) void dedup_insert_kernel(long n, int L, const int64_t* ids, int* table, unsigned mask,
diff --git a/pytorch_news_recommender_amd/csrc/fused16_bwd.hip b/pytorch_news_recommender_amd/csrc/fused16_bwd.hip
--- a/pytorch_news_recommender_amd/csrc/fused16_bwd.hip
+++ b/pytorch_news_recommender_amd/csrc/fused16_bwd.hip
@@ -574,7 +574,7 @@
     return __uint_as_float((unsigned)(k + 127) << 23);
 }
 
-__global__ __launch_bounds__(256) void absmax_kernel(long n, const float* x, unsigned* max_bits) {
+__device__ __forceinline__ unsigned absmax_block(long n, const float* x) {
     unsigned m = 0u;
     const long tid = (long)blockIdx.x * blockDim.x + threadIdx.x, nth = (long)gridDim.x * blockDim.x;
     if ((reinterpret_cast<uintptr_t>(x) & 15) == 0) {
@@ -604,10 +604,29 @@
     __shared__ unsigned wmax[4];
     if ((threadIdx.x & 63) == 0) wmax[threadIdx.x >> 6] = m;
     __syncthreads();
-    if (threadIdx.x == 0) {
-        m = max(max(wmax[0], wmax[1]), max(wmax[2], wmax[3]));
-        if (m != 0u) atomicMax(max_bits, m);
-    }
+    return max(max(wmax[0], wmax[1]), max(wmax[2], wmax[3]));
+}
+
+__global__ __launch_bounds__(256) void absmax_kernel(long n, const float* x, unsigned* max_bits) {
+    const unsigned m = absmax_block(n, x);
+    if (threadIdx.x == 0 && m != 0u) atomicMax(max_bits, m);
+}
+
+constexpr int ABSMAX_ROW = 512;
+__global__ __launch_bounds__(256) void absmax_row_kernel(long n, const float* x, unsigned* row) {
+    const unsigned m = absmax_block(n, x);
+    if (threadIdx.x == 0) row[blockIdx.x] = m;
+}
+
+__device__ __forceinline__ unsigned block_rowmax(const unsigned* row, int n) {
+    __shared__ unsigned rmax[4];
+    unsigned m = 0u;
+    for (int i = threadIdx.x; i < n; i += 256) m = max(m, row[i]);
+#pragma unroll
+    for (int o = 32; o > 0; o >>= 1) m = max(m, (unsigned)__shfl_xor((int)m, o, 64));
+    if ((threadIdx.x & 63) == 0) rmax[threadIdx.x >> 6] = m;
+    __syncthreads();
+    return max(max(rmax[0], rmax[1]), max(rmax[2], rmax[3]));
 }
 
 __device__ __forceinline__ void dout16_rows(long n_seq, int d, int h, int dk, float scale, float* sc, const float* dout, _Float16* dout16,
@@ -1039,6 +1058,20 @@
     dout16_rows(n_seq, d, h, dk, scale, sc, dout, dout16, n_rows_blocks);
 }
 
+__global__ __launch_bounds__(256) void dout16_maps_row_kernel(long n_seq, int d, int h, int dk, int q, float fixed_scale, float qscale,
+                                                              const unsigned* max_row, int n_max, float* sc, const float* dout,
+                                                              _Float16* dout16, Maps16 m) {
+    const unsigned max_bits = block_rowmax(max_row, n_max);
+    const float scale = loss_scale_from_max(max_bits, fixed_scale);
+    const int n_rows_blocks = (int)gridDim.x - MAPS16_BLOCKS;
+    if ((int)blockIdx.x >= n_rows_blocks) {
+        maps16_entry(((int)blockIdx.x - n_rows_blocks) * 256 + (int)threadIdx.x, d, h, dk, q, 1.0f / scale, qscale, m);
+        return;
+    }
+    if (blockIdx.x == 0 && threadIdx.x == 0) reinterpret_cast<unsigned*>(sc)[2] = max_bits;
+    dout16_rows(n_seq, d, h, dk, scale, sc, dout, dout16, n_rows_blocks);
+}
+
 static size_t up256(size_t x) { return (x + 255) / 256 * 256; }
 
 
@@ -1059,6 +1092,7 @@
     L.red = take((size_t)2 * L.n_wg * B16_RED * 4);
     L.maps = take((size_t)(B16_DQ * 2 + F16_KP + F16_QP * 2 + F16_DP) * 4);
     L.scale = take(256);
+    L.absmax = take((size_t)ABSMAX_ROW * 4);
     L.tn_splits_qkv = 40;
     L.tn_splits_add = 192;
     if (const char* e = getenv("NRMS_TN_SPLITS_QKV")) L.tn_splits_qkv = atoi(e);
@@ -1149,6 +1183,48 @@
     hipLaunchKernelGGL(dout16_maps_kernel, dim3(row_blocks + MAPS16_BLOCKS), dim3(256), 0, stream, n_seq, d, h, dk, q, fixed_scale,
                        qscale, max_bits, sc, dout, dout16, m);
     return check_launch("dout16");
+}
+
+static int launch_dout16_maps_row(long n_seq, int d, int h, int dk, int q, float fixed_scale, float qscale, float* sc, unsigned* max_row,
+                                  const float* dout, _Float16* dout16, const Maps16& m, hipStream_t stream) {
+    const long nd = n_seq * d;
+    int n_max = 0;
+    if (!(fixed_scale > 0.f)) {
+        n_max = nd > (long)ABSMAX_ROW * 1024 ? ABSMAX_ROW : (int)cdiv(nd, 1024);
+        hipLaunchKernelGGL(absmax_row_kernel, dim3(n_max), dim3(256), 0, stream, nd, dout, max_row);
+    }
+    const int row_blocks = cdiv(n_seq * F16_DP, 256) > 4096 ? 4096 : cdiv(n_seq * F16_DP, 256);
+    hipLaunchKernelGGL(dout16_maps_row_kernel, dim3(row_blocks + MAPS16_BLOCKS), dim3(256), 0, stream, n_seq, d, h, dk, q, fixed_scale,
+                       qscale, max_row, n_max, sc, dout, dout16, m);
+    return check_launch("dout16");
+}
+
+static bool bwd16_attn_dma(int S) {
+    const char* staged_env = getenv("NRMS_BWD_ATTN_STAGED");
+    return S <= 32 && !(staged_env != nullptr && atoi(staged_env) != 0);
+}
+
+bool fused_bwd16_serial_scale_chain() {
+    const char* e = getenv("NRMS_SERIAL_SCALE_CHAIN");
+    return e != nullptr && atoi(e) != 0;
+}
+
+static int launch_prep16b(const Fused16Bwd& f, const Fused16BwdLayout& L, bool clear_max, hipStream_t stream) {
+    char* base = (char*)f.workspace;
+    Prep16bArgs p{};
+    p.d = f.d; p.h = f.h; p.dk = f.d / f.h; p.q = f.q; p.w_qkv = f.w_qkv; p.b_qkv = f.b_qkv; p.w_add = f.w_add; p.q_vec = f.q_vec;
+    p.btiles = (_Float16*)(base + L.btiles); p.xtiles = (_Float16*)(base + L.xtiles); p.qv16 = (_Float16*)(base + L.qv16);
+    p.bqkv32 = (float*)(base + L.bqkv32);
+    p.dma_tiles = bwd16_attn_dma(f.S) ? 1 : 0;
+    p.max_bits = clear_max ? (unsigned*)(base + L.scale) + 2 : nullptr;
+    TimingScope ts("prep16", stream);
+    hipLaunchKernelGGL(prep16b_kernel, dim3(2048), dim3(256), 0, stream, p);
+    return check_launch("prep16b");
+}
+
+int launch_fused_bwd16_planes(const Fused16Bwd& f, hipStream_t stream) {
+    if (f.n_seq <= 0) return NRMS_OK;
+    return launch_prep16b(f, fused16_bwd_layout((long)f.n_seq * f.S, f.n_seq), false, stream);
 }
 
 int launch_fused_bwd16(const Fused16Bwd& f, hipStream_t stream) {
@@ -1183,23 +1259,23 @@
     hipStream_t s_add = side ? ss->s[0] : stream, s_qkv = side ? ss->s[1] : stream;
     SideJoinGuard join_guard(ss, stream);
     const int Mp = f.n_seq * 32 * (f.S > 32 ? 2 : 1);
-    const char* staged_env = getenv("NRMS_BWD_ATTN_STAGED");
-    const bool attn_dma = f.S <= 32 && !(staged_env != nullptr && atoi(staged_env) != 0);
+    const bool attn_dma = bwd16_attn_dma(f.S);
     {
-        Prep16bArgs p{};
-        p.d = f.d; p.h = f.h; p.dk = dk; p.q = f.q; p.w_qkv = f.w_qkv; p.b_qkv = f.b_qkv; p.w_add = f.w_add; p.q_vec = f.q_vec;
-        p.btiles = btiles; p.xtiles = xtiles; p.qv16 = qv16; p.bqkv32 = bqkv32;
-        p.dma_tiles = attn_dma ? 1 : 0;
-        p.max_bits = (unsigned*)(sc + 2);
-        TimingScope ts("prep16", stream);
-        hipLaunchKernelGGL(prep16b_kernel, dim3(2048), dim3(256), 0, stream, p);
-        int rc = check_launch("prep16b");
+        const bool serial = fused_bwd16_serial_scale_chain();
+        int rc = NRMS_OK;
+        if (f.planes_ready == nullptr) rc = launch_prep16b(f, L, serial, stream);
         if (rc) return rc;
         Maps16 mp;
         mp.nmap_qkv = nmap_qkv; mp.nscale_qkv = nscale_qkv; mp.kmap_x = kmap_x; mp.nmap_add = nmap_add; mp.nscale_add = nscale_add;
         mp.kmap_ctx = kmap_ctx;
-        rc = launch_dout16_maps((long)f.n_seq, f.d, f.h, dk, f.q, f.loss_scale, qscale, sc, f.dout, dout16, mp, stream);
+        if (serial) rc = launch_dout16_maps((long)f.n_seq, f.d, f.h, dk, f.q, f.loss_scale, qscale, sc, f.dout, dout16, mp, stream);
+        else rc = launch_dout16_maps_row((long)f.n_seq, f.d, f.h, dk, f.q, f.loss_scale, qscale, sc, (unsigned*)(base + L.absmax), f.dout,
+                                         dout16, mp, stream);
         if (rc) return rc;
+        if (f.planes_ready != nullptr && hipStreamWaitEvent(stream, f.planes_ready, 0) != hipSuccess) {
+            set_error("fused_bwd16: hipStreamWaitEvent failed");
+            return NRMS_ELAUNCH;
+        }
     }
     Bwd16Args a{};
     a.n_seq = f.n_seq; a.S = f.S; a.d = f.d; a.h = f.h; a.dk = dk; a.q = f.q;
diff --git a/pytorch_news_recommender_amd/csrc/gemm.h b/pytorch_news_recommender_amd/csrc/gemm.h
--- a/pytorch_news_recommender_amd/csrc/gemm.h
+++ b/pytorch_news_recommender_amd/csrc/gemm.h
@@ -28,6 +28,7 @@
     const int* a_rows;
     const int* m_dev;
     const int* c_rows;
+    bool w_planes_ready;
 };
 
 __device__ __forceinline__ int nt_swz(int row) { return (0x1230 >> (((row >> 2) & 3) * 4)) & 3; }
@@ -250,6 +251,7 @@
 
 int launch_gemm_nt_bf16(int amode, int emode, int npass, const NTArgs& a, void* wplanes, hipStream_t stream,
                         const char* name);
+int launch_gemm_nt_bf16_planes(const NTArgs& a, void* wplanes, hipStream_t stream);
 size_t gemm_nt_bf16_wplane_bytes(int N, int K);
 int launch_gemm_tn_bf16(int npass, const TNArgs& a, hipStream_t stream, const char* name);
 
@@ -297,7 +299,7 @@
 size_t title_order_cnt_ints(int n_seq);
 int launch_title_order(int n_seq, int S, const int64_t* ids, int* order, int* cnt, hipStream_t stream, int n_classes = 2);
 
-struct Fused16BwdLayout { int n_wg, tn_splits_qkv, tn_splits_add; size_t btiles, xtiles, qv16, bqkv32, dout16, dz16, dctx16, dqkv16, red, maps, scale, partial, total; };
+struct Fused16BwdLayout { int n_wg, tn_splits_qkv, tn_splits_add; size_t btiles, xtiles, qv16, bqkv32, dout16, dz16, dctx16, dqkv16, red, maps, scale, absmax, partial, total; };
 Fused16BwdLayout fused16_bwd_layout(long M, int n_seq);
 struct Fused16Bwd {
     int n_seq, S, d, h, q;
@@ -318,8 +320,11 @@
     const float** sc_out;
     bool defer_join;
     const float* w_o; const void* attn16; float* dw_o; float* db_o;
+    hipEvent_t planes_ready;
 };
 int launch_fused_bwd16(const Fused16Bwd& f, hipStream_t stream);
+int launch_fused_bwd16_planes(const Fused16Bwd& f, hipStream_t stream);
+bool fused_bwd16_serial_scale_chain();
 size_t fused16v1_bwd_bytes(long M, int n_seq, int h);
 int launch_fused_bwd16v1(const Fused16Bwd& f, hipStream_t stream);
 int fused_bwd16_join(hipStream_t stream, bool user = true);
@@ -335,8 +340,14 @@
 int launch_user64_bwd(int n_seq, int S, int d, int h, int q, const float* w_add, const float* q_vec, void* planes, const float* dout,
                       const float* t, const float* w, const void* qkv, float* ds, float* dq_partial, float* dq_vec, float* dqkv,
                       hipStream_t stream);
+int launch_user64_bwd_planes(int d, int h, int q, const float* w_add, const float* q_vec, void* planes, hipStream_t stream);
+int launch_user64_bwd_kernel(int n_seq, int S, int d, int h, int q, const void* planes, const float* dout, const float* t,
+                             const float* w, const void* qkv, float* ds, float* dq_partial, float* dqkv, hipStream_t stream);
+int launch_user64_bwd_dq(int n_seq, int q, const float* dq_partial, float* dq_vec, hipStream_t stream);
 
 int launch_sanitize_ids(long n, const void* src, bool src_is_int32, int64_t* dst, int vocab, int* n_bad, hipStream_t stream);
+int launch_sanitize_ids2(long n0, const void* src0, long n1, const void* src1, bool src_is_int32, int64_t* dst, int vocab, int* n_bad,
+                         hipStream_t stream);
 int launch_title_dedup(long n, int L, const int64_t* ids, int* table, long table_size, int* inverse, int* rep_rows,
                        int* n_unique, hipStream_t stream);
 int launch_gather_dropout(long M, int d, const int64_t* ids, const float* table, const Dropout& drop, float* x,
diff --git a/pytorch_news_recommender_amd/csrc/gemm_bf16.hip b/pytorch_news_recommender_amd/csrc/gemm_bf16.hip
--- a/pytorch_news_recommender_amd/csrc/gemm_bf16.hip
+++ b/pytorch_news_recommender_amd/csrc/gemm_bf16.hip
@@ -301,6 +301,11 @@
     }
 }
 
+int launch_gemm_nt_bf16_planes(const NTArgs& g, void* wplanes, hipStream_t stream) {
+    const int Kp = cdiv(g.K, BF_BK) * BF_BK, Np = cdiv(g.N, 16) * 16;
+    return launch_split_planes(g.W, g.N, Np, g.K, Kp, wplanes, (void*)((__bf16*)wplanes + (long)Np * Kp), stream);
+}
+
 int launch_gemm_nt_bf16(int amode, int emode, int npass, const NTArgs& g_in, void* wplanes, hipStream_t stream,
                         const char* name) {
     if (g_in.M <= 0) return NRMS_OK;
@@ -312,8 +317,10 @@
     a.Np = cdiv(g_in.N, 16) * 16;
     a.whi = (const __bf16*)wplanes;
     a.wlo = a.whi + (long)a.Np * a.Kp;
-    int rc = launch_split_planes(g_in.W, g_in.N, a.Np, g_in.K, a.Kp, wplanes, (void*)a.wlo, stream);
-    if (rc) return rc;
+    if (!g_in.w_planes_ready) {
+        const int rc = launch_gemm_nt_bf16_planes(g_in, wplanes, stream);
+        if (rc) return rc;
+    }
     if (npass == 3) {
         if (amode == A_PLAIN && emode == E_STORE) return launch_bf_mode<A_PLAIN, E_STORE, 3>(a, stream, name);
         if (amode == A_DZ && emode == E_DCTX) return launch_bf_mode<A_DZ, E_DCTX, 3>(a, stream, name);
diff --git a/pytorch_news_recommender_amd/csrc/pool.hip b/pytorch_news_recommender_amd/csrc/pool.hip
--- a/pytorch_news_recommender_amd/csrc/pool.hip
+++ b/pytorch_news_recommender_amd/csrc/pool.hip
@@ -1,4 +1,6 @@
 #include "gemm.h"
+
+#include <stdlib.h>
 
 namespace nrms {
 
@@ -275,30 +277,29 @@
     }
 }
 
-__global__ void ce_loss_kernel(int B, int C, const float* scores, float* loss_sum, float* dscores, float gscale) {
-    __shared__ float red[256];
-    float local = 0.f;
-    for (int b = threadIdx.x; b < B; b += blockDim.x) {
-        const float* s = scores + (long)b * C;
-        float mx = -3.0e38f;
-        for (int c = 0; c < C; ++c) mx = fmaxf(mx, s[c]);
-        double sum = 0.0;
-        for (int c0 = 0; c0 < C; c0 += 16) {
-            const int c1 = c0 + 16 < C ? c0 + 16 : C;
-            float run = 0.f;
-            for (int c = c0; c < c1; ++c) run += expf(s[c] - mx);
-            sum += (double)run;
-        }
-        local += (float)(((double)mx - (double)s[0]) + log(sum));
-        if (dscores != nullptr) {
-            const float inv = (float)(1.0 / sum);
-            for (int c = 0; c < C; ++c) {
-                const float e = expf(s[c] - mx);
-                const float p = (c == 0) ? __builtin_fmaf(e, inv, -1.0f) : e * inv;
-                dscores[(long)b * C + c] = p * gscale;
-            }
-        }
-    }
+__device__ __forceinline__ float ce_row(const float* s, int C, float* ds, float gscale) {
+    float mx = -3.0e38f;
+    for (int c = 0; c < C; ++c) mx = fmaxf(mx, s[c]);
+    double sum = 0.0;
+    for (int c0 = 0; c0 < C; c0 += 16) {
+        const int c1 = c0 + 16 < C ? c0 + 16 : C;
+        float run = 0.f;
+        for (int c = c0; c < c1; ++c) run += expf(s[c] - mx);
+        sum += (double)run;
+    }
+    const float loss = (float)(((double)mx - (double)s[0]) + log(sum));
+    if (ds != nullptr) {
+        const float inv = (float)(1.0 / sum);
+        for (int c = 0; c < C; ++c) {
+            const float e = expf(s[c] - mx);
+            const float p = (c == 0) ? __builtin_fmaf(e, inv, -1.0f) : e * inv;
+            ds[c] = p * gscale;
+        }
+    }
+    return loss;
+}
+
+__device__ __forceinline__ void ce_loss_tree(float local, float* red, float* loss_sum) {
     red[threadIdx.x] = local;
     __syncthreads();
     for (int o = 128; o > 0; o >>= 1) {
@@ -306,6 +307,64 @@
         __syncthreads();
     }
     if (threadIdx.x == 0) loss_sum[0] += red[0];
+}
+
+__global__ void ce_loss_kernel(int B, int C, const float* scores, float* loss_sum, float* dscores, float gscale) {
+    __shared__ float red[256];
+    float local = 0.f;
+    for (int b = threadIdx.x; b < B; b += blockDim.x)
+        local += ce_row(scores + (long)b * C, C, dscores != nullptr ? dscores + (long)b * C : nullptr, gscale);
+    ce_loss_tree(local, red, loss_sum);
+}
+
+__global__ __launch_bounds__(256) void click_ce_step_kernel(int B, int C, int d, const float* cand, const float* user,
+                                                            const uint8_t* mask, float gscale, float* scores, float* dscores,
+                                                            float* loss_sum, float* dcand, float* duser, float* loss_rows,
+                                                            unsigned* ticket) {
+    __shared__ float red[256];
+    __shared__ int last;
+    const int b = blockIdx.x;
+    const int lane = threadIdx.x & 63;
+    const float* uvec = user + (long)b * d;
+    for (int c = threadIdx.x >> 6; c < C; c += 4) {
+        const long u = (long)b * C + c;
+        const float* cv = cand + u * d;
+        float p = 0.f;
+        for (int k = lane; k < d; k += 64) p += cv[k] * uvec[k];
+        p = wave_sum(p);
+        if (lane == 0) scores[u] = (mask != nullptr && mask[u] == 0) ? -1e9f : p;
+    }
+    __syncthreads();
+    if (threadIdx.x == 0) loss_rows[b] = ce_row(scores + (long)b * C, C, dscores + (long)b * C, gscale);
+    __syncthreads();
+    for (int k = threadIdx.x; k < d; k += blockDim.x) {
+        const float uv = uvec[k];
+        float du = 0.f;
+        for (int c = 0; c < C; ++c) {
+            const long u = (long)b * C + c;
+            const float g = (mask != nullptr && mask[u] == 0) ? 0.f : dscores[u];
+            dcand[u * d + k] = g * uv;
+            du += g * cand[u * d + k];
+        }
+        duser[(long)b * d + k] = du;
+    }
+    if (threadIdx.x == 0) {
+        asm volatile("s_waitcnt vmcnt(0)" ::: "memory");
+        __builtin_amdgcn_fence(__ATOMIC_RELEASE, "agent");
+        asm volatile("s_waitcnt vmcnt(0)" ::: "memory");
+        const unsigned t = __hip_atomic_fetch_add(ticket, 1u, __ATOMIC_RELAXED, __HIP_MEMORY_SCOPE_AGENT);
+        last = t == (unsigned)(B - 1);
+        if (last) {
+            __builtin_amdgcn_fence(__ATOMIC_ACQUIRE, "agent");
+            asm volatile("s_waitcnt vmcnt(0)" ::: "memory");
+        }
+    }
+    __syncthreads();
+    if (!last) return;
+    float local = 0.f;
+    for (int r = threadIdx.x; r < B; r += blockDim.x) local += loss_rows[r];
+    ce_loss_tree(local, red, loss_sum);
+    if (threadIdx.x == 0) __hip_atomic_store(ticket, 0u, __ATOMIC_RELAXED, __HIP_MEMORY_SCOPE_AGENT);
 }
 
 template <bool GUARD>
@@ -476,6 +535,34 @@
     return check_launch("ce_loss");
 }
 
+extern "C" size_t nrms_click_ce_step_workspace_bytes(int32_t B) { return B >= 0 ? 256 + (size_t)B * sizeof(float) : 0; }
+
+extern "C" int nrms_click_ce_step(int32_t B, int32_t C, int32_t d, const float* cand, const float* user, const uint8_t* mask,
+                                  float grad_scale, float* scores, float* dscores, float* loss_sum, float* dcand, float* duser,
+                                  void* workspace, size_t workspace_bytes, void* stream) {
+    NRMS_REQUIRE(B >= 0 && C > 0 && d > 0 && cand && user && scores && dscores && loss_sum && dcand && duser && workspace,
+                 "click_ce_step: bad arguments");
+    NRMS_REQUIRE(workspace_bytes >= nrms_click_ce_step_workspace_bytes(B) && ((uintptr_t)workspace & 3) == 0,
+                 "click_ce_step: workspace %zu < required %zu bytes (or not 4-byte aligned)", workspace_bytes,
+                 nrms_click_ce_step_workspace_bytes(B));
+    if (B == 0) return NRMS_OK;
+    hipStream_t s = (hipStream_t)stream;
+    unsigned* ticket = (unsigned*)workspace;
+    float* loss_rows = (float*)((char*)workspace + 256);
+    const char* serial_env = getenv("NRMS_SERIAL_SCORE_HEAD");
+    if (serial_env != nullptr && atoi(serial_env) != 0) {
+        int rc = nrms_click_score_fwd(B, C, d, cand, user, mask, scores, stream);
+        if (rc == NRMS_OK) rc = nrms_ce_loss_fwd_bwd(B, C, scores, loss_sum, dscores, grad_scale, stream);
+        if (rc == NRMS_OK) rc = nrms_click_score_bwd(B, C, d, cand, user, mask, dscores, dcand, duser, stream);
+        return rc;
+    }
+    TimingScope ts_ce("ce_loss_click_ce_step", s);
+    TimingScope ts_bwd("click_bwd_click_ce_step", s);
+    hipLaunchKernelGGL(click_ce_step_kernel, dim3(B), dim3(256), 0, s, B, C, d, cand, user, mask, grad_scale, scores, dscores,
+                       loss_sum, dcand, duser, loss_rows, ticket);
+    return check_launch("click_ce_step");
+}
+
 namespace nrms {
 AdamConsts adam_consts(double lr, double beta1, double beta2, double eps, int32_t step) {
     const double bc1 = 1.0 - pow(beta1, (double)step);
diff --git a/pytorch_news_recommender_amd/csrc/user64.hip b/pytorch_news_recommender_amd/csrc/user64.hip
--- a/pytorch_news_recommender_amd/csrc/user64.hip
+++ b/pytorch_news_recommender_amd/csrc/user64.hip
@@ -801,33 +801,46 @@
 }
 
 size_t user64_dq_partial_floats(int n_seq) { return (size_t)cdiv(n_seq > 0 ? n_seq : 1, 2) * U_QP; }
+int launch_user64_bwd_planes(int d, int h, int q, const float* w_add, const float* q_vec, void* planes, hipStream_t stream) {
+    char* pb = (char*)planes;
+    U64PrepArgs p{};
+    p.d = d; p.h = h; p.dk = d / h; p.q = q; p.w_add = w_add; p.q_vec = q_vec;
+    p.btiles = (__bf16*)pb; p.qv = (float*)(pb + (size_t)h * U_BTILE);
+    TimingScope ts("user64_prep", stream);
+    hipLaunchKernelGGL(user64_prep_kernel, dim3(512), dim3(256), 0, stream, p);
+    return check_launch("user64_prep");
+}
+
+int launch_user64_bwd_kernel(int n_seq, int S, int d, int h, int q, const void* planes, const float* dout, const float* t,
+                             const float* w, const void* qkv, float* ds, float* dq_partial, float* dqkv, hipStream_t stream) {
+    if (n_seq <= 0) return NRMS_OK;
+    const char* pb = (const char*)planes;
+    U64BwdArgs a{};
+    a.n_seq = n_seq; a.S = S; a.d = d; a.h = h; a.dk = d / h; a.q = q; a.qscale = 1.0f / sqrtf((float)(d / h));
+    a.btiles = pb; a.qv = (const float*)(pb + (size_t)h * U_BTILE); a.dout = dout; a.t = t; a.w = w;
+    a.qkvf = (const b8*)qkv; a.ctxf = (const b8*)((const char*)qkv + user64_ctxf_offset(n_seq, h));
+    a.ds = ds; a.dq_partial = dq_partial; a.dqkv = dqkv;
+    const hipError_t e = hipFuncSetAttribute((const void*)user64_bwd_kernel, hipFuncAttributeMaxDynamicSharedMemorySize, U_BWD_LDS);
+    if (e != hipSuccess) { set_error("user64_bwd: hipFuncSetAttribute: %s", hipGetErrorString(e)); return NRMS_ELAUNCH; }
+    TimingScope ts("user64_bwd", stream);
+    hipLaunchKernelGGL(user64_bwd_kernel, dim3(cdiv(n_seq, 2)), dim3(U_THREADS), U_BWD_LDS, stream, a);
+    return check_launch("user64_bwd");
+}
+
+int launch_user64_bwd_dq(int n_seq, int q, const float* dq_partial, float* dq_vec, hipStream_t stream) {
+    if (n_seq <= 0) return NRMS_OK;
+    return launch_colsum_add(dq_partial, cdiv(n_seq, 2), q, dq_vec, stream);
+}
+
 int launch_user64_bwd(int n_seq, int S, int d, int h, int q, const float* w_add, const float* q_vec, void* planes, const float* dout,
                       const float* t, const float* w, const void* qkv, float* ds, float* dq_partial, float* dq_vec, float* dqkv,
                       hipStream_t stream) {
     if (n_seq <= 0) return NRMS_OK;
-    char* pb = (char*)planes;
-    U64PrepArgs p{};
-    p.d = d; p.h = h; p.dk = d / h; p.q = q; p.w_add = w_add; p.q_vec = q_vec;
-    p.btiles = (__bf16*)pb; p.qv = (float*)(pb + (size_t)h * U_BTILE);
-    {
-        TimingScope ts("user64_prep", stream);
-        hipLaunchKernelGGL(user64_prep_kernel, dim3(512), dim3(256), 0, stream, p);
-    }
-    U64BwdArgs a{};
-    a.n_seq = n_seq; a.S = S; a.d = d; a.h = h; a.dk = d / h; a.q = q; a.qscale = 1.0f / sqrtf((float)(d / h));
-    a.btiles = pb; a.qv = p.qv; a.dout = dout; a.t = t; a.w = w;
-    a.qkvf = (const b8*)qkv; a.ctxf = (const b8*)((const char*)qkv + user64_ctxf_offset(n_seq, h));
-    a.ds = ds; a.dq_partial = dq_partial; a.dqkv = dqkv;
-    const hipError_t e = hipFuncSetAttribute((const void*)user64_bwd_kernel, hipFuncAttributeMaxDynamicSharedMemorySize, U_BWD_LDS);
-    if (e != hipSuccess) { set_error("user64_bwd: hipFuncSetAttribute: %s", hipGetErrorString(e)); return NRMS_ELAUNCH; }
-    const int n_wg = cdiv(n_seq, 2);
-    {
-        TimingScope ts("user64_bwd", stream);
-        hipLaunchKernelGGL(user64_bwd_kernel, dim3(n_wg), dim3(U_THREADS), U_BWD_LDS, stream, a);
-    }
-    int rc = check_launch("user64_bwd");
+    int rc = launch_user64_bwd_planes(d, h, q, w_add, q_vec, planes, stream);
     if (rc) return rc;
-    return launch_colsum_add(dq_partial, n_wg, q, dq_vec, stream);
-}
-
-}
+    rc = launch_user64_bwd_kernel(n_seq, S, d, h, q, planes, dout, t, w, qkv, ds, dq_partial, dqkv, stream);
+    if (rc) return rc;
+    return launch_user64_bwd_dq(n_seq, q, dq_partial, dq_vec, stream);
+}
+
+}
diff --git a/pytorch_news_recommender_amd/engine.py b/pytorch_news_recommender_amd/engine.py
--- a/pytorch_news_recommender_amd/engine.py
+++ b/pytorch_news_recommender_amd/engine.py
@@ -269,6 +269,20 @@
         self._bad_event = ev
         return dst
 
+    def sanitize_ids2(self, src0, src1, dst):
+        n0, n1 = src0.numel(), src1.numel()
+        if src0.dtype != src1.dtype or n0 == 0 or n1 == 0:
+            flat = dst.reshape(-1)
+            self.sanitize_ids(src0, flat[:n0])
+            self.sanitize_ids(src1, flat[n0:])
+            return dst
+        fn = self.lib.nrms_sanitize_ids2_i32 if src0.dtype == torch.int32 else self.lib.nrms_sanitize_ids2
+        rc = fn(_lib.ptr(src0), C.c_int64(n0), _lib.ptr(src1), C.c_int64(n1), _lib.ptr(dst), int(self.dims.n_words),
+                _lib.ptr(self._bad_ids), _stream())
+        _lib.check(rc, "nrms_sanitize_ids2")
+        self.note_bad_ids()
+        return dst
+
     def note_bad_ids(self):
         self._bad_host.copy_(self._bad_ids, non_blocking=True)
         ev = torch.cuda.Event()
@@ -365,7 +379,7 @@
         return out
 
     def forward(self, flat, hist_ids, cand_ids, cand_mask, training, p_drop=0.0, seed=0, user_mask=None,
-                user_mask_mode=0):
+                user_mask_mode=0, want_scores=True):
         B, H, L = hist_ids.shape
         Cn = cand_ids.shape[1]
         d = self.dims.word_embed_size
@@ -373,8 +387,7 @@
         sfx = "" if training else "_eval"
         self.poll_ids()
         ids = self._buf("ids" + sfx, N * L, torch.int64)[:N * L].view(N, L)
-        self.sanitize_ids(hist_ids.reshape(B * H, L).contiguous(), ids[:B * H])
-        self.sanitize_ids(cand_ids.reshape(B * Cn, L).contiguous(), ids[B * H:])
+        self.sanitize_ids2(hist_ids.reshape(B * H, L).contiguous(), cand_ids.reshape(B * Cn, L).contiguous(), ids)
         nv = self._buf("news_vec" + sfx, N * d)[:N * d].view(N, d)
         p = float(p_drop)
         p_embed = 0.0 if self.dims.style == "v1" else p
@@ -386,8 +399,10 @@
         self.encode_users(flat, hist, out=user, save=training, tag="user" + sfx, mask=user_mask, mask_mode=user_mask_mode)
         if cand_mask is not None:
             cand_mask = cand_mask.contiguous()
-        scores = torch.empty(B, Cn, dtype=torch.float32, device=self.device)
-        self.click_scores(cand, user, cand_mask, out=scores)
+        scores = None
+        if want_scores:
+            scores = torch.empty(B, Cn, dtype=torch.float32, device=self.device)
+            self.click_scores(cand, user, cand_mask, out=scores)
         if training:
             self._gen += 1
             self._saved = dict(B=B, H=H, C=Cn, L=L, ids=ids, nv=nv, user=user, mask=cand_mask, p=p, p_embed=p_embed,
@@ -404,6 +419,30 @@
                                            C.c_float(gs), _stream())
         _lib.check(rc, "nrms_ce_loss_fwd_bwd")
         return loss_sum, dscores
+
+    def click_ce_step(self, grad_scale=None):
+        sv = self._saved
+        if sv is None:
+            raise _lib.NrmsError("click_ce_step() without a training forward()")
+        B, H, Cn = sv["B"], sv["H"], sv["C"]
+        key, _ = self.POOLED_VEC
+        width = sv[key].shape[1]
+        cand, user, dvec, duser = self._head_buffers(sv, width)
+        scores = torch.empty(B, Cn, dtype=torch.float32, device=self.device)
+        dscores = torch.empty_like(scores)
+        loss_sum = torch.zeros(1, dtype=torch.float32, device=self.device)
+        nbytes = int(self.lib.nrms_click_ce_step_workspace_bytes(B))
+        ws = getattr(self, "_score_head_ws", None)
+        if ws is None or ws.numel() * 4 < nbytes:
+            ws = self._score_head_ws = torch.zeros((nbytes + 3) // 4, dtype=torch.int32, device=self.device)
+        gs = (1.0 / B) if grad_scale is None else grad_scale
+        rc = self.lib.nrms_click_ce_step(B, Cn, width, _lib.ptr(cand), _lib.ptr(user), _lib.ptr(sv["mask"]), C.c_float(gs),
+                                         _lib.ptr(scores), _lib.ptr(dscores), _lib.ptr(loss_sum),
+                                         C.c_void_p(dvec[B * H:].data_ptr()), _lib.ptr(duser), _lib.ptr(ws),
+                                         C.c_size_t(ws.numel() * 4), _stream())
+        _lib.check(rc, "nrms_click_ce_step")
+        self._head_done = (sv["gen"], dscores)
+        return scores, loss_sum, dscores
 
     def _bwd_workspace(self, *descs):
         nbytes = max(self.lib.nrms_encoder_bwd_workspace_bytes(C.byref(d)) for d in descs)
@@ -456,6 +495,8 @@
             if getattr(self, "_pooled_gen", None) != sv["gen"]:
                 raise _lib.NrmsError("backward(dscores=None) needs the gradients of pooled_ce_loss(), and none was computed for "
                                      "training forward #%d" % sv["gen"])
+        elif getattr(self, "_head_done", None) is not None and self._head_done[0] == sv["gen"] and self._head_done[1] is dscores:
+            self._head_done = None
         else:
             rc = self.lib.nrms_click_score_bwd(B, Cn, width, _lib.ptr(cand), _lib.ptr(user), _lib.ptr(sv["mask"]),
                                                _lib.ptr(dscores.contiguous()), C.c_void_p(dvec[B * H:].data_ptr()), _lib.ptr(duser),
diff --git a/pytorch_news_recommender_amd/model/_flat_model.py b/pytorch_news_recommender_amd/model/_flat_model.py
--- a/pytorch_news_recommender_amd/model/_flat_model.py
+++ b/pytorch_news_recommender_amd/model/_flat_model.py
@@ -6,7 +6,7 @@
 import torch.nn as nn
 
 from .. import _lib
-from ..engine import nrms_entries
+from ..engine import NRMSEngine, nrms_entries
 
 
 def news_encoder_entries(dims, extra):
@@ -181,12 +181,18 @@
         st = self._opt
         p_drop = float(self.config.dropout) if self.training else 0.0
         seed = self._next_seed() if p_drop > 0 else 0
-        scores = eng.forward(self._flat, *args, training=True, p_drop=p_drop, seed=seed)
-        gb = scores.shape[0] * world_size if global_batch is None else global_batch
-        if pooled:
-            loss_sum, dscores = self._pooled_loss(batch, 1.0 / gb), None
+        fused_head = not pooled and type(eng).forward is NRMSEngine.forward and type(eng).backward is NRMSEngine.backward
+        if fused_head:
+            eng.forward(self._flat, *args, training=True, p_drop=p_drop, seed=seed, want_scores=False)
+            gb = eng._saved["B"] * world_size if global_batch is None else global_batch
+            scores, loss_sum, dscores = eng.click_ce_step(grad_scale=1.0 / gb)
         else:
-            loss_sum, dscores = eng.ce_loss(scores, grad_scale=1.0 / gb)
+            scores = eng.forward(self._flat, *args, training=True, p_drop=p_drop, seed=seed)
+            gb = scores.shape[0] * world_size if global_batch is None else global_batch
+            if pooled:
+                loss_sum, dscores = self._pooled_loss(batch, 1.0 / gb), None
+            else:
+                loss_sum, dscores = eng.ce_loss(scores, grad_scale=1.0 / gb)
         lr_ = float(self.config.learning_rate if lr is None else lr)
         if self._fuses_table_adam(world_size, all_reduce):
             n_table = self._layout.entries[self._names[0]][2]
```

Measured after the change: 177,800 users/s, median of 6. About the same (+0.4%).
